# handasontam/PERT-GNN-KDD23

Hardware: AMD Instinct MI355X
Metric: training graphs/sec (whole node) (higher is better)
Workload: dtype bf16; 1 GPU; model=PERT-GNN 8L/256H, global_batch=1024, vocab=realistic, interfaces=2041, entry_unions=266, graph_mode=full, parallelism=dp1

## Files before the change

csrc/bindings.cpp:

```cpp
#include <hip/hip_runtime.h>
#include <torch/extension.h>

#include <cstdlib>

#include <c10/cuda/CUDAStream.h>

namespace {

#define CHECK_IN(t)                                                      \
  TORCH_CHECK((t).is_cuda(), #t " must be on GPU");                      \
  TORCH_CHECK((t).is_contiguous(), #t " must be contiguous")

inline hipStream_t cur_stream() {
  return (hipStream_t)c10::cuda::getCurrentCUDAStream().stream();
}

}

void launch_edge_attn_fwd(const float*, const float*, const float*,
                          const float*, const int*, const int*, const float*,
                          float*, float*, int, int, hipStream_t);
void launch_edge_attn_bwd(const float*, const float*, const float*,
                          const float*, const float*, const float*, const int*,
                          const int*, const int*, const int*, float*, float*,
                          float*, float*, float*, float*, int, int, long,
                          hipStream_t);
void launch_seg_pool_fwd(const float*, const float*, const float*, const int*,
                         float*, float*, int, int, int, hipStream_t);
void launch_seg_pool_bwd(const float*, const float*, const float*, const long*,
                         float*, long, int, hipStream_t);
void launch_embed_node_fwd(const float*, const long*, const float*, float*,
                           long, int, int, hipStream_t);
void launch_embed_node_fwd16(const float*, const long*, const float*, void*,
                             long, int, int, hipStream_t);
void launch_vocab_scatter16(const void*, const long*, long, float*, long, int,
                            int, int, int, hipStream_t);
void launch_embed_edge_fwd(const long*, const float*, const float*, float*,
                           long, int, int, hipStream_t);
void launch_gather_rows(const long*, const float*, float*, long, int,
                        hipStream_t);
bool bn_wide_ok(int);
int bn_wide_slab_rows(long, int);
void launch_bn_fwd(const float*, const float*, const float*, float*, float*,
                   float*, float*, float*, float*, long, int, float, float,
                   bool, bool, float, const unsigned long long*, float*,
                   hipStream_t);
void launch_counter_bump(unsigned long long*, hipStream_t);
void launch_bn_bwd(const float*, const float*, const float*, const float*,
                   const float*, const float*, float*, float*, float*, float*,
                   long, int, bool, float, float*, hipStream_t);
void launch_bn_stats_only(const float*, long, int, float*, float*,
                          hipStream_t);
void launch_bn_finalize_apply(const float*, const float*, const float*,
                              const float*, const float*, float*, float*,
                              float*, float*, float*, long, int, float, float,
                              bool, bool, float, const unsigned long long*,
                              hipStream_t);
void launch_bn_bwd_partials_only(const float*, const float*, const float*,
                                 const float*, const float*, long, int, bool,
                                 float*, float, float*, hipStream_t);
void launch_bn_bwd_apply_only(const float*, const float*, const float*,
                              const float*, const float*, const float*,
                              const float*, const float*, float*, long, int,
                              bool, float, hipStream_t);
void launch_bn_grad_affine(const float*, float*, float*, int, hipStream_t);
void launch_bn_stats_only16(const void*, long, int, float*, float*,
                            hipStream_t);
void launch_bn_fwd16(const void*, const float*, const float*, float*, float*,
                     float*, float*, float*, void*, long, int, float, float,
                     bool, bool, float, const unsigned long long*, float*,
                     unsigned char*, hipStream_t);
void launch_bn_finalize_apply16(const void*, const float*, const float*,
                                const float*, const float*, float*, float*,
                                float*, float*, void*, long, int, float, float,
                                bool, bool, float, const unsigned long long*,
                                unsigned char*, hipStream_t);
void launch_bn_bwd_partials_only16(const void*, const void*, const void*,
                                   const float*, const float*, long, int, bool,
                                   float*, float, float*,
                                   const unsigned char*, hipStream_t);
void launch_bn_bwd_apply_only16(const void*, const void*, const void*,
                                const float*, const float*, const float*,
                                const float*, const float*, void*, long, int,
                                bool, float, const unsigned char*,
                                hipStream_t);
void launch_bn_bwd16(const void*, const void*, const void*, const float*,
                     const float*, const float*, float*, void*, float*,
                     float*, long, int, bool, float, float*,
                     const unsigned char*, hipStream_t);
void launch_seg_pool_fwd16(const void*, const float*, const float*,
                           const int*, float*, float*, int, int, int,
                           hipStream_t);
void launch_seg_pool_bwd16(const float*, const float*, const float*,
                           const long*, void*, long, int, hipStream_t);
void launch_gemm_bf16_nt_a16o16(const void*, const float*, const float*,
                                void*, int, int, int, hipStream_t);
void launch_gemm_bf16_nn_a16o16(const void*, const float*, void*, int, int,
                                int, hipStream_t);
void launch_gemm_bf16_tn_a16b16(const void*, const void*, float*, float*, int,
                                int, int, hipStream_t);
void launch_gemm_fp16_nt_a16o16(const void*, const float*, const float*,
                                void*, int, int, int, hipStream_t);
void launch_gemm_fp16_nn_a16o16(const void*, const float*, void*, int, int,
                                int, hipStream_t);
void launch_gemm_fp16_tn_a16b16(const void*, const void*, float*, float*, int,
                                int, int, hipStream_t);
void launch_quantile_loss_fwd(const float*, const float*, float*, long, float,
                              hipStream_t);
void launch_quantile_loss_bwd(const float*, const float*, const float*, float*,
                              long, float, hipStream_t);
void launch_eval_metrics(const float*, const float*, float*, long, float,
                         hipStream_t);
void launch_adam(float*, const float*, float*, float*, float*, long, float,
                 float, float, float, float, hipStream_t);
void launch_adam_dynamic(float*, const float*, float*, float*, float*, float*,
                         long, float, float, float, float, float, float,
                         float, hipStream_t);
void launch_gemm_f32_nt(const float*, const float*, const float*, float*, int,
                        int, int, bool, hipStream_t);
void launch_gemm_f32_nn(const float*, const float*, const float*, float*, int,
                        int, int, bool, hipStream_t);
void launch_gemm_f32_tn(const float*, const float*, float*, float*, int, int,
                        int, hipStream_t);
void launch_colsum(const float*, float*, long, int, hipStream_t);
void launch_gemm_bf16_nt(const float*, const float*, const float*, float*,
                         int, int, int, bool, hipStream_t);
void launch_gemm_bf16_nn(const float*, const float*, const float*, float*,
                         int, int, int, bool, hipStream_t);
void launch_gemm_bf16_tn(const float*, const float*, float*, float*, int, int,
                         int, hipStream_t);
void launch_gemm_fp16_nt(const float*, const float*, const float*, float*,
                         int, int, int, bool, hipStream_t);
void launch_gemm_fp16_nn(const float*, const float*, const float*, float*,
                         int, int, int, bool, hipStream_t);
void launch_gemm_fp16_tn(const float*, const float*, float*, float*, int, int,
                         int, hipStream_t);
void launch_embed_grouped_scatter(const float*, const int*, const int*, float*,
                                  float*, long, int, int, int, int, int,
                                  hipStream_t);
void launch_embed_grouped_scatter_bal(const void*, int, const int*,
                                      const int*, const int*, const int*,
                                      const int*, const int*, float*, float*,
                                      float*, int, int, int, int, int, int,
                                      hipStream_t);
void launch_rows_sum_lists(const void*, int, const int*, const int*, void*, int,
                           int, int, int, hipStream_t);
void launch_vocab_scatter(const float*, const long*, long, float*, long, int,
                          int, int, int, hipStream_t);
void launch_vocab_scatter_dual(const float*, const long*, int, float*, float*,
                               long, int, int, int, hipStream_t);
void launch_edge_attn_fused_fwd(const float*, const float*, const float*,
                                const long*, int, const int*, const int*,
                                float*, float*, int, int, int, hipStream_t);
void launch_edge_attn_fused_bwd(const float*, const float*, const float*,
                                const float*, const long*, int, const float*,
                                const int*, const int*, const int*,
                                const int*, const int*, float*, float*,
                                float*, int, int, long, int, hipStream_t);
void launch_edge_attn_fused_fwd16(const void*, const void*, const void*,
                                  int, const long*, int, const int*,
                                  const int*, void*, int, float*, int, int,
                                  int, hipStream_t);
void launch_edge_attn_fused_bwd16(const void*, int, const void*,
                                  const void*, const void*, int, const long*,
                                  int, const float*, const int*, const int*,
                                  const int*, const int*, const int*, void*,
                                  void*, float*, int, int, long, int,
                                  hipStream_t);
void launch_edge_attn_fused_infer(const float*, const float*, const float*,
                                  const long*, int, const int*, const int*,
                                  const float*, const float*, int, float*,
                                  int, int, int, hipStream_t);
void launch_edge_attn_fused_infer16(const void*, const void*, const void*,
                                    int, const long*, int, const int*,
                                    const int*, const float*, const float*,
                                    int, void*, int, int, int, int,
                                    hipStream_t);
void launch_vocab_scatter_dual16(const void*, const long*, int, float*,
                                 float*, long, int, int, int, hipStream_t);
void launch_gemm_bf16_nt_o16(const float*, const float*, const float*, void*,
                             int, int, int, hipStream_t);
void launch_gemm_a16_glds_nt(const void*, const void*, const float*,
                             const float*, void*, int, int, int, int, bool,
                             hipStream_t);
void launch_convert_w16(const float*, void*, long, hipStream_t);
void launch_gemm_a16_glds_tn(const void*, const void*, float*, float*, int,
                             int, int, hipStream_t);
void launch_transpose_convert_w16(const float*, void*, int, int, hipStream_t);
void launch_gemm_skinny_nn(const void*, const float*, float*, int, int, int,
                           hipStream_t);
void launch_gemm_bf16_nn_a16(const void*, const float*, float*, int, int, int,
                             hipStream_t);
void launch_gemm_bf16_tn_a16(const void*, const float*, float*, float*, int,
                             int, int, hipStream_t);
int ptables_max_groups();
void launch_ptables_fwd(int, const float* const*, const float* const*,
                        void* const*, const int*, int, int, hipStream_t);
void launch_ptables_dgrad(const void* const*, const float* const*, const int*,
                          float* const*, const int*, int, int, bool,
                          hipStream_t);
bool launch_ptables_wgrad(int, const void* const*, const float* const*,
                          float* const*, const int*, int, bool, hipStream_t);
std::vector<torch::Tensor> collate_native(
    std::vector<torch::Tensor>, std::vector<torch::Tensor>,
    std::vector<torch::Tensor>, std::vector<torch::Tensor>,
    std::vector<torch::Tensor>, std::vector<torch::Tensor>,
    std::vector<torch::Tensor>, std::vector<torch::Tensor>,
    std::vector<torch::Tensor>, bool);


std::vector<torch::Tensor> edge_attn_fwd(torch::Tensor q, torch::Tensor k,
                                         torch::Tensor v, torch::Tensor e,
                                         torch::Tensor row_ptr,
                                         torch::Tensor csr_src,
                                         torch::Tensor skip) {
  CHECK_IN(q); CHECK_IN(k); CHECK_IN(v); CHECK_IN(e);
  CHECK_IN(row_ptr); CHECK_IN(csr_src);
  const int n = q.size(0);
  const int h = q.size(1);
  TORCH_CHECK(h <= 512, "H must be <= 512");
  auto out = torch::empty_like(q);
  auto alpha = torch::empty({e.size(0)}, q.options());
  const float* skip_p = nullptr;
  if (skip.defined() && skip.numel() > 0) {
    CHECK_IN(skip);
    skip_p = skip.data_ptr<float>();
  }
  launch_edge_attn_fwd(q.data_ptr<float>(), k.data_ptr<float>(),
                       v.data_ptr<float>(), e.data_ptr<float>(),
                       row_ptr.data_ptr<int>(), csr_src.data_ptr<int>(),
                       skip_p, out.data_ptr<float>(), alpha.data_ptr<float>(),
                       n, h, cur_stream());
  return {out, alpha};
}

std::vector<torch::Tensor> edge_attn_bwd(
    torch::Tensor g, torch::Tensor q, torch::Tensor k, torch::Tensor v,
    torch::Tensor e, torch::Tensor alpha, torch::Tensor row_ptr,
    torch::Tensor csr_src, torch::Tensor col_ptr, torch::Tensor csc_dst,
    torch::Tensor csc_eid) {
  CHECK_IN(g); CHECK_IN(q); CHECK_IN(alpha);
  const int n = q.size(0);
  const int h = q.size(1);
  const long ne = e.size(0);
  auto dq = torch::empty_like(q);
  auto dk = torch::empty_like(k);
  auto dv = torch::empty_like(v);
  auto de = torch::empty_like(e);
  auto dek = torch::empty_like(e);
  auto dev = torch::empty_like(e);
  launch_edge_attn_bwd(g.data_ptr<float>(), q.data_ptr<float>(),
                       k.data_ptr<float>(), v.data_ptr<float>(),
                       e.data_ptr<float>(), alpha.data_ptr<float>(),
                       row_ptr.data_ptr<int>(), csr_src.data_ptr<int>(),
                       col_ptr.data_ptr<int>(), csc_eid.data_ptr<int>(),
                       dq.data_ptr<float>(), dk.data_ptr<float>(),
                       dv.data_ptr<float>(), de.data_ptr<float>(),
                       dek.data_ptr<float>(), dev.data_ptr<float>(), n, h, ne,
                       cur_stream());
  return {dq, dk, dv, de};
}

torch::Tensor seg_pool_fwd(torch::Tensor x, torch::Tensor probs,
                           torch::Tensor nn, torch::Tensor batch_ptr,
                           int64_t num_graphs) {
  CHECK_IN(x); CHECK_IN(probs); CHECK_IN(nn); CHECK_IN(batch_ptr);
  const int h = x.size(1);
  const long n = x.size(0);
  long p = 8192 / std::max<int64_t>(num_graphs, 1);
  const long per_g = (n + std::max<int64_t>(num_graphs, 1) - 1) /
                     std::max<int64_t>(num_graphs, 1);
  p = std::min<long>(std::max<long>(std::min(p, per_g), 1), 64);
  auto partial = torch::empty({num_graphs * p, h}, x.options());
  auto out = torch::empty({num_graphs, h}, x.options());
  launch_seg_pool_fwd(x.data_ptr<float>(), probs.data_ptr<float>(),
                      nn.data_ptr<float>(), batch_ptr.data_ptr<int>(),
                      partial.data_ptr<float>(), out.data_ptr<float>(),
                      (int)num_graphs, (int)p, h, cur_stream());
  return out;
}

torch::Tensor seg_pool_bwd(torch::Tensor gout, torch::Tensor probs,
                           torch::Tensor nn, torch::Tensor batch) {
  CHECK_IN(gout); CHECK_IN(batch);
  const long n = batch.size(0);
  const int h = gout.size(1);
  auto dx = torch::empty({n, h}, gout.options());
  launch_seg_pool_bwd(gout.data_ptr<float>(), probs.data_ptr<float>(),
                      nn.data_ptr<float>(), batch.data_ptr<long>(),
                      dx.data_ptr<float>(), n, h, cur_stream());
  return dx;
}

torch::Tensor embed_node_fwd(torch::Tensor x_raw, torch::Tensor idx,
                             torch::Tensor table, bool out16 = false) {
  CHECK_IN(x_raw); CHECK_IN(idx); CHECK_IN(table);
  const long n = x_raw.size(0);
  const int f = x_raw.size(1);
  const int h = table.size(1);
  if (out16) {
    auto out = torch::empty({n, f + h},
                            x_raw.options().dtype(torch::kBFloat16));
    launch_embed_node_fwd16(x_raw.data_ptr<float>(), idx.data_ptr<long>(),
                            table.data_ptr<float>(), out.data_ptr(), n, f, h,
                            cur_stream());
    return out;
  }
  auto out = torch::empty({n, f + h}, x_raw.options());
  launch_embed_node_fwd(x_raw.data_ptr<float>(), idx.data_ptr<long>(),
                        table.data_ptr<float>(), out.data_ptr<float>(), n, f,
                        h, cur_stream());
  return out;
}

torch::Tensor embed_edge_fwd(torch::Tensor attr, torch::Tensor ifc,
                             torch::Tensor rpc) {
  CHECK_IN(attr); CHECK_IN(ifc); CHECK_IN(rpc);
  const long e = attr.size(0);
  const int h = ifc.size(1);
  const int astride = attr.size(1);
  auto out = torch::empty({e, 2 * h}, ifc.options());
  launch_embed_edge_fwd(attr.data_ptr<long>(), ifc.data_ptr<float>(),
                        rpc.data_ptr<float>(), out.data_ptr<float>(), e, h,
                        astride, cur_stream());
  return out;
}

torch::Tensor gather_rows(torch::Tensor idx, torch::Tensor table) {
  CHECK_IN(idx); CHECK_IN(table);
  const long n = idx.size(0);
  const int h = table.size(1);
  auto out = torch::empty({n, h}, table.options());
  launch_gather_rows(idx.data_ptr<long>(), table.data_ptr<float>(),
                     out.data_ptr<float>(), n, h, cur_stream());
  return out;
}

static const unsigned long long* rng_seed_ptr(torch::Tensor& seed,
                                              double dropout_p) {
  if (dropout_p <= 0.0 || !seed.defined() || seed.numel() == 0) return nullptr;
  TORCH_CHECK(seed.scalar_type() == torch::kLong && seed.is_cuda(),
              "dropout seed must be an int64 CUDA scalar");
  return (const unsigned long long*)seed.data_ptr<long>();
}

static torch::Tensor bn_wide_slab(const torch::Tensor& x) {
  const long rows = bn_wide_slab_rows(x.size(0), (int)x.size(1));
  return torch::empty({rows, 2 * x.size(1)},
                      x.options().dtype(torch::kFloat32));
}
static float* bn_slab_ptr(const torch::Tensor& slab) {
  return slab.numel() ? slab.data_ptr<float>() : nullptr;
}
static const unsigned char* bn_mask_ptr(const torch::Tensor& ym,
                                        const torch::Tensor& x) {
  if (ym.scalar_type() != torch::kUInt8) return nullptr;
  TORCH_CHECK(ym.is_contiguous() && x.size(1) % 8 == 0 &&
                  ym.numel() == x.size(0) * (x.size(1) / 8) &&
                  bn_wide_ok((int)x.size(1)),
              "BN keep mask must be a contiguous uint8 [n, h/8] tensor");
  return ym.data_ptr<unsigned char>();
}
static torch::Tensor bn_new_mask(const torch::Tensor& x, bool training,
                                 bool relu) {
  const long n = x.size(0), h = x.size(1);
  const bool on = training && relu && n > 0 && bn_wide_ok((int)h);
  return torch::empty({on ? n : 0, on ? h / 8 : 0},
                      x.options().dtype(torch::kUInt8));
}

std::vector<torch::Tensor> bn_relu_fwd(torch::Tensor x, torch::Tensor gamma,
                                       torch::Tensor beta,
                                       torch::Tensor running_mean,
                                       torch::Tensor running_var,
                                       double momentum, double eps,
                                       bool training, bool relu,
                                       double dropout_p = 0.0,
                                       torch::Tensor seed = {}) {
  CHECK_IN(x); CHECK_IN(gamma); CHECK_IN(beta);
  const long n = x.size(0);
  const int h = x.size(1);
  auto y = torch::empty_like(x);
  auto mean = torch::empty({h}, x.options());
  auto invstd = torch::empty({h}, x.options());
  auto partials = torch::empty({2 * h}, x.options());
  auto slab = training ? bn_wide_slab(x) : torch::empty({0}, x.options());
  const auto* sp = rng_seed_ptr(seed, dropout_p);
  launch_bn_fwd(x.data_ptr<float>(), gamma.data_ptr<float>(),
                beta.data_ptr<float>(), running_mean.data_ptr<float>(),
                running_var.data_ptr<float>(), mean.data_ptr<float>(),
                invstd.data_ptr<float>(), partials.data_ptr<float>(),
                y.data_ptr<float>(), n, h, (float)momentum, (float)eps,
                training, relu, (float)dropout_p, sp, bn_slab_ptr(slab),
                cur_stream());
  if (sp) launch_counter_bump((unsigned long long*)seed.data_ptr<long>(),
                              cur_stream());
  return {y, mean, invstd};
}

std::vector<torch::Tensor> bn_relu_bwd(torch::Tensor g, torch::Tensor x,
                                       torch::Tensor gamma, torch::Tensor mean,
                                       torch::Tensor invstd, torch::Tensor y,
                                       bool relu, double keep_inv = 1.0) {
  CHECK_IN(g); CHECK_IN(x);
  const long n = x.size(0);
  const int h = x.size(1);
  auto dx = torch::empty_like(x);
  auto dgamma = torch::empty({h}, x.options());
  auto dbeta = torch::empty({h}, x.options());
  auto partials = torch::empty({2 * h}, x.options());
  auto slab = bn_wide_slab(x);
  launch_bn_bwd(g.data_ptr<float>(), x.data_ptr<float>(), y.data_ptr<float>(),
                mean.data_ptr<float>(), invstd.data_ptr<float>(),
                gamma.data_ptr<float>(), partials.data_ptr<float>(),
                dx.data_ptr<float>(), dgamma.data_ptr<float>(),
                dbeta.data_ptr<float>(), n, h, relu, (float)keep_inv,
                bn_slab_ptr(slab), cur_stream());
  return {dx, dgamma, dbeta};
}

torch::Tensor quantile_loss_fwd(torch::Tensor y, torch::Tensor y_hat,
                                double tau) {
  CHECK_IN(y); CHECK_IN(y_hat);
  auto out = torch::empty({}, y_hat.options());
  launch_quantile_loss_fwd(y.data_ptr<float>(), y_hat.data_ptr<float>(),
                           out.data_ptr<float>(), y.size(0), (float)tau,
                           cur_stream());
  return out;
}

torch::Tensor quantile_loss_bwd(torch::Tensor g, torch::Tensor y,
                                torch::Tensor y_hat, double tau) {
  auto gc = g.contiguous();
  auto dy_hat = torch::empty_like(y_hat);
  launch_quantile_loss_bwd(gc.data_ptr<float>(), y.data_ptr<float>(),
                           y_hat.data_ptr<float>(), dy_hat.data_ptr<float>(),
                           y.size(0), (float)tau, cur_stream());
  return dy_hat;
}

std::vector<torch::Tensor> eval_metrics(torch::Tensor y, torch::Tensor y_hat,
                                        double tau) {
  CHECK_IN(y); CHECK_IN(y_hat);
  auto out3 = torch::empty({3}, y_hat.options());
  launch_eval_metrics(y.data_ptr<float>(), y_hat.data_ptr<float>(),
                      out3.data_ptr<float>(), y.size(0), (float)tau,
                      cur_stream());
  return {out3[0], out3[1], out3[2]};
}

void adam_step(torch::Tensor p, torch::Tensor g, torch::Tensor m,
               torch::Tensor v, torch::Tensor state, double lr, double b1,
               double b2, double eps, double gscale = 1.0) {
  CHECK_IN(p); CHECK_IN(g); CHECK_IN(m); CHECK_IN(v); CHECK_IN(state);
  launch_adam(p.data_ptr<float>(), g.data_ptr<float>(), m.data_ptr<float>(),
              v.data_ptr<float>(), state.data_ptr<float>(), p.numel(),
              (float)lr, (float)b1, (float)b2, (float)eps, (float)gscale, cur_stream());
}

void adam_step_dynamic(torch::Tensor p, torch::Tensor g, torch::Tensor m,
                       torch::Tensor v, torch::Tensor state,
                       torch::Tensor sstate, double lr, double b1, double b2,
                       double eps, double backoff, double growth,
                       double growth_interval) {
  CHECK_IN(p); CHECK_IN(g); CHECK_IN(m); CHECK_IN(v); CHECK_IN(state);
  CHECK_IN(sstate);
  TORCH_CHECK(sstate.numel() >= 3, "scaler state needs 3 elements");
  launch_adam_dynamic(p.data_ptr<float>(), g.data_ptr<float>(),
                      m.data_ptr<float>(), v.data_ptr<float>(),
                      state.data_ptr<float>(), sstate.data_ptr<float>(),
                      p.numel(), (float)lr, (float)b1, (float)b2, (float)eps,
// ... 467 lines not shown
      gamma.data_ptr<float>(), beta.data_ptr<float>(),
      running_mean.data_ptr<float>(), running_var.data_ptr<float>(),
      mean.data_ptr<float>(), invstd.data_ptr<float>(), y.data_ptr<float>(),
      x.size(0), h, (float)momentum, (float)eps, training, relu,
      (float)dropout_p, sp, cur_stream());
  if (sp) launch_counter_bump((unsigned long long*)seed.data_ptr<long>(),
                              cur_stream());
  return {y, mean, invstd};
}

torch::Tensor bn_bwd_partials(torch::Tensor g, torch::Tensor x,
                              torch::Tensor y, torch::Tensor mean,
                              torch::Tensor invstd, bool relu,
                              double keep_inv = 1.0) {
  CHECK_IN(g); CHECK_IN(x);
  const long h = x.size(1);
  auto partials = torch::empty({2 * h + 1}, x.options());
  auto slab = bn_wide_slab(x);
  launch_bn_bwd_partials_only(g.data_ptr<float>(), x.data_ptr<float>(),
                              y.data_ptr<float>(), mean.data_ptr<float>(),
                              invstd.data_ptr<float>(), x.size(0), h,
                              relu, partials.data_ptr<float>(),
                              (float)keep_inv, bn_slab_ptr(slab),
                              cur_stream());
  partials.narrow(0, 2 * h, 1).fill_((float)x.size(0));
  return partials;
}

std::vector<torch::Tensor> bn_bwd_apply(torch::Tensor g, torch::Tensor x,
                                        torch::Tensor y, torch::Tensor mean,
                                        torch::Tensor invstd,
                                        torch::Tensor gamma,
                                        torch::Tensor partials_global,
                                        torch::Tensor partials_local,
                                        bool relu, double keep_inv = 1.0) {
  CHECK_IN(g); CHECK_IN(x);
  const int h = x.size(1);
  TORCH_CHECK(partials_global.numel() == 2 * h + 1,
              "bn_bwd_apply expects [2h+1] partials with the global count "
              "in the tail slot");
  auto dx = torch::empty_like(x);
  auto dgamma = torch::empty({h}, x.options());
  auto dbeta = torch::empty({h}, x.options());
  launch_bn_bwd_apply_only(g.data_ptr<float>(), x.data_ptr<float>(),
                           y.data_ptr<float>(), mean.data_ptr<float>(),
                           invstd.data_ptr<float>(), gamma.data_ptr<float>(),
                           partials_global.data_ptr<float>(),
                           partials_global.data_ptr<float>() + 2 * h,
                           dx.data_ptr<float>(), x.size(0), h, relu,
                           (float)keep_inv, cur_stream());
  launch_bn_grad_affine(partials_local.data_ptr<float>(),
                        dgamma.data_ptr<float>(), dbeta.data_ptr<float>(), h,
                        cur_stream());
  return {dx, dgamma, dbeta};
}

torch::Tensor linear_dgrad(torch::Tensor g, torch::Tensor w, int64_t prec) {
  CHECK_IN(g); CHECK_IN(w);
  const int m = g.size(0);
  const int n = w.size(0);
  const int k = w.size(1);
  auto dx = torch::empty({m, k}, g.options());
  if (prec == 1)
    launch_gemm_bf16_nn(g.data_ptr<float>(), w.data_ptr<float>(), nullptr,
                        dx.data_ptr<float>(), m, n, k, false, cur_stream());
  else if (prec == 2)
    launch_gemm_fp16_nn(g.data_ptr<float>(), w.data_ptr<float>(), nullptr,
                        dx.data_ptr<float>(), m, n, k, false, cur_stream());
  else
    launch_gemm_f32_nn(g.data_ptr<float>(), w.data_ptr<float>(), nullptr,
                       dx.data_ptr<float>(), m, n, k, false, cur_stream());
  return dx;
}

std::vector<torch::Tensor> linear_wgrad(torch::Tensor g, torch::Tensor x,
                                        bool has_bias, int64_t prec) {
  CHECK_IN(g); CHECK_IN(x);
  const int m = x.size(0);
  const int k = x.size(1);
  const int n = g.size(1);
  auto dw = torch::empty({n, k}, x.options());
  torch::Tensor db = torch::empty({0}, g.options());
  float* db_ptr = nullptr;
  if (has_bias) {
    db = torch::empty({n}, g.options());
    db_ptr = db.data_ptr<float>();
  }
  if (prec == 1)
    launch_gemm_bf16_tn(g.data_ptr<float>(), x.data_ptr<float>(),
                        dw.data_ptr<float>(), db_ptr, m, n, k, cur_stream());
  else if (prec == 2)
    launch_gemm_fp16_tn(g.data_ptr<float>(), x.data_ptr<float>(),
                        dw.data_ptr<float>(), db_ptr, m, n, k, cur_stream());
  else
    launch_gemm_f32_tn(g.data_ptr<float>(), x.data_ptr<float>(),
                       dw.data_ptr<float>(), db_ptr, m, n, k, cur_stream());
  return {dw, db};
}

std::vector<torch::Tensor> vocab_scatter_dual(torch::Tensor g,
                                              torch::Tensor ea, int64_t rows0,
                                              int64_t rows1) {
  CHECK_IN(g); CHECK_IN(ea);
  const int h = g.size(1);
  TORCH_CHECK(h % 256 == 0, "dual scatter needs h % 256 == 0");
  TORCH_CHECK((size_t)(rows0 + rows1) * h * 4 <= 160 * 1024, "tables too large");
  auto fopt = g.options().dtype(torch::kFloat32);
  auto dt0 = torch::empty({rows0, h}, fopt);
  auto dt1 = torch::empty({rows1, h}, fopt);
  if (g.scalar_type() == torch::kBFloat16)
    launch_vocab_scatter_dual16(g.data_ptr(), ea.data_ptr<long>(),
                                (int)ea.size(1), dt0.data_ptr<float>(),
                                dt1.data_ptr<float>(), g.size(0), (int)rows0,
                                (int)rows1, h, cur_stream());
  else
    launch_vocab_scatter_dual(g.data_ptr<float>(), ea.data_ptr<long>(),
                              (int)ea.size(1), dt0.data_ptr<float>(),
                              dt1.data_ptr<float>(), g.size(0), (int)rows0,
                              (int)rows1, h, cur_stream());
  return {dt0, dt1};
}

torch::Tensor linear_fwd_bf16_o16(torch::Tensor x, torch::Tensor w,
                                  torch::Tensor b) {
  CHECK_IN(x); CHECK_IN(w);
  const int m = x.size(0);
  const int k = x.size(1);
  const int n = w.size(0);
  auto y = torch::empty({m, n}, x.options().dtype(torch::kBFloat16));
  const float* bias = nullptr;
  if (b.defined() && b.numel() > 0) bias = b.data_ptr<float>();
  launch_gemm_bf16_nt_o16(x.data_ptr<float>(), w.data_ptr<float>(), bias,
                          y.data_ptr(), m, n, k,
                          cur_stream());
  return y;
}

torch::Tensor linear_dgrad16(torch::Tensor g, torch::Tensor w) {
  CHECK_IN(g); CHECK_IN(w);
  const int m = g.size(0);
  const int n = w.size(0);
  const int k = w.size(1);
  auto dx = torch::empty({m, k}, w.options());
  if (m <= 16) {
    launch_gemm_skinny_nn(g.data_ptr(), w.data_ptr<float>(),
                          dx.data_ptr<float>(), m, n, k, cur_stream());
    return dx;
  }
  launch_gemm_bf16_nn_a16(g.data_ptr(),
                          w.data_ptr<float>(), dx.data_ptr<float>(), m, n, k,
                          cur_stream());
  return dx;
}

std::vector<torch::Tensor> linear_wgrad16(torch::Tensor g, torch::Tensor x,
                                          bool has_bias) {
  CHECK_IN(g); CHECK_IN(x);
  const int m = x.size(0);
  const int k = x.size(1);
  const int n = g.size(1);
  auto dw = torch::empty({n, k}, x.options());
  torch::Tensor db = torch::empty({0}, x.options());
  float* db_ptr = nullptr;
  if (has_bias) {
    db = torch::empty({n}, x.options());
    db_ptr = db.data_ptr<float>();
  }
  launch_gemm_bf16_tn_a16(g.data_ptr(),
                          x.data_ptr<float>(), dw.data_ptr<float>(), db_ptr,
                          m, n, k, cur_stream());
  return {dw, db};
}



std::vector<torch::Tensor> bn_relu_fwd16(torch::Tensor x, torch::Tensor gamma,
                                         torch::Tensor beta,
                                         torch::Tensor running_mean,
                                         torch::Tensor running_var,
                                         double momentum, double eps,
                                         bool training, bool relu,
                                         double dropout_p = 0.0,
                                         torch::Tensor seed = {}) {
  CHECK_IN(x); CHECK_IN(gamma); CHECK_IN(beta);
  const long n = x.size(0);
  const int h = x.size(1);
  auto fopt = x.options().dtype(torch::kFloat32);
  auto y = torch::empty({n, h}, x.options().dtype(torch::kBFloat16));
  auto mean = torch::empty({h}, fopt);
  auto invstd = torch::empty({h}, fopt);
  auto partials = torch::empty({2 * h}, fopt);
  auto slab = training ? bn_wide_slab(x) : torch::empty({0}, fopt);
  auto mask = bn_new_mask(x, training, relu);
  const auto* sp = rng_seed_ptr(seed, dropout_p);
  launch_bn_fwd16(x.data_ptr(), gamma.data_ptr<float>(),
                  beta.data_ptr<float>(), running_mean.data_ptr<float>(),
                  running_var.data_ptr<float>(), mean.data_ptr<float>(),
                  invstd.data_ptr<float>(), partials.data_ptr<float>(),
                  y.data_ptr(), n, h, (float)momentum, (float)eps, training,
                  relu, (float)dropout_p, sp, bn_slab_ptr(slab),
                  mask.numel() ? mask.data_ptr<unsigned char>() : nullptr,
                  cur_stream());
  if (sp) launch_counter_bump((unsigned long long*)seed.data_ptr<long>(),
                              cur_stream());
  return {y, mean, invstd, mask};
}

std::vector<torch::Tensor> bn_relu_bwd16(torch::Tensor g, torch::Tensor x,
                                         torch::Tensor gamma,
                                         torch::Tensor mean,
                                         torch::Tensor invstd, torch::Tensor y,
                                         bool relu, double keep_inv = 1.0) {
  CHECK_IN(g); CHECK_IN(x);
  const long n = x.size(0);
  const int h = x.size(1);
  auto fopt = x.options().dtype(torch::kFloat32);
  auto dx = torch::empty_like(x);
  auto dgamma = torch::empty({h}, fopt);
  auto dbeta = torch::empty({h}, fopt);
  auto partials = torch::empty({2 * h}, fopt);
  auto slab = bn_wide_slab(x);
  launch_bn_bwd16(g.data_ptr(), x.data_ptr(), y.data_ptr(),
                  mean.data_ptr<float>(), invstd.data_ptr<float>(),
                  gamma.data_ptr<float>(), partials.data_ptr<float>(),
                  dx.data_ptr(), dgamma.data_ptr<float>(),
                  dbeta.data_ptr<float>(), n, h, relu, (float)keep_inv,
                  bn_slab_ptr(slab), bn_mask_ptr(y, x), cur_stream());
  return {dx, dgamma, dbeta};
}

std::vector<torch::Tensor> bn_finalize_apply16(
    torch::Tensor x, torch::Tensor partials,
    torch::Tensor gamma, torch::Tensor beta, torch::Tensor running_mean,
    torch::Tensor running_var, double momentum, double eps, bool training,
    bool relu, double dropout_p = 0.0, torch::Tensor seed = {}) {
  CHECK_IN(x); CHECK_IN(partials);
  const int h = x.size(1);
  TORCH_CHECK(partials.numel() == 2 * h + 1,
              "bn_finalize_apply16 expects [2h+1] partials with the global "
              "count in the tail slot");
  auto fopt = x.options().dtype(torch::kFloat32);
  auto y = torch::empty({x.size(0), h}, x.options().dtype(torch::kBFloat16));
  auto mean = torch::empty({h}, fopt);
  auto invstd = torch::empty({h}, fopt);
  auto mask = bn_new_mask(x, training, relu);
  const auto* sp = rng_seed_ptr(seed, dropout_p);
  launch_bn_finalize_apply16(
      x.data_ptr(), partials.data_ptr<float>(),
      partials.data_ptr<float>() + 2 * h,
      gamma.data_ptr<float>(), beta.data_ptr<float>(),
      running_mean.data_ptr<float>(), running_var.data_ptr<float>(),
      mean.data_ptr<float>(), invstd.data_ptr<float>(), y.data_ptr(),
      x.size(0), h, (float)momentum, (float)eps, training, relu,
      (float)dropout_p, sp,
      mask.numel() ? mask.data_ptr<unsigned char>() : nullptr, cur_stream());
  if (sp) launch_counter_bump((unsigned long long*)seed.data_ptr<long>(),
                              cur_stream());
  return {y, mean, invstd, mask};
}

torch::Tensor bn_bwd_partials16(torch::Tensor g, torch::Tensor x,
                                torch::Tensor y, torch::Tensor mean,
                                torch::Tensor invstd, bool relu,
                                double keep_inv = 1.0) {
  CHECK_IN(g); CHECK_IN(x);
  const long h = x.size(1);
  auto partials = torch::empty({2 * h + 1},
                               x.options().dtype(torch::kFloat32));
  auto slab = bn_wide_slab(x);
  launch_bn_bwd_partials_only16(g.data_ptr(), x.data_ptr(),
                                y.data_ptr(), mean.data_ptr<float>(),
                                invstd.data_ptr<float>(), x.size(0), h,
                                relu, partials.data_ptr<float>(),
                                (float)keep_inv, bn_slab_ptr(slab),
                                bn_mask_ptr(y, x), cur_stream());
  partials.narrow(0, 2 * h, 1).fill_((float)x.size(0));
  return partials;
}

std::vector<torch::Tensor> bn_bwd_apply16(
    torch::Tensor g, torch::Tensor x, torch::Tensor y, torch::Tensor mean,
    torch::Tensor invstd, torch::Tensor gamma, torch::Tensor partials_global,
    torch::Tensor partials_local, bool relu, double keep_inv = 1.0) {
  CHECK_IN(g); CHECK_IN(x);
  const int h = x.size(1);
  TORCH_CHECK(partials_global.numel() == 2 * h + 1,
              "bn_bwd_apply16 expects [2h+1] partials with the global count "
              "in the tail slot");
  auto fopt = x.options().dtype(torch::kFloat32);
  auto dx = torch::empty_like(x);
  auto dgamma = torch::empty({h}, fopt);
  auto dbeta = torch::empty({h}, fopt);
  launch_bn_bwd_apply_only16(g.data_ptr(), x.data_ptr(), y.data_ptr(),
                             mean.data_ptr<float>(), invstd.data_ptr<float>(),
                             gamma.data_ptr<float>(),
                             partials_global.data_ptr<float>(),
                             partials_global.data_ptr<float>() + 2 * h,
                             dx.data_ptr(), x.size(0), h, relu,
                             (float)keep_inv, bn_mask_ptr(y, x), cur_stream());
  launch_bn_grad_affine(partials_local.data_ptr<float>(),
                        dgamma.data_ptr<float>(), dbeta.data_ptr<float>(), h,
                        cur_stream());
  return {dx, dgamma, dbeta};
}

torch::Tensor seg_pool_fwd16(torch::Tensor x, torch::Tensor probs,
                             torch::Tensor nn, torch::Tensor batch_ptr,
                             int64_t num_graphs) {
  CHECK_IN(x); CHECK_IN(probs); CHECK_IN(nn); CHECK_IN(batch_ptr);
  const int h = x.size(1);
  const long n = x.size(0);
  long p = 8192 / std::max<int64_t>(num_graphs, 1);
  const long per_g = (n + std::max<int64_t>(num_graphs, 1) - 1) /
                     std::max<int64_t>(num_graphs, 1);
  p = std::min<long>(std::max<long>(std::min(p, per_g), 1), 64);
  auto fopt = x.options().dtype(torch::kFloat32);
  auto partial = torch::empty({num_graphs * p, h}, fopt);
  auto out = torch::empty({num_graphs, h}, fopt);
  launch_seg_pool_fwd16(x.data_ptr(), probs.data_ptr<float>(),
                        nn.data_ptr<float>(), batch_ptr.data_ptr<int>(),
                        partial.data_ptr<float>(), out.data_ptr<float>(),
                        (int)num_graphs, (int)p, h, cur_stream());
  return out;
}

torch::Tensor seg_pool_bwd16(torch::Tensor gout, torch::Tensor probs,
                             torch::Tensor nn, torch::Tensor batch) {
  CHECK_IN(gout); CHECK_IN(batch);
  const long n = batch.size(0);
  const int h = gout.size(1);
  auto dx = torch::empty({n, h}, gout.options().dtype(torch::kBFloat16));
  launch_seg_pool_bwd16(gout.data_ptr<float>(), probs.data_ptr<float>(),
                        nn.data_ptr<float>(), batch.data_ptr<long>(),
                        dx.data_ptr(), n, h, cur_stream());
  return dx;
}

torch::Tensor linear_fwd_a16o16(torch::Tensor x, torch::Tensor w,
                                torch::Tensor b, bool fp16c = false) {
  CHECK_IN(x); CHECK_IN(w);
  const int m = x.size(0);
  const int k = x.size(1);
  const int n = w.size(0);
  auto y = torch::empty({m, n}, x.options());
  const float* bias = nullptr;
  if (b.defined() && b.numel() > 0) bias = b.data_ptr<float>();
  if (fp16c) {
    launch_gemm_fp16_nt_a16o16(x.data_ptr(), w.data_ptr<float>(), bias,
                               y.data_ptr(), m, n, k, cur_stream());
    return y;
  }
  if (m >= 512 && n % 128 == 0 && k % 32 == 0) {
    auto w16 = torch::empty({n, k}, x.options());
    launch_convert_w16(w.data_ptr<float>(), w16.data_ptr(), (long)n * k,
                       cur_stream());
    launch_gemm_a16_glds_nt(x.data_ptr(), w16.data_ptr(),
                            w.data_ptr<float>(), bias, y.data_ptr(),
                            1, m, n, k, false, cur_stream());
    return y;
  }
  launch_gemm_bf16_nt_a16o16(x.data_ptr(), w.data_ptr<float>(), bias,
                             y.data_ptr(), m, n, k, cur_stream());
  return y;
}

torch::Tensor linear_dgrad16_o16(torch::Tensor g, torch::Tensor w,
                                 bool fp16c = false) {
  CHECK_IN(g); CHECK_IN(w);
  const int m = g.size(0);
  const int n = w.size(0);
  const int k = w.size(1);
  auto dx = torch::empty({m, k}, g.options());
  if (fp16c) {
    launch_gemm_fp16_nn_a16o16(g.data_ptr(), w.data_ptr<float>(),
                               dx.data_ptr(), m, n, k, cur_stream());
    return dx;
  }
  if (m >= 512 && k % 128 == 0 && n % 64 == 0) {
    auto wt16 = torch::empty({k, n}, g.options());
    launch_transpose_convert_w16(w.data_ptr<float>(), wt16.data_ptr(), n, k,
                                 cur_stream());
    launch_gemm_a16_glds_nt(g.data_ptr(), wt16.data_ptr(), nullptr, nullptr,
                            dx.data_ptr(), 1, m, k, n, false,
                            cur_stream());
    const int m_done = m - m % 128;
    if (m_done < m)
      launch_gemm_bf16_nn_a16o16(
          (const char*)g.data_ptr() + (long)m_done * n * 2,
          w.data_ptr<float>(),
          (char*)dx.data_ptr() + (long)m_done * k * 2, m - m_done, n, k,
          cur_stream());
    return dx;
  }
  launch_gemm_bf16_nn_a16o16(g.data_ptr(), w.data_ptr<float>(),
                             dx.data_ptr(), m, n, k, cur_stream());
  return dx;
}

std::vector<torch::Tensor> linear_wgrad16_b16(torch::Tensor g, torch::Tensor x,
                                              bool has_bias,
                                              bool fp16c = false) {
  CHECK_IN(g); CHECK_IN(x);
  const int m = x.size(0);
  const int k = x.size(1);
  const int n = g.size(1);
  auto fopt = x.options().dtype(torch::kFloat32);
  auto dw = torch::empty({n, k}, fopt);
  torch::Tensor db = torch::empty({0}, fopt);
  float* db_ptr = nullptr;
  if (has_bias) {
    db = torch::empty({n}, fopt);
    db_ptr = db.data_ptr<float>();
  }
  if (fp16c) {
    launch_gemm_fp16_tn_a16b16(g.data_ptr(), x.data_ptr(),
                               dw.data_ptr<float>(), db_ptr, m, n, k,
                               cur_stream());
    return {dw, db};
  }
  const char* det = getenv("PERTGNN_DETERMINISTIC");
  if (!(det && det[0] == '1') && m >= 512 && n % 128 == 0 && k % 128 == 0) {
    launch_gemm_a16_glds_tn(g.data_ptr(), x.data_ptr(), dw.data_ptr<float>(),
                            db_ptr, m, n, k, cur_stream());
    return {dw, db};
  }
  launch_gemm_bf16_tn_a16b16(g.data_ptr(), x.data_ptr(),
                             dw.data_ptr<float>(), db_ptr, m, n, k,
                             cur_stream());
  return {dw, db};
}


namespace {

int ptables_check(const torch::Tensor& ifc_table,
                  const torch::Tensor& rpc_table,
                  const std::vector<torch::Tensor>& we_ifc,
                  const std::vector<torch::Tensor>& we_rpc) {
  CHECK_IN(ifc_table); CHECK_IN(rpc_table);
  TORCH_CHECK(ifc_table.dim() == 2 && rpc_table.dim() == 2,
              "ptables: tables must be 2-D");
  TORCH_CHECK(ifc_table.scalar_type() == torch::kFloat32 &&
                  rpc_table.scalar_type() == torch::kFloat32,
              "ptables: tables must be float32");
  const int64_t h = ifc_table.size(1);
  TORCH_CHECK(h > 0 && rpc_table.size(1) == h,
              "ptables: tables must share a non-empty hidden size");
  TORCH_CHECK(!we_ifc.empty() && we_ifc.size() == we_rpc.size(),
              "ptables: need one we_ifc and one we_rpc per layer, got ",
              we_ifc.size(), " and ", we_rpc.size());
  for (const auto* list : {&we_ifc, &we_rpc})
    for (const auto& w : *list) {
      TORCH_CHECK(w.is_cuda() && w.device() == ifc_table.device(),
                  "ptables: weight must be on the tables' GPU");
      TORCH_CHECK(w.is_contiguous(), "ptables: weight must be contiguous");
      TORCH_CHECK(w.scalar_type() == torch::kFloat32,
                  "ptables: weight must be float32");
      TORCH_CHECK(w.dim() == 2 && w.size(0) == h && w.size(1) == h,
                  "ptables: weight must be [", h, ", ", h, "]");
    }
  TORCH_CHECK(ifc_table.size(0) < (1 << 30) && rpc_table.size(0) < (1 << 30) &&
                  h < (1 << 15),
              "ptables: table too large");
  return (int)h;
}

}

std::vector<torch::Tensor> ptables_fwd(torch::Tensor ifc_table,
                                       torch::Tensor rpc_table,
                                       std::vector<torch::Tensor> we_ifc,
                                       std::vector<torch::Tensor> we_rpc) {
  const int h = ptables_check(ifc_table, rpc_table, we_ifc, we_rpc);
  const int layers = (int)we_ifc.size();
  auto opt = ifc_table.options().dtype(torch::kBFloat16);
  std::vector<torch::Tensor> out;
  std::vector<const float*> a, w;
  std::vector<void*> c;
  std::vector<int> m;
  for (int t = 0; t < 2; ++t) {
    const auto& table = t == 0 ? ifc_table : rpc_table;
    const auto& ws = t == 0 ? we_ifc : we_rpc;
    for (int l = 0; l < layers; ++l) {
      out.push_back(torch::empty({table.size(0), h}, opt));
      a.push_back(table.data_ptr<float>());
      w.push_back(ws[l].data_ptr<float>());
      c.push_back(out.back().data_ptr());
      m.push_back((int)table.size(0));
    }
  }
  launch_ptables_fwd(2 * layers, a.data(), w.data(), c.data(), m.data(), h, h,
                     cur_stream());
  return out;
}

std::vector<torch::Tensor> ptables_bwd(std::vector<torch::Tensor> dP,
                                       torch::Tensor ifc_table,
                                       torch::Tensor rpc_table,
                                       std::vector<torch::Tensor> we_ifc,
                                       std::vector<torch::Tensor> we_rpc,
                                       int64_t dgrad_splits) {
  const int h = ptables_check(ifc_table, rpc_table, we_ifc, we_rpc);
  const int layers = (int)we_ifc.size();
  TORCH_CHECK((int)dP.size() == 2 * layers, "ptables_bwd: need ", 2 * layers,
              " dP entries, got ", dP.size());
  const int64_t rows[2] = {ifc_table.size(0), rpc_table.size(0)};
  bool missing = false;
  for (int g = 0; g < 2 * layers; ++g) {
    const auto& d = dP[g];
    if (!d.defined() || d.numel() == 0) {
      missing |= rows[g / layers] > 0;
      continue;
    }
    TORCH_CHECK(d.is_cuda() && d.device() == ifc_table.device(),
                "ptables_bwd: dP must be on the tables' GPU");
    TORCH_CHECK(d.is_contiguous(), "ptables_bwd: dP must be contiguous");
    TORCH_CHECK(d.scalar_type() == torch::kBFloat16,
                "ptables_bwd: dP must be bfloat16");
    TORCH_CHECK(d.dim() == 2 && d.size(0) == rows[g / layers] && d.size(1) == h,
                "ptables_bwd: dP[", g, "] must be [", rows[g / layers], ", ",
                h, "]");
  }
  const char* det_env = getenv("PERTGNN_DETERMINISTIC");
  const bool det = det_env && det_env[0] == '1';
  const int splits =
      det ? 1 : (int)std::min<int64_t>(std::max<int64_t>(dgrad_splits, 1), layers);

  const int64_t hh = (int64_t)h * h;
  const int64_t n_dw = 2 * layers * hh;
  auto buf = torch::empty({n_dw + (rows[0] + rows[1]) * h},
                          ifc_table.options());
  auto dW = buf.narrow(0, 0, n_dw).view({2 * layers, h, h});
  auto d_ifc = buf.narrow(0, n_dw, rows[0] * h).view({rows[0], h});
  auto d_rpc = buf.narrow(0, n_dw + rows[0] * h, rows[1] * h).view({rows[1], h});

  std::vector<const void*> dp_w, dp_d;
  std::vector<const float*> a_w, w_d;
  std::vector<float*> dw_w;
  std::vector<int> m_w;
  int npairs[2] = {0, 0};
  for (int g = 0; g < 2 * layers; ++g) {
    const auto& d = dP[g];
    if (!d.defined() || d.numel() == 0) continue;
    const int t = g / layers;
    const auto& table = t == 0 ? ifc_table : rpc_table;
    const auto& w = (t == 0 ? we_ifc : we_rpc)[g % layers];
    dp_w.push_back(d.data_ptr());
    a_w.push_back(table.data_ptr<float>());
    dw_w.push_back(dW.data_ptr<float>() + g * hh);
    m_w.push_back((int)rows[t]);
    dp_d.push_back(d.data_ptr());
    w_d.push_back(w.data_ptr<float>());
    ++npairs[t];
  }
  auto s = cur_stream();
  const bool zero_dw =
      missing || launch_ptables_wgrad((int)dp_w.size(), dp_w.data(), a_w.data(),
                                      dw_w.data(), m_w.data(), h, true, s);
  const bool zero_dt = splits > 1;
  if (zero_dw || zero_dt) {
    float* beg = buf.data_ptr<float>() + (zero_dw ? 0 : n_dw);
    const int64_t cnt = (zero_dw ? n_dw : 0) +
                        (zero_dt ? (rows[0] + rows[1]) * h : 0);
    const hipError_t err = hipMemsetAsync(beg, 0, cnt * sizeof(float), s);
    TORCH_CHECK(err == hipSuccess, "ptables_bwd: memset failed: ",
                hipGetErrorString(err));
  }
  float* outs[2] = {d_ifc.data_ptr<float>(), d_rpc.data_ptr<float>()};
  const int ms[2] = {(int)rows[0], (int)rows[1]};
  launch_ptables_dgrad(dp_d.data(), w_d.data(), npairs, outs, ms, h, splits,
                       zero_dt, s);
  launch_ptables_wgrad((int)dp_w.size(), dp_w.data(), a_w.data(), dw_w.data(),
                       m_w.data(), h, false, s);
  return {d_ifc, d_rpc, dW};
}

PYBIND11_MODULE(TORCH_EXTENSION_NAME, mod) {
  mod.def("ptables_fwd", &ptables_fwd, py::arg("ifc_table"),
          py::arg("rpc_table"), py::arg("we_ifc"), py::arg("we_rpc"));
  mod.def("ptables_bwd", &ptables_bwd, py::arg("dP"), py::arg("ifc_table"),
          py::arg("rpc_table"), py::arg("we_ifc"), py::arg("we_rpc"),
          py::arg("dgrad_splits") = 1);
  mod.def("ptables_max_groups", &ptables_max_groups);
  mod.def("linear_fwd_bf16_o16", &linear_fwd_bf16_o16);
  mod.def("linear_dgrad16", &linear_dgrad16);
  mod.def("linear_wgrad16", &linear_wgrad16);
  mod.def("vocab_scatter_dual", &vocab_scatter_dual);
  mod.def("linear_dgrad", &linear_dgrad);
  mod.def("linear_wgrad", &linear_wgrad);
  mod.def("embed_grouped_scatter_bal", &embed_grouped_scatter_bal);
  mod.def("edge_table_grad", &edge_table_grad, py::arg("de"), py::arg("idx1"),
          py::arg("lptr1"), py::arg("idx2"), py::arg("lptr2"),
          py::arg("idx3"), py::arg("lptr3"), py::arg("V"), py::arg("R"),
          py::arg("out_dtype"), py::arg("unroll") = 8);
  mod.def("bn_stats", &bn_stats);
  mod.def("bn_finalize_apply", &bn_finalize_apply, py::arg("x"),
          py::arg("partials"), py::arg("gamma"), py::arg("beta"),
          py::arg("running_mean"), py::arg("running_var"), py::arg("momentum"),
          py::arg("eps"), py::arg("training"), py::arg("relu"),
          py::arg("dropout_p") = 0.0, py::arg("seed") = torch::Tensor());
  mod.def("bn_bwd_partials", &bn_bwd_partials, py::arg("g"), py::arg("x"),
          py::arg("y"), py::arg("mean"), py::arg("invstd"), py::arg("relu"),
          py::arg("keep_inv") = 1.0);
  mod.def("bn_bwd_apply", &bn_bwd_apply, py::arg("g"), py::arg("x"),
          py::arg("y"), py::arg("mean"), py::arg("invstd"), py::arg("gamma"),
          py::arg("partials_global"), py::arg("partials_local"),
          py::arg("relu"), py::arg("keep_inv") = 1.0);
  mod.def("vocab_scatter", &vocab_scatter);
  mod.def("collate_native", &collate_native,
          py::call_guard<py::gil_scoped_release>());
  mod.def("edge_attn_fused_fwd", &edge_attn_fused_fwd, py::arg("qkvs"),
          py::arg("pifc"), py::arg("prpc"), py::arg("edge_attr"),
          py::arg("row_ptr"), py::arg("csr_src"), py::arg("out16"),
          py::arg("heads") = 1);
  mod.def("edge_attn_fused_bwd", &edge_attn_fused_bwd, py::arg("g"),
          py::arg("qkvs"), py::arg("pifc"), py::arg("prpc"),
          py::arg("edge_attr"), py::arg("alpha"), py::arg("row_ptr"),
          py::arg("csr_src"), py::arg("col_ptr"), py::arg("csc_dst"),
          py::arg("csc_eid"), py::arg("heads") = 1);
  mod.def("edge_attn_fused_infer", &edge_attn_fused_infer, py::arg("qkvs"),
          py::arg("pifc"), py::arg("prpc"), py::arg("edge_attr"),
          py::arg("row_ptr"), py::arg("csr_src"), py::arg("bn_scale"),
          py::arg("bn_shift"), py::arg("relu"), py::arg("out16"),
          py::arg("heads") = 1);
  mod.def("embed_grouped_scatter", &embed_grouped_scatter);
  mod.def("linear_fwd", &linear_fwd);
  mod.def("linear_fwd_bf16", &linear_fwd_bf16);
  mod.def("linear_fwd_fp16", &linear_fwd_fp16);
  mod.def("linear_bwd_fp16", &linear_bwd_fp16);
  mod.def("linear_bwd_bf16", &linear_bwd_bf16);
  mod.def("gemm_nt_bf16", &gemm_nt_bf16);
  mod.def("gemm_nn_bf16", &gemm_nn_bf16);
  mod.def("gemm_tn_bf16", &gemm_tn_bf16);
  mod.def("linear_bwd", &linear_bwd);
  mod.def("gemm_nt", &gemm_nt);
  mod.def("gemm_nn", &gemm_nn);
  mod.def("gemm_tn", &gemm_tn);
  mod.def("edge_attn_fwd", &edge_attn_fwd);
  mod.def("edge_attn_bwd", &edge_attn_bwd);
  mod.def("seg_pool_fwd", &seg_pool_fwd);
  mod.def("seg_pool_bwd", &seg_pool_bwd);
  mod.def("embed_node_fwd", &embed_node_fwd, py::arg("x_raw"), py::arg("idx"), py::arg("table"), py::arg("out16") = false);
  mod.def("embed_edge_fwd", &embed_edge_fwd);
  mod.def("gather_rows", &gather_rows);
  mod.def("bn_relu_fwd16", &bn_relu_fwd16, py::arg("x"), py::arg("gamma"),
          py::arg("beta"), py::arg("running_mean"), py::arg("running_var"),
          py::arg("momentum"), py::arg("eps"), py::arg("training"),
          py::arg("relu"), py::arg("dropout_p") = 0.0,
          py::arg("seed") = torch::Tensor());
  mod.def("bn_relu_bwd16", &bn_relu_bwd16, py::arg("g"), py::arg("x"),
          py::arg("gamma"), py::arg("mean"), py::arg("invstd"), py::arg("y"),
          py::arg("relu"), py::arg("keep_inv") = 1.0);
  mod.def("bn_finalize_apply16", &bn_finalize_apply16, py::arg("x"),
          py::arg("partials"), py::arg("gamma"), py::arg("beta"),
          py::arg("running_mean"), py::arg("running_var"), py::arg("momentum"),
          py::arg("eps"), py::arg("training"), py::arg("relu"),
          py::arg("dropout_p") = 0.0, py::arg("seed") = torch::Tensor());
  mod.def("bn_bwd_partials16", &bn_bwd_partials16, py::arg("g"), py::arg("x"),
          py::arg("y"), py::arg("mean"), py::arg("invstd"), py::arg("relu"),
          py::arg("keep_inv") = 1.0);
  mod.def("bn_bwd_apply16", &bn_bwd_apply16, py::arg("g"), py::arg("x"),
          py::arg("y"), py::arg("mean"), py::arg("invstd"), py::arg("gamma"),
          py::arg("partials_global"), py::arg("partials_local"),
          py::arg("relu"), py::arg("keep_inv") = 1.0);
  mod.def("seg_pool_fwd16", &seg_pool_fwd16);
  mod.def("seg_pool_bwd16", &seg_pool_bwd16);
  mod.def("linear_fwd_a16o16", &linear_fwd_a16o16, py::arg("x"), py::arg("w"),
          py::arg("b"), py::arg("fp16c") = false);
  mod.def("linear_dgrad16_o16", &linear_dgrad16_o16, py::arg("g"),
          py::arg("w"), py::arg("fp16c") = false);
  mod.def("linear_wgrad16_b16", &linear_wgrad16_b16, py::arg("g"),
          py::arg("x"), py::arg("has_bias"), py::arg("fp16c") = false);
  mod.def("bn_relu_fwd", &bn_relu_fwd, py::arg("x"), py::arg("gamma"),
          py::arg("beta"), py::arg("running_mean"), py::arg("running_var"),
          py::arg("momentum"), py::arg("eps"), py::arg("training"),
          py::arg("relu"), py::arg("dropout_p") = 0.0,
          py::arg("seed") = torch::Tensor());
  mod.def("bn_relu_bwd", &bn_relu_bwd, py::arg("g"), py::arg("x"),
          py::arg("gamma"), py::arg("mean"), py::arg("invstd"), py::arg("y"),
          py::arg("relu"), py::arg("keep_inv") = 1.0);
  mod.def("quantile_loss_fwd", &quantile_loss_fwd);
  mod.def("quantile_loss_bwd", &quantile_loss_bwd);
  mod.def("eval_metrics", &eval_metrics);
  mod.def("adam_step_dynamic", &adam_step_dynamic);
  mod.def("adam_step", &adam_step, py::arg("p"), py::arg("g"), py::arg("m"),
          py::arg("v"), py::arg("state"), py::arg("lr"), py::arg("b1"),
          py::arg("b2"), py::arg("eps"), py::arg("gscale") = 1.0);
}
```

csrc/hip/common.h:

```cpp
#pragma once

#include <hip/hip_runtime.h>

#include <stdexcept>
#include <string>

#define PERTGNN_WAVE 64

#define HIP_CHECK(expr)                                                        \
  do {                                                                         \
    hipError_t _e = (expr);                                                    \
    if (_e != hipSuccess) {                                                    \
      throw std::runtime_error(std::string("HIP error ") +                     \
                               hipGetErrorString(_e) + " at " + __FILE__ +     \
                               ":" + std::to_string(__LINE__));                \
    }                                                                          \
  } while (0)

[[noreturn]] inline void pertgnn_shape_fail(const char* launcher,
                                            const char* what, long v) {
  throw std::runtime_error(std::string("pertgnn ") + launcher +
                           ": unsupported shape (" + what + "=" +
                           std::to_string(v) + ")");
}

__device__ __forceinline__ float wave_reduce_sum(float v) {
#pragma unroll
  for (int off = 32; off > 0; off >>= 1) v += __shfl_xor(v, off, 64);
  return v;
}

template <int W>
__device__ __forceinline__ float subwave_reduce_sum(float v) {
#pragma unroll
  for (int off = W / 2; off > 0; off >>= 1) v += __shfl_xor(v, off, 64);
  return v;
}

__device__ __forceinline__ float wave_reduce_max(float v) {
#pragma unroll
  for (int off = 32; off > 0; off >>= 1) v = fmaxf(v, __shfl_xor(v, off, 64));
  return v;
}

static inline int ceil_div(long a, long b) { return (int)((a + b - 1) / b); }

__device__ __forceinline__ int xcd_swizzle(int bid, int nwg) {
  const int xcd = bid % 8;
  const int q = nwg / 8;
  const int r = nwg % 8;
  return (xcd < r ? xcd * (q + 1) : r * (q + 1) + (xcd - r) * q) + bid / 8;
}
```

csrc/hip/edge_attn_fused.hip:

```cpp

#include "common.h"
#include <cmath>
#include <cstdlib>

#define WAVES_PER_BLOCK 4

typedef __attribute__((ext_vector_type(4))) float f32x4_t;
typedef __attribute__((ext_vector_type(4))) __bf16 bf16x4_t;

template <int VPT, bool VEC>
struct Slice {
  static __device__ __forceinline__ void load(const float* base, int lane,
                                              int h, float (&dst)[VPT]) {
    if constexpr (VEC) {
#pragma unroll
      for (int q = 0; q < VPT; q += 4)
        *reinterpret_cast<f32x4_t*>(&dst[q]) =
            *reinterpret_cast<const f32x4_t*>(&base[lane * VPT + q]);
    } else {
#pragma unroll
      for (int j = 0; j < VPT; ++j) {
        const int c = lane + j * PERTGNN_WAVE;
        dst[j] = (c < h) ? base[c] : 0.f;
      }
    }
  }
  static __device__ __forceinline__ void load(const __bf16* base, int lane,
                                              int h, float (&dst)[VPT]) {
    if constexpr (VEC) {
#pragma unroll
      for (int q = 0; q < VPT; q += 4) {
        const bf16x4_t v =
            *reinterpret_cast<const bf16x4_t*>(&base[lane * VPT + q]);
#pragma unroll
        for (int u = 0; u < 4; ++u) dst[q + u] = (float)v[u];
      }
    } else {
#pragma unroll
      for (int j = 0; j < VPT; ++j) {
        const int c = lane + j * PERTGNN_WAVE;
        dst[j] = (c < h) ? (float)base[c] : 0.f;
      }
    }
  }
  static __device__ __forceinline__ void load_add(const float* a,
                                                  const float* b, int lane,
                                                  int h, float (&dst)[VPT]) {
    if constexpr (VEC) {
#pragma unroll
      for (int q = 0; q < VPT; q += 4) {
        const f32x4_t va = *reinterpret_cast<const f32x4_t*>(&a[lane * VPT + q]);
        const f32x4_t vb = *reinterpret_cast<const f32x4_t*>(&b[lane * VPT + q]);
#pragma unroll
        for (int u = 0; u < 4; ++u) dst[q + u] = va[u] + vb[u];
      }
    } else {
#pragma unroll
      for (int j = 0; j < VPT; ++j) {
        const int c = lane + j * PERTGNN_WAVE;
        dst[j] = (c < h) ? a[c] + b[c] : 0.f;
      }
    }
  }
  static __device__ __forceinline__ void load_add(const __bf16* a,
                                                  const __bf16* b, int lane,
                                                  int h, float (&dst)[VPT]) {
    if constexpr (VEC) {
#pragma unroll
      for (int q = 0; q < VPT; q += 4) {
        const bf16x4_t va =
            *reinterpret_cast<const bf16x4_t*>(&a[lane * VPT + q]);
        const bf16x4_t vb =
            *reinterpret_cast<const bf16x4_t*>(&b[lane * VPT + q]);
#pragma unroll
        for (int u = 0; u < 4; ++u) dst[q + u] = (float)va[u] + (float)vb[u];
      }
    } else {
#pragma unroll
      for (int j = 0; j < VPT; ++j) {
        const int c = lane + j * PERTGNN_WAVE;
        dst[j] = (c < h) ? (float)a[c] + (float)b[c] : 0.f;
      }
    }
  }
  static __device__ __forceinline__ void store(float* base, int lane, int h,
                                               const float (&src)[VPT]) {
    if constexpr (VEC) {
#pragma unroll
      for (int q = 0; q < VPT; q += 4)
        *reinterpret_cast<f32x4_t*>(&base[lane * VPT + q]) =
            *reinterpret_cast<const f32x4_t*>(&src[q]);
    } else {
#pragma unroll
      for (int j = 0; j < VPT; ++j) {
        const int c = lane + j * PERTGNN_WAVE;
        if (c < h) base[c] = src[j];
      }
    }
  }
  static __device__ __forceinline__ void store(__bf16* base, int lane, int h,
                                               const float (&src)[VPT]) {
    if constexpr (VEC) {
#pragma unroll
      for (int q = 0; q < VPT; q += 4) {
        bf16x4_t v;
#pragma unroll
        for (int u = 0; u < 4; ++u) v[u] = (__bf16)src[q + u];
        *reinterpret_cast<bf16x4_t*>(&base[lane * VPT + q]) = v;
      }
    } else {
#pragma unroll
      for (int j = 0; j < VPT; ++j) {
        const int c = lane + j * PERTGNN_WAVE;
        if (c < h) base[c] = (__bf16)src[j];
      }
    }
  }
};

template <int LPR, int LPH>
struct HeadMap {
  static constexpr int HEADS = LPR / LPH;
  static __device__ __forceinline__ int head(int lane) {
    if constexpr (HEADS == 1) return 0;
    else return lane / LPH;
  }
  static __device__ __forceinline__ int sub(int lane) {
    if constexpr (HEADS == 1) return lane;
    else return lane % LPH;
  }
  static __device__ __forceinline__ long slot(int p, int hd) {
    if constexpr (HEADS == 1) return p;
    else return (long)p * HEADS + hd;
  }
};

template <int VPT, bool VEC, typename QT = float, int LPR = PERTGNN_WAVE,
          typename TO = float, typename PT = float, int LPH = LPR,
          bool PCH = false>
__global__ void edge_attn_fused_fwd_kernel(
    const QT* __restrict__ qkvs,
    const PT* __restrict__ pifc,
    const PT* __restrict__ prpc,
    const long* __restrict__ ea, int astride,
    const int* __restrict__ row_ptr, const int* __restrict__ csr_src,
    TO* __restrict__ out, float* __restrict__ alpha, int n, int h,
    float scale) {
  using S = Slice<VPT, VEC>;
  static_assert(VEC || LPR == PERTGNN_WAVE, "sub-wave rows need VEC layout");
  static_assert(PCH ? !VEC : (VEC || LPH == LPR),
                "heads split the sub-row (VEC) or the columns (PCH)");
  static_assert(LPH >= 1 && LPH <= LPR && (LPH & (LPH - 1)) == 0,
                "lanes per head: a power of two within the row");
  constexpr int RPW = PERTGNN_WAVE / LPR;
  const int wid = threadIdx.x / PERTGNN_WAVE;
  const int lane0 = threadIdx.x % PERTGNN_WAVE;
  const int sub = lane0 / LPR;
  const int lane = lane0 % LPR;
  const int row = (blockIdx.x * WAVES_PER_BLOCK + wid) * RPW + sub;
  if (row >= n) return;
  const long ld = 4L * h;

  float qr[VPT], acc[VPT];
  S::load(&qkvs[row * ld], lane, h, qr);
#pragma unroll
  for (int j = 0; j < VPT; ++j) acc[j] = 0.f;

  const int beg = row_ptr[row], end = row_ptr[row + 1];
  if constexpr (PCH) {
    constexpr int HPJ = PERTGNN_WAVE / LPH;
    const int heads = h / LPH;
    const int hg = lane / LPH, hl = lane % LPH;
    float m[VPT], s[VPT];
#pragma unroll
    for (int j = 0; j < VPT; ++j) { m[j] = -INFINITY; s[j] = 0.f; }
    for (int p = beg; p < end; ++p) {
      const long src = csr_src[p];
      const long a0 = ea[(long)p * astride];
      const long a1 = ea[(long)p * astride + 1];
      float ec[VPT], ke[VPT], ve[VPT], logit[VPT];
      S::load_add(&pifc[a0 * h], &prpc[a1 * h], lane, h, ec);
      S::load(&qkvs[src * ld + h], lane, h, ke);
      S::load(&qkvs[src * ld + 2 * h], lane, h, ve);
#pragma unroll
      for (int j = 0; j < VPT; ++j)
        logit[j] = subwave_reduce_sum<LPH>(qr[j] * (ke[j] + ec[j])) * scale;
      const bool writer = hl == (p - beg) % LPH;
#pragma unroll
      for (int j = 0; j < VPT; ++j) {
        if (writer && lane + j * PERTGNN_WAVE < h)
          alpha[(long)p * heads + hg + j * HPJ] = logit[j];
        const float m_new = fmaxf(m[j], logit[j]);
        const float corr = __expf(m[j] - m_new);
        const float pexp = __expf(logit[j] - m_new);
        s[j] = s[j] * corr + pexp;
        acc[j] = acc[j] * corr + pexp * (ve[j] + ec[j]);
        m[j] = m_new;
      }
    }
    float sk[VPT], res[VPT], inv_s[VPT];
    S::load(&qkvs[row * ld + 3 * h], lane, h, sk);
#pragma unroll
    for (int j = 0; j < VPT; ++j) {
      inv_s[j] = (s[j] > 0.f) ? 1.f / s[j] : 0.f;
      res[j] = acc[j] * inv_s[j] + sk[j];
    }
    S::store(&out[(long)row * h], lane, h, res);
#pragma unroll
    for (int j = 0; j < VPT; ++j) {
      if (lane + j * PERTGNN_WAVE < h) {
        for (int p = beg + hl; p < end; p += LPH) {
          const long sl = (long)p * heads + hg + j * HPJ;
          alpha[sl] = __expf(alpha[sl] - m[j]) * inv_s[j];
        }
      }
    }
    return;
  }
  using HM = HeadMap<LPR, LPH>;
  const int hd = HM::head(lane), hl = HM::sub(lane);
  float m = -INFINITY, s = 0.f;
  for (int p = beg; p < end; ++p) {
    const long src = csr_src[p];
    const long a0 = ea[(long)p * astride];
    const long a1 = ea[(long)p * astride + 1];
    float ec[VPT], ke[VPT], ve[VPT];
    S::load_add(&pifc[a0 * h], &prpc[a1 * h], lane, h, ec);
    S::load(&qkvs[src * ld + h], lane, h, ke);
    S::load(&qkvs[src * ld + 2 * h], lane, h, ve);
    float part = 0.f;
#pragma unroll
    for (int j = 0; j < VPT; ++j) part += qr[j] * (ke[j] + ec[j]);
    const float logit = subwave_reduce_sum<LPH>(part) * scale;
    if (hl == (p - beg) % LPH) alpha[HM::slot(p, hd)] = logit;
    const float m_new = fmaxf(m, logit);
    const float corr = __expf(m - m_new);
    const float pexp = __expf(logit - m_new);
    s = s * corr + pexp;
#pragma unroll
    for (int j = 0; j < VPT; ++j)
      acc[j] = acc[j] * corr + pexp * (ve[j] + ec[j]);
    m = m_new;
  }

  const float inv_s = (s > 0.f) ? 1.f / s : 0.f;
  float sk[VPT], res[VPT];
  S::load(&qkvs[row * ld + 3 * h], lane, h, sk);
#pragma unroll
  for (int j = 0; j < VPT; ++j) res[j] = acc[j] * inv_s + sk[j];
  S::store(&out[(long)row * h], lane, h, res);
  for (int p = beg + hl; p < end; p += LPH)
    alpha[HM::slot(p, hd)] = __expf(alpha[HM::slot(p, hd)] - m) * inv_s;
}

template <int VPT, bool VEC, typename QT = float, int LPR = PERTGNN_WAVE,
          typename TO = float, typename PT = float, int LPH = LPR,
          bool PCH = false>
__global__ void edge_attn_fused_infer_kernel(
    const QT* __restrict__ qkvs,
    const PT* __restrict__ pifc,
    const PT* __restrict__ prpc,
    const long* __restrict__ ea, int astride,
    const int* __restrict__ row_ptr, const int* __restrict__ csr_src,
    const float* __restrict__ bn_scale,
    const float* __restrict__ bn_shift,
    int relu, TO* __restrict__ out, int n, int h, float scale) {
  using S = Slice<VPT, VEC>;
  static_assert(VEC || LPR == PERTGNN_WAVE, "sub-wave rows need VEC layout");
  static_assert(PCH ? !VEC : (VEC || LPH == LPR),
                "heads split the sub-row (VEC) or the columns (PCH)");
  static_assert(LPH >= 1 && LPH <= LPR && (LPH & (LPH - 1)) == 0,
                "lanes per head: a power of two within the row");
  constexpr int RPW = PERTGNN_WAVE / LPR;
  const int wid = threadIdx.x / PERTGNN_WAVE;
  const int lane0 = threadIdx.x % PERTGNN_WAVE;
  const int sub = lane0 / LPR;
  const int lane = lane0 % LPR;
  const int row = (blockIdx.x * WAVES_PER_BLOCK + wid) * RPW + sub;
  if (row >= n) return;
  const long ld = 4L * h;

  float qr[VPT], acc[VPT];
  S::load(&qkvs[row * ld], lane, h, qr);
#pragma unroll
  for (int j = 0; j < VPT; ++j) acc[j] = 0.f;

  const int beg = row_ptr[row], end = row_ptr[row + 1];
  float sk[VPT], res[VPT];
  if constexpr (PCH) {
    float m[VPT], s[VPT];
#pragma unroll
    for (int j = 0; j < VPT; ++j) { m[j] = -INFINITY; s[j] = 0.f; }
    for (int p = beg; p < end; ++p) {
      const long src = csr_src[p];
      const long a0 = ea[(long)p * astride];
      const long a1 = ea[(long)p * astride + 1];
      float ec[VPT], ke[VPT], ve[VPT];
      S::load_add(&pifc[a0 * h], &prpc[a1 * h], lane, h, ec);
      S::load(&qkvs[src * ld + h], lane, h, ke);
      S::load(&qkvs[src * ld + 2 * h], lane, h, ve);
#pragma unroll
      for (int j = 0; j < VPT; ++j) {
        const float logit =
            subwave_reduce_sum<LPH>(qr[j] * (ke[j] + ec[j])) * scale;
        const float m_new = fmaxf(m[j], logit);
        const float corr = __expf(m[j] - m_new);
        const float pexp = __expf(logit - m_new);
        s[j] = s[j] * corr + pexp;
        acc[j] = acc[j] * corr + pexp * (ve[j] + ec[j]);
        m[j] = m_new;
      }
    }
    S::load(&qkvs[row * ld + 3 * h], lane, h, sk);
#pragma unroll
    for (int j = 0; j < VPT; ++j)
      res[j] = acc[j] * ((s[j] > 0.f) ? 1.f / s[j] : 0.f) + sk[j];
  } else {
    float m = -INFINITY, s = 0.f;
    for (int p = beg; p < end; ++p) {
      const long src = csr_src[p];
      const long a0 = ea[(long)p * astride];
      const long a1 = ea[(long)p * astride + 1];
      float ec[VPT], ke[VPT], ve[VPT];
      S::load_add(&pifc[a0 * h], &prpc[a1 * h], lane, h, ec);
      S::load(&qkvs[src * ld + h], lane, h, ke);
      S::load(&qkvs[src * ld + 2 * h], lane, h, ve);
      float part = 0.f;
#pragma unroll
      for (int j = 0; j < VPT; ++j) part += qr[j] * (ke[j] + ec[j]);
      const float logit = subwave_reduce_sum<LPH>(part) * scale;
      const float m_new = fmaxf(m, logit);
      const float corr = __expf(m - m_new);
      const float pexp = __expf(logit - m_new);
      s = s * corr + pexp;
#pragma unroll
      for (int j = 0; j < VPT; ++j)
        acc[j] = acc[j] * corr + pexp * (ve[j] + ec[j]);
      m = m_new;
    }

    const float inv_s = (s > 0.f) ? 1.f / s : 0.f;
    S::load(&qkvs[row * ld + 3 * h], lane, h, sk);
#pragma unroll
    for (int j = 0; j < VPT; ++j) res[j] = acc[j] * inv_s + sk[j];
  }
  if (bn_scale != nullptr) {
    float bs[VPT], bb[VPT];
    S::load(bn_scale, lane, h, bs);
    S::load(bn_shift, lane, h, bb);
#pragma unroll
    for (int j = 0; j < VPT; ++j) res[j] = res[j] * bs[j] + bb[j];
  }
  if (relu) {
#pragma unroll
    for (int j = 0; j < VPT; ++j) res[j] = fmaxf(res[j], 0.f);
  }
  S::store(&out[(long)row * h], lane, h, res);
}

template <int VPT, bool VEC, typename QT = float,
          int LPR = PERTGNN_WAVE, typename TG = float, typename PT = float,
          int LPH = LPR, bool PCH = false>
__global__ void edge_attn_fused_bwd_row_kernel(
    const TG* __restrict__ g, const QT* __restrict__ qkvs,
    const PT* __restrict__ pifc, const PT* __restrict__ prpc,
    const long* __restrict__ ea, int astride, const float* __restrict__ alpha,
    const int* __restrict__ row_ptr, const int* __restrict__ csr_src,
    QT* __restrict__ dqkvs, float* __restrict__ dal, int n, int h,
    float scale) {
  using S = Slice<VPT, VEC>;
  static_assert(VEC || LPR == PERTGNN_WAVE, "sub-wave rows need VEC layout");
  static_assert(PCH ? !VEC : (VEC || LPH == LPR),
                "heads split the sub-row (VEC) or the columns (PCH)");
  static_assert(LPH >= 1 && LPH <= LPR && (LPH & (LPH - 1)) == 0,
                "lanes per head: a power of two within the row");
  constexpr int RPW = PERTGNN_WAVE / LPR;
  const int wid = threadIdx.x / PERTGNN_WAVE;
  const int lane0 = threadIdx.x % PERTGNN_WAVE;
  const int lane = lane0 % LPR;
  const int row = (blockIdx.x * WAVES_PER_BLOCK + wid) * RPW + lane0 / LPR;
  if (row >= n) return;
  const long ld = 4L * h;

  float gr[VPT], a1[VPT], a2[VPT];
  S::load(&g[(long)row * h], lane, h, gr);
#pragma unroll
  for (int j = 0; j < VPT; ++j) { a1[j] = 0.f; a2[j] = 0.f; }

  const int beg = row_ptr[row], end = row_ptr[row + 1];
  if constexpr (PCH) {
    constexpr int HPJ = PERTGNN_WAVE / LPH;
    const int heads = h / LPH;
    const int hg = lane / LPH, hl = lane % LPH;
    float sdot[VPT];
#pragma unroll
    for (int j = 0; j < VPT; ++j) sdot[j] = 0.f;
    for (int p = beg; p < end; ++p) {
      const long src = csr_src[p];
      const long e0 = ea[(long)p * astride];
      const long e1 = ea[(long)p * astride + 1];
      float ec[VPT], ke[VPT], ve[VPT];
      S::load_add(&pifc[e0 * h], &prpc[e1 * h], lane, h, ec);
      S::load(&qkvs[src * ld + h], lane, h, ke);
      S::load(&qkvs[src * ld + 2 * h], lane, h, ve);
      const bool writer = hl == (p - beg) % LPH;
#pragma unroll
      for (int j = 0; j < VPT; ++j) {
        const float dalpha =
            subwave_reduce_sum<LPH>(gr[j] * (ve[j] + ec[j]));
        const bool live = lane + j * PERTGNN_WAVE < h;
        const long sl = (long)p * heads + hg + j * HPJ;
        const float a = live ? alpha[sl] : 0.f;
        sdot[j] += a * dalpha;
        if (writer && live) dal[sl] = dalpha;
        const float kec = ke[j] + ec[j];
        a1[j] += a * dalpha * kec;
        a2[j] += a * kec;
      }
    }
    float dq[VPT];
#pragma unroll
    for (int j = 0; j < VPT; ++j) dq[j] = scale * (a1[j] - sdot[j] * a2[j]);
    S::store(&dqkvs[row * ld], lane, h, dq);
    S::store(&dqkvs[row * ld + 3 * h], lane, h, gr);
#pragma unroll
    for (int j = 0; j < VPT; ++j) {
      if (lane + j * PERTGNN_WAVE < h) {
        for (int p = beg + hl; p < end; p += LPH) {
          const long sl = (long)p * heads + hg + j * HPJ;
          dal[sl] = scale * alpha[sl] * (dal[sl] - sdot[j]);
        }
      }
    }
    return;
  }
  using HM = HeadMap<LPR, LPH>;
  const int hd = HM::head(lane), hl = HM::sub(lane);
  float sdot = 0.f;
  for (int p = beg; p < end; ++p) {
    const long src = csr_src[p];
    const long e0 = ea[(long)p * astride];
    const long e1 = ea[(long)p * astride + 1];
    float ec[VPT], ke[VPT], ve[VPT];
    S::load_add(&pifc[e0 * h], &prpc[e1 * h], lane, h, ec);
    S::load(&qkvs[src * ld + h], lane, h, ke);
    S::load(&qkvs[src * ld + 2 * h], lane, h, ve);
    float part = 0.f;
#pragma unroll
    for (int j = 0; j < VPT; ++j) part += gr[j] * (ve[j] + ec[j]);
    const float dalpha = subwave_reduce_sum<LPH>(part);
    const float a = alpha[HM::slot(p, hd)];
    sdot += a * dalpha;
    if (hl == (p - beg) % LPH) dal[HM::slot(p, hd)] = dalpha;
#pragma unroll
    for (int j = 0; j < VPT; ++j) {
      const float kec = ke[j] + ec[j];
      a1[j] += a * dalpha * kec;
      a2[j] += a * kec;
    }
  }
  float dq[VPT];
#pragma unroll
  for (int j = 0; j < VPT; ++j) dq[j] = scale * (a1[j] - sdot * a2[j]);
  S::store(&dqkvs[row * ld], lane, h, dq);
  S::store(&dqkvs[row * ld + 3 * h], lane, h, gr);
  for (int p = beg + hl; p < end; p += LPH)
    dal[HM::slot(p, hd)] =
        scale * alpha[HM::slot(p, hd)] * (dal[HM::slot(p, hd)] - sdot);
}

template <int VPT, bool VEC, typename QT = float, typename ET = float,
          int LPR = PERTGNN_WAVE, typename TG = float, int LPH = LPR,
          bool PCH = false>
__global__ void edge_attn_fused_bwd_col_kernel(
    const TG* __restrict__ g, const QT* __restrict__ qkvs,
    const float* __restrict__ alpha, const float* __restrict__ dal,
    const int* __restrict__ col_ptr, const int* __restrict__ csc_dst,
    const int* __restrict__ csc_eid, QT* __restrict__ dqkvs,
    ET* __restrict__ de, int n, int h) {
  using S = Slice<VPT, VEC>;
  static_assert(VEC || LPR == PERTGNN_WAVE, "sub-wave rows need VEC layout");
  static_assert(PCH ? !VEC : (VEC || LPH == LPR),
                "heads split the sub-row (VEC) or the columns (PCH)");
  static_assert(LPH >= 1 && LPH <= LPR && (LPH & (LPH - 1)) == 0,
                "lanes per head: a power of two within the row");
  constexpr int RPW = PERTGNN_WAVE / LPR;
  const int wid = threadIdx.x / PERTGNN_WAVE;
  const int lane0 = threadIdx.x % PERTGNN_WAVE;
  const int lane = lane0 % LPR;
  const int row = (blockIdx.x * WAVES_PER_BLOCK + wid) * RPW + lane0 / LPR;
  if (row >= n) return;
  const long ld = 4L * h;
  float ka[VPT], va[VPT];
#pragma unroll
  for (int j = 0; j < VPT; ++j) { ka[j] = 0.f; va[j] = 0.f; }
  if constexpr (PCH) {
    constexpr int HPJ = PERTGNN_WAVE / LPH;
    const int heads = h / LPH;
    const int hg = lane / LPH;
    for (int p = col_ptr[row]; p < col_ptr[row + 1]; ++p) {
      const long eid = csc_eid[p];
      const long dst = csc_dst[p];
      float qd[VPT], gd[VPT], des[VPT];
      S::load(&qkvs[dst * ld], lane, h, qd);
      S::load(&g[dst * h], lane, h, gd);
#pragma unroll
      for (int j = 0; j < VPT; ++j) {
        const bool live = lane + j * PERTGNN_WAVE < h;
        const long sl = eid * heads + hg + j * HPJ;
        const float dk1 = (live ? dal[sl] : 0.f) * qd[j];
        const float dv1 = (live ? alpha[sl] : 0.f) * gd[j];
        ka[j] += dk1;
        va[j] += dv1;
        des[j] = dk1 + dv1;
      }
      S::store(&de[eid * h], lane, h, des);
    }
    S::store(&dqkvs[(long)row * ld + h], lane, h, ka);
    S::store(&dqkvs[(long)row * ld + 2 * h], lane, h, va);
    return;
  }
  using HM = HeadMap<LPR, LPH>;
  const int hd = HM::head(lane);
  for (int p = col_ptr[row]; p < col_ptr[row + 1]; ++p) {
    const long eid = csc_eid[p];
    const long dst = csc_dst[p];
    const float dl = dal[eid * HM::HEADS + hd];
    const float a = alpha[eid * HM::HEADS + hd];
    float qd[VPT], gd[VPT], des[VPT];
    S::load(&qkvs[dst * ld], lane, h, qd);
    S::load(&g[dst * h], lane, h, gd);
#pragma unroll
    for (int j = 0; j < VPT; ++j) {
      const float dk1 = dl * qd[j];
      const float dv1 = a * gd[j];
      ka[j] += dk1;
      va[j] += dv1;
      des[j] = dk1 + dv1;
    }
    S::store(&de[eid * h], lane, h, des);
  }
  S::store(&dqkvs[(long)row * ld + h], lane, h, ka);
  S::store(&dqkvs[(long)row * ld + 2 * h], lane, h, va);
}




[[noreturn]] static void attn_heads_fail(const char* launcher, int h,
                                         int heads, int lpr) {
  throw std::runtime_error(
      std::string("pertgnn ") + launcher + ": unsupported shape (h=" +
      std::to_string(h) + ", heads=" + std::to_string(heads) + ", lpr=" +
      std::to_string(lpr) + "): the lanes of a row cannot be split into " +
      "these heads");
}

static bool attn_heads_ok(int h, int heads) {
  return heads >= 1 && h % heads == 0;
}

static int vec_lph(int h, int heads, int vpt, int lpr) {
  if (!attn_heads_ok(h, heads)) return 0;
  const int c = h / heads;
  if (c % vpt != 0) return 0;
  const int lph = c / vpt;
  if (lph < 1 || lph > lpr || (lph & (lph - 1)) != 0) return 0;
  return lph;
}

static int pch_lanes(int h, int heads) {
  if (!attn_heads_ok(h, heads)) return 0;
  const int c = h / heads;
  return (c <= PERTGNN_WAVE && PERTGNN_WAVE % c == 0) ? c : 0;
}

#define HEAD_CHAIN(M, A, LPR, L, NAME)                                         \
  do {                                                                         \
    if ((L) == 64 && 64 <= LPR) M(A, LPR, (64 <= LPR ? 64 : LPR));             \
    else if ((L) == 32 && 32 <= LPR) M(A, LPR, (32 <= LPR ? 32 : LPR));        \
    else if ((L) == 16 && 16 <= LPR) M(A, LPR, (16 <= LPR ? 16 : LPR));        \
    else if ((L) == 8 && 8 <= LPR) M(A, LPR, (8 <= LPR ? 8 : LPR));            \
    else if ((L) == 4 && 4 <= LPR) M(A, LPR, (4 <= LPR ? 4 : LPR));            \
    else if ((L) == 2 && 2 <= LPR) M(A, LPR, (2 <= LPR ? 2 : LPR));            \
    else if ((L) == 1) M(A, LPR, 1);                                           \
    else attn_heads_fail(NAME, h, heads, LPR);                                 \
  } while (0)

void launch_edge_attn_fused_fwd(const float* qkvs, const float* pifc,
                                const float* prpc, const long* ea, int astride,
                                const int* row_ptr, const int* csr_src,
                                float* out, float* alpha, int n, int h,
                                int heads, hipStream_t stream) {
  const int vpt = (h + PERTGNN_WAVE - 1) / PERTGNN_WAVE;
  const bool vec = (h % 256 == 0);
  if (heads != 1) {
    const dim3 grid(ceil_div(n, WAVES_PER_BLOCK));
    const dim3 block(WAVES_PER_BLOCK * PERTGNN_WAVE);
    const float scale =
        attn_heads_ok(h, heads) ? 1.f / std::sqrt((float)(h / heads)) : 0.f;
#define FWD_VEC(V, LPR, LPH)                                                   \
  do {                                                                         \
    if (n > 0)                                                                 \
      edge_attn_fused_fwd_kernel<V, true, float, LPR, float, float, LPH>       \
          <<<grid, block, 0, stream>>>(qkvs, pifc, prpc, ea, astride, row_ptr, \
                                       csr_src, out, alpha, n, h, scale);      \
  } while (0)
#define FWD_PCH(V, LPR, C)                                                     \
  do {                                                                         \
    if (n > 0)                                                                 \
      edge_attn_fused_fwd_kernel<V, false, float, LPR, float, float, C, true>  \
          <<<grid, block, 0, stream>>>(qkvs, pifc, prpc, ea, astride, row_ptr, \
                                       csr_src, out, alpha, n, h, scale);      \
  } while (0)
    const char* name = "edge_attn_fused launcher";
    if (vec && vpt == 4) {
      HEAD_CHAIN(FWD_VEC, 4, 64, vec_lph(h, heads, 4, 64), name);
    } else if (vec && vpt == 8) {
      HEAD_CHAIN(FWD_VEC, 8, 64, vec_lph(h, heads, 8, 64), name);
    } else if (!vec && vpt >= 1 && vpt <= 8) {
      const int c = pch_lanes(h, heads);
      switch (vpt) {
#define CASE(V) case V: HEAD_CHAIN(FWD_PCH, V, 64, c, name); break;
        CASE(1) CASE(2) CASE(3) CASE(4) CASE(5) CASE(6) CASE(7) CASE(8)
#undef CASE
      }
    } else {
      attn_heads_fail(name, h, heads, PERTGNN_WAVE);
    }
#undef FWD_VEC
#undef FWD_PCH
    return;
  }
  if (n == 0) return;
  const float scale = 1.f / std::sqrt((float)h);
  const dim3 grid(ceil_div(n, WAVES_PER_BLOCK));
  const dim3 block(WAVES_PER_BLOCK * PERTGNN_WAVE);
  switch (vpt) {
#define CASE(V)                                                                \
  case V:                                                                      \
    if (vec && (V % 4 == 0))                                                   \
      edge_attn_fused_fwd_kernel<V, true><<<grid, block, 0, stream>>>(         \
          qkvs, pifc, prpc, ea, astride, row_ptr, csr_src, out, alpha, n, h,   \
          scale);                                                              \
    else                                                                       \
      edge_attn_fused_fwd_kernel<V, false><<<grid, block, 0, stream>>>(        \
          qkvs, pifc, prpc, ea, astride, row_ptr, csr_src, out, alpha, n, h,   \
          scale);                                                              \
    break;
    CASE(1) CASE(2) CASE(3) CASE(4) CASE(5) CASE(6) CASE(7) CASE(8)
#undef CASE
    default: pertgnn_shape_fail("edge_attn_fused launcher", "vpt", vpt);
  }
}

void launch_edge_attn_fused_bwd(const float* g, const float* qkvs,
                                const float* pifc, const float* prpc,
                                const long* ea, int astride,
                                const float* alpha, const int* row_ptr,
                                const int* csr_src, const int* col_ptr,
                                const int* csc_dst, const int* csc_eid,
                                float* dqkvs, float* de, float* dal, int n,
                                int h, long num_edges, int heads,
                                hipStream_t stream) {
  const int vpt = (h + PERTGNN_WAVE - 1) / PERTGNN_WAVE;
  const bool vec = (h % 256 == 0);
  if (heads != 1) {
    const dim3 grid(ceil_div(n, WAVES_PER_BLOCK));
    const dim3 block(WAVES_PER_BLOCK * PERTGNN_WAVE);
    const float scale =
        attn_heads_ok(h, heads) ? 1.f / std::sqrt((float)(h / heads)) : 0.f;
#define BWD_VEC(V, LPR, LPH)                                                   \
  do {                                                                         \
    if (n > 0) {                                                               \
      edge_attn_fused_bwd_row_kernel<V, true, float, LPR, float, float, LPH>   \
          <<<grid, block, 0, stream>>>(g, qkvs, pifc, prpc, ea, astride,       \
                                       alpha, row_ptr, csr_src, dqkvs, dal,    \
                                       n, h, scale);                           \
      edge_attn_fused_bwd_col_kernel<V, true, float, float, LPR, float, LPH>   \
          <<<grid, block, 0, stream>>>(g, qkvs, alpha, dal, col_ptr, csc_dst,  \
                                       csc_eid, dqkvs, de, n, h);              \
    }                                                                          \
  } while (0)
#define BWD_PCH(V, LPR, C)                                                     \
  do {                                                                         \
    if (n > 0) {                                                               \
      edge_attn_fused_bwd_row_kernel<V, false, float, LPR, float, float, C,    \
                                     true>                                     \
          <<<grid, block, 0, stream>>>(g, qkvs, pifc, prpc, ea, astride,       \
                                       alpha, row_ptr, csr_src, dqkvs, dal,    \
                                       n, h, scale);                           \
      edge_attn_fused_bwd_col_kernel<V, false, float, float, LPR, float, C,    \
                                     true>                                     \
          <<<grid, block, 0, stream>>>(g, qkvs, alpha, dal, col_ptr, csc_dst,  \
                                       csc_eid, dqkvs, de, n, h);              \
    }                                                                          \
  } while (0)
    const char* name = "edge_attn_fused launcher";
    if (vec && vpt == 4) {
      HEAD_CHAIN(BWD_VEC, 4, 64, vec_lph(h, heads, 4, 64), name);
    } else if (vec && vpt == 8) {
      HEAD_CHAIN(BWD_VEC, 8, 64, vec_lph(h, heads, 8, 64), name);
    } else if (!vec && vpt >= 1 && vpt <= 8) {
      const int c = pch_lanes(h, heads);
      switch (vpt) {
#define CASE(V) case V: HEAD_CHAIN(BWD_PCH, V, 64, c, name); break;
        CASE(1) CASE(2) CASE(3) CASE(4) CASE(5) CASE(6) CASE(7) CASE(8)
#undef CASE
      }
    } else {
      attn_heads_fail(name, h, heads, PERTGNN_WAVE);
    }
#undef BWD_VEC
#undef BWD_PCH
    return;
  }
  if (n == 0) return;
  const float scale = 1.f / std::sqrt((float)h);
  const dim3 grid(ceil_div(n, WAVES_PER_BLOCK));
  const dim3 block(WAVES_PER_BLOCK * PERTGNN_WAVE);
  switch (vpt) {
#define CASE(V)                                                                \
  case V:                                                                      \
    if (vec && (V % 4 == 0)) {                                                 \
      edge_attn_fused_bwd_row_kernel<V, true><<<grid, block, 0, stream>>>(     \
          g, qkvs, pifc, prpc, ea, astride, alpha, row_ptr, csr_src, dqkvs,    \
          dal, n, h, scale);                                                   \
      edge_attn_fused_bwd_col_kernel<V, true><<<grid, block, 0, stream>>>(     \
          g, qkvs, alpha, dal, col_ptr, csc_dst, csc_eid, dqkvs, de, n, h);    \
    } else {                                                                   \
      edge_attn_fused_bwd_row_kernel<V, false><<<grid, block, 0, stream>>>(    \
          g, qkvs, pifc, prpc, ea, astride, alpha, row_ptr, csr_src, dqkvs,    \
          dal, n, h, scale);                                                   \
      edge_attn_fused_bwd_col_kernel<V, false><<<grid, block, 0, stream>>>(    \
          g, qkvs, alpha, dal, col_ptr, csc_dst, csc_eid, dqkvs, de, n, h);    \
    }                                                                          \
    break;
    CASE(1) CASE(2) CASE(3) CASE(4) CASE(5) CASE(6) CASE(7) CASE(8)
#undef CASE
    default: pertgnn_shape_fail("edge_attn_fused launcher", "vpt", vpt);
  }
}



static int attn_lpr() {
  static int v = [] {
    const char* e = getenv("PERTGNN_ATTN_LPR");
    const int x = e ? atoi(e) : 32;
    return (x == 16 || x == 32 || x == 64) ? x : 32;
  }();
  return v;
}

void launch_edge_attn_fused_fwd16(const void* qkvs_v, const void* pifc_v,
                                  const void* prpc_v, int p16, const long* ea,
                                  int astride, const int* row_ptr,
                                  const int* csr_src, void* out_v, int out16,
                                  float* alpha, int n, int h, int heads,
                                  hipStream_t stream) {
  const __bf16* qkvs = (const __bf16*)qkvs_v;
  if (n == 0 && heads == 1) return;
  const float scale =
      attn_heads_ok(h, heads) ? 1.f / std::sqrt((float)(h / heads)) : 0.f;
  const dim3 block(WAVES_PER_BLOCK * PERTGNN_WAVE);
  const int lpr = attn_lpr();
  const int rpb = WAVES_PER_BLOCK * (PERTGNN_WAVE / lpr);
  const dim3 grid(ceil_div(n, rpb));
  const char* name = "edge_attn_fused act16 launcher";
#define FWD16(VPT, LPR, LPH)                                                   \
  do {                                                                         \
    if (n == 0) break;                                                         \
    if (p16 && out16) {                                                        \
      edge_attn_fused_fwd_kernel<VPT, true, __bf16, LPR, __bf16, __bf16, LPH>  \
          <<<grid, block, 0, stream>>>(qkvs, (const __bf16*)pifc_v,            \
                                       (const __bf16*)prpc_v, ea, astride,     \
                                       row_ptr, csr_src, (__bf16*)out_v,       \
                                       alpha, n, h, scale);                    \
    } else if (p16) {                                                          \
      edge_attn_fused_fwd_kernel<VPT, true, __bf16, LPR, float, __bf16, LPH>   \
          <<<grid, block, 0, stream>>>(qkvs, (const __bf16*)pifc_v,            \
                                       (const __bf16*)prpc_v, ea, astride,     \
                                       row_ptr, csr_src, (float*)out_v,        \
                                       alpha, n, h, scale);                    \
    } else if (out16) {                                                        \
      edge_attn_fused_fwd_kernel<VPT, true, __bf16, LPR, __bf16, float, LPH>   \
          <<<grid, block, 0, stream>>>(qkvs, (const float*)pifc_v,             \
                                       (const float*)prpc_v, ea, astride,      \
                                       row_ptr, csr_src, (__bf16*)out_v,       \
                                       alpha, n, h, scale);                    \
    } else {                                                                   \
      edge_attn_fused_fwd_kernel<VPT, true, __bf16, LPR, float, float, LPH>    \
          <<<grid, block, 0, stream>>>(qkvs, (const float*)pifc_v,             \
                                       (const float*)prpc_v, ea, astride,      \
                                       row_ptr, csr_src, (float*)out_v,        \
                                       alpha, n, h, scale);                    \
    }                                                                          \
  } while (0)
#define FWD16_H(VPT, LPR)                                                      \
  HEAD_CHAIN(FWD16, VPT, LPR, vec_lph(h, heads, VPT, LPR), name)
  if (h == 256) {
    if (lpr == 16) FWD16_H(16, 16);
    else if (lpr == 32) FWD16_H(8, 32);
    else FWD16_H(4, 64);
  } else if (h == 512) {
    if (lpr == 16 || lpr == 32) FWD16_H(16, 32);
    else FWD16_H(8, 64);
  } else if (h % 256 == 0 && h / PERTGNN_WAVE <= 32) {
    if (heads != 1) attn_heads_fail(name, h, heads, PERTGNN_WAVE);
    const int vpt = h / PERTGNN_WAVE;
    if (vpt == 4) FWD16(4, 64, 64);
    else if (vpt == 8) FWD16(8, 64, 64);
    else if (vpt == 16) FWD16(16, 64, 64);
    else FWD16(32, 64, 64);
  } else {
    pertgnn_shape_fail("edge_attn_fused act16 launcher", "h", h);
  }
#undef FWD16_H
#undef FWD16
}

void launch_edge_attn_fused_bwd16(const void* g_v, int g16,
                                  const void* qkvs_v,
                                  const void* pifc_v, const void* prpc_v,
                                  int p16, const long* ea, int astride,
                                  const float* alpha, const int* row_ptr,
                                  const int* csr_src, const int* col_ptr,
                                  const int* csc_dst, const int* csc_eid,
                                  void* dqkvs_v, void* de_v, float* dal,
                                  int n, int h, long num_edges, int heads,
                                  hipStream_t stream) {
  const __bf16* qkvs = (const __bf16*)qkvs_v;
  __bf16* dqkvs = (__bf16*)dqkvs_v;
  __bf16* de = (__bf16*)de_v;
  if (n == 0 && heads == 1) return;
  const float scale =
      attn_heads_ok(h, heads) ? 1.f / std::sqrt((float)(h / heads)) : 0.f;
  const dim3 block(WAVES_PER_BLOCK * PERTGNN_WAVE);
  const int lpr = attn_lpr();
  const int rpb = WAVES_PER_BLOCK * (PERTGNN_WAVE / lpr);
  const dim3 grid(ceil_div(n, rpb));
  const char* name = "edge_attn_fused act16 launcher";
#define BWD16(VPT, LPR, LPH)                                                   \
  do {                                                                         \
    if (n == 0) break;                                                         \
    if (g16 && p16) {                                                          \
      edge_attn_fused_bwd_row_kernel<VPT, true, __bf16, LPR, __bf16, __bf16,   \
                                     LPH>                                      \
          <<<grid, block, 0, stream>>>((const __bf16*)g_v, qkvs,               \
                                       (const __bf16*)pifc_v,                  \
                                       (const __bf16*)prpc_v,                  \
                                       ea, astride, alpha, row_ptr, csr_src,   \
                                       dqkvs, dal, n, h, scale);               \
      edge_attn_fused_bwd_col_kernel<VPT, true, __bf16, __bf16, LPR, __bf16,   \
                                     LPH>                                      \
          <<<grid, block, 0, stream>>>((const __bf16*)g_v, qkvs, alpha, dal,   \
                                       col_ptr, csc_dst, csc_eid, dqkvs, de,   \
                                       n, h);                                  \
    } else if (g16) {                                                          \
      edge_attn_fused_bwd_row_kernel<VPT, true, __bf16, LPR, __bf16, float,    \
                                     LPH>                                      \
          <<<grid, block, 0, stream>>>((const __bf16*)g_v, qkvs,               \
                                       (const float*)pifc_v,                   \
                                       (const float*)prpc_v,                   \
                                       ea, astride, alpha, row_ptr, csr_src,   \
                                       dqkvs, dal, n, h, scale);               \
      edge_attn_fused_bwd_col_kernel<VPT, true, __bf16, __bf16, LPR, __bf16,   \
                                     LPH>                                      \
          <<<grid, block, 0, stream>>>((const __bf16*)g_v, qkvs, alpha, dal,   \
                                       col_ptr, csc_dst, csc_eid, dqkvs, de,   \
                                       n, h);                                  \
    } else if (p16) {                                                          \
              \
      edge_attn_fused_bwd_row_kernel<VPT, true, __bf16, LPR, float, __bf16,    \
                                     LPH>                                      \
          <<<grid, block, 0, stream>>>((const float*)g_v, qkvs,                \
                                       (const __bf16*)pifc_v,                  \
                                       (const __bf16*)prpc_v,                  \
                                       ea, astride, alpha, row_ptr, csr_src,   \
                                       dqkvs, dal, n, h, scale);               \
      edge_attn_fused_bwd_col_kernel<VPT, true, __bf16, __bf16, LPR, float,    \
                                     LPH>                                      \
          <<<grid, block, 0, stream>>>((const float*)g_v, qkvs, alpha, dal,    \
                                       col_ptr, csc_dst, csc_eid, dqkvs, de,   \
                                       n, h);                                  \
    } else {                                                                   \
      edge_attn_fused_bwd_row_kernel<VPT, true, __bf16, LPR, float, float,     \
                                     LPH>                                      \
          <<<grid, block, 0, stream>>>((const float*)g_v, qkvs,                \
                                       (const float*)pifc_v,                   \
                                       (const float*)prpc_v,                   \
                                       ea, astride, alpha, row_ptr, csr_src,   \
                                       dqkvs, dal, n, h, scale);               \
      edge_attn_fused_bwd_col_kernel<VPT, true, __bf16, __bf16, LPR, float,    \
                                     LPH>                                      \
          <<<grid, block, 0, stream>>>((const float*)g_v, qkvs, alpha, dal,    \
                                       col_ptr, csc_dst, csc_eid, dqkvs, de,   \
                                       n, h);                                  \
    }                                                                          \
  } while (0)
#define BWD16_H(VPT, LPR)                                                      \
  HEAD_CHAIN(BWD16, VPT, LPR, vec_lph(h, heads, VPT, LPR), name)
  if (h == 256) {
    if (lpr == 16) BWD16_H(16, 16);
    else if (lpr == 32) BWD16_H(8, 32);
    else BWD16_H(4, 64);
  } else if (h == 512) {
    if (lpr == 16 || lpr == 32) BWD16_H(16, 32);
    else BWD16_H(8, 64);
  } else if (h % 256 == 0 && h / PERTGNN_WAVE <= 32) {
    if (heads != 1) attn_heads_fail(name, h, heads, PERTGNN_WAVE);
    const int vpt = h / PERTGNN_WAVE;
    if (vpt == 4) BWD16(4, 64, 64);
    else if (vpt == 8) BWD16(8, 64, 64);
    else if (vpt == 16) BWD16(16, 64, 64);
    else BWD16(32, 64, 64);
  } else {
    pertgnn_shape_fail("edge_attn_fused act16 launcher", "h", h);
  }
#undef BWD16_H
#undef BWD16
}



void launch_edge_attn_fused_infer(const float* qkvs, const float* pifc,
                                  const float* prpc, const long* ea,
                                  int astride, const int* row_ptr,
                                  const int* csr_src, const float* bn_scale,
                                  const float* bn_shift, int relu, float* out,
                                  int n, int h, int heads,
                                  hipStream_t stream) {
  const int vpt = (h + PERTGNN_WAVE - 1) / PERTGNN_WAVE;
  const bool vec = (h % 256 == 0);
  if (heads != 1) {
    const dim3 grid(ceil_div(n, WAVES_PER_BLOCK));
    const dim3 block(WAVES_PER_BLOCK * PERTGNN_WAVE);
    const float scale =
        attn_heads_ok(h, heads) ? 1.f / std::sqrt((float)(h / heads)) : 0.f;
#define INF_VEC(V, LPR, LPH)                                                   \
  do {                                                                         \
    if (n > 0)                                                                 \
      edge_attn_fused_infer_kernel<V, true, float, LPR, float, float, LPH>     \
          <<<grid, block, 0, stream>>>(qkvs, pifc, prpc, ea, astride, row_ptr, \
                                       csr_src, bn_scale, bn_shift, relu, out, \
                                       n, h, scale);                           \
  } while (0)
#define INF_PCH(V, LPR, C)                                                     \
  do {                                                                         \
    if (n > 0)                                                                 \
      edge_attn_fused_infer_kernel<V, false, float, LPR, float, float, C,      \
                                   true>                                       \
          <<<grid, block, 0, stream>>>(qkvs, pifc, prpc, ea, astride, row_ptr, \
                                       csr_src, bn_scale, bn_shift, relu, out, \
                                       n, h, scale);                           \
  } while (0)
    const char* name = "edge_attn_fused infer launcher";
    if (vec && vpt == 4) {
      HEAD_CHAIN(INF_VEC, 4, 64, vec_lph(h, heads, 4, 64), name);
    } else if (vec && vpt == 8) {
      HEAD_CHAIN(INF_VEC, 8, 64, vec_lph(h, heads, 8, 64), name);
    } else if (!vec && vpt >= 1 && vpt <= 8) {
      const int c = pch_lanes(h, heads);
      switch (vpt) {
#define CASE(V) case V: HEAD_CHAIN(INF_PCH, V, 64, c, name); break;
        CASE(1) CASE(2) CASE(3) CASE(4) CASE(5) CASE(6) CASE(7) CASE(8)
#undef CASE
      }
    } else {
      attn_heads_fail(name, h, heads, PERTGNN_WAVE);
    }
#undef INF_VEC
#undef INF_PCH
    return;
  }
  if (n == 0) return;
  const float scale = 1.f / std::sqrt((float)h);
  const dim3 grid(ceil_div(n, WAVES_PER_BLOCK));
  const dim3 block(WAVES_PER_BLOCK * PERTGNN_WAVE);
  switch (vpt) {
#define CASE(V)                                                                \
  case V:                                                                      \
    if (vec && (V % 4 == 0))                                                   \
      edge_attn_fused_infer_kernel<V, true><<<grid, block, 0, stream>>>(       \
          qkvs, pifc, prpc, ea, astride, row_ptr, csr_src, bn_scale,           \
          bn_shift, relu, out, n, h, scale);                                   \
    else                                                                       \
      edge_attn_fused_infer_kernel<V, false><<<grid, block, 0, stream>>>(      \
          qkvs, pifc, prpc, ea, astride, row_ptr, csr_src, bn_scale,           \
          bn_shift, relu, out, n, h, scale);                                   \
    break;
    CASE(1) CASE(2) CASE(3) CASE(4) CASE(5) CASE(6) CASE(7) CASE(8)
#undef CASE
    default: pertgnn_shape_fail("edge_attn_fused infer launcher", "vpt", vpt);
  }
}

void launch_edge_attn_fused_infer16(const void* qkvs_v, const void* pifc_v,
                                    const void* prpc_v, int p16,
                                    const long* ea, int astride,
                                    const int* row_ptr, const int* csr_src,
                                    const float* bn_scale,
                                    const float* bn_shift, int relu,
                                    void* out_v, int out16, int n, int h,
                                    int heads, hipStream_t stream) {
  const __bf16* qkvs = (const __bf16*)qkvs_v;
  if (n == 0 && heads == 1) return;
  const float scale =
      attn_heads_ok(h, heads) ? 1.f / std::sqrt((float)(h / heads)) : 0.f;
  const dim3 block(WAVES_PER_BLOCK * PERTGNN_WAVE);
  const int lpr = attn_lpr();
  const int rpb = WAVES_PER_BLOCK * (PERTGNN_WAVE / lpr);
  const dim3 grid(ceil_div(n, rpb));
  const char* name = "edge_attn_fused infer act16 launcher";
#define INF16(VPT, LPR, LPH)                                                   \
  do {                                                                         \
    if (n == 0) break;                                                         \
    if (p16 && out16) {                                                        \
      edge_attn_fused_infer_kernel<VPT, true, __bf16, LPR, __bf16, __bf16,     \
                                   LPH>                                        \
          <<<grid, block, 0, stream>>>(qkvs, (const __bf16*)pifc_v,            \
                                       (const __bf16*)prpc_v, ea, astride,     \
                                       row_ptr, csr_src, bn_scale, bn_shift,   \
                                       relu, (__bf16*)out_v, n, h, scale);     \
    } else if (p16) {                                                          \
      edge_attn_fused_infer_kernel<VPT, true, __bf16, LPR, float, __bf16,      \
                                   LPH>                                        \
          <<<grid, block, 0, stream>>>(qkvs, (const __bf16*)pifc_v,            \
                                       (const __bf16*)prpc_v, ea, astride,     \
                                       row_ptr, csr_src, bn_scale, bn_shift,   \
                                       relu, (float*)out_v, n, h, scale);      \
    } else if (out16) {                                                        \
      edge_attn_fused_infer_kernel<VPT, true, __bf16, LPR, __bf16, float,      \
                                   LPH>                                        \
          <<<grid, block, 0, stream>>>(qkvs, (const float*)pifc_v,             \
                                       (const float*)prpc_v, ea, astride,      \
                                       row_ptr, csr_src, bn_scale, bn_shift,   \
                                       relu, (__bf16*)out_v, n, h, scale);     \
    } else {                                                                   \
      edge_attn_fused_infer_kernel<VPT, true, __bf16, LPR, float, float,       \
                                   LPH>                                        \
          <<<grid, block, 0, stream>>>(qkvs, (const float*)pifc_v,             \
                                       (const float*)prpc_v, ea, astride,      \
                                       row_ptr, csr_src, bn_scale, bn_shift,   \
                                       relu, (float*)out_v, n, h, scale);      \
    }                                                                          \
  } while (0)
#define INF16_H(VPT, LPR)                                                      \
  HEAD_CHAIN(INF16, VPT, LPR, vec_lph(h, heads, VPT, LPR), name)
  if (h == 256) {
    if (lpr == 16) INF16_H(16, 16);
    else if (lpr == 32) INF16_H(8, 32);
    else INF16_H(4, 64);
  } else if (h == 512) {
    if (lpr == 16 || lpr == 32) INF16_H(16, 32);
    else INF16_H(8, 64);
  } else if (h % 256 == 0 && h / PERTGNN_WAVE <= 32) {
    if (heads != 1) attn_heads_fail(name, h, heads, PERTGNN_WAVE);
    const int vpt = h / PERTGNN_WAVE;
    if (vpt == 4) INF16(4, 64, 64);
    else if (vpt == 8) INF16(8, 64, 64);
    else if (vpt == 16) INF16(16, 64, 64);
    else INF16(32, 64, 64);
  } else {
    pertgnn_shape_fail("edge_attn_fused infer act16 launcher", "h", h);
  }
#undef INF16_H
#undef INF16
}
```

csrc/hip/segops.hip:

```cpp
#include "common.h"
#include <cstdlib>


#define WAVES_PER_BLOCK 4

template <int VPT, typename TX = float>
__global__ void seg_pool_p1_kernel(const TX* __restrict__ x,
                                   const float* __restrict__ probs,
                                   const float* __restrict__ nn,
                                   const int* __restrict__ batch_ptr,
                                   float* __restrict__ partial, int b, int P,
                                   int h) {
  const int wid = threadIdx.x / PERTGNN_WAVE;
  const int lane = threadIdx.x % PERTGNN_WAVE;
  const int w = blockIdx.x * WAVES_PER_BLOCK + wid;
  if (w >= b * P) return;
  const int g = w / P;
  const int sub = w % P;
  float acc[VPT];
#pragma unroll
  for (int j = 0; j < VPT; ++j) acc[j] = 0.f;
  for (int i = batch_ptr[g] + sub; i < batch_ptr[g + 1]; i += P) {
    const float wt = probs[i] / nn[i];
#pragma unroll
// ... 1369 lines not shown
  }
}

template <typename TS, int U>
__global__ __launch_bounds__(256) void bn_stats_wide_kernel(
    const TS* __restrict__ x, long n, int h, float* __restrict__ out,
    int slab) {
  __shared__ float red[4096];
  const int lpr = h >> 3;
  const int slots = 256 / lpr;
  const int slot = threadIdx.x / lpr;
  const int c0 = (threadIdx.x - slot * lpr) * 8;
  const long rows_per_block = (n + gridDim.x - 1) / gridDim.x;
  const long r0 = (long)blockIdx.x * rows_per_block;
  const long r1 = min(n, r0 + rows_per_block);
  float s[8], q[8];
#pragma unroll
  for (int j = 0; j < 8; ++j) s[j] = q[j] = 0.f;
  long r = r0 + slot;
  for (; r + (long)(U - 1) * slots < r1; r += (long)U * slots) {
    float v[U][8];
#pragma unroll
    for (int u = 0; u < U; ++u) bn_ld8(&x[(r + (long)u * slots) * h + c0], v[u]);
#pragma unroll
    for (int u = 0; u < U; ++u)
#pragma unroll
      for (int j = 0; j < 8; ++j) {
        s[j] += v[u][j];
        q[j] += v[u][j] * v[u][j];
      }
  }
  for (; r < r1; r += slots) {
    float v[8];
    bn_ld8(&x[r * h + c0], v);
#pragma unroll
    for (int j = 0; j < 8; ++j) {
      s[j] += v[j];
      q[j] += v[j] * v[j];
    }
  }
  bn_wide_combine(red, s, q, slot, slots, c0, h, out, slab, r0 < r1);
}

template <typename TS, int MODE, int U>
__global__ __launch_bounds__(256) void bn_bwd_partial_wide_kernel(
    const TS* __restrict__ g, const TS* __restrict__ x,
    const void* __restrict__ ym, const float* __restrict__ mean,
    const float* __restrict__ invstd, long n, int h, float* __restrict__ out,
    int slab, float keep_inv) {
  __shared__ float red[4096];
  const TS* y = (const TS*)ym;
  const unsigned char* mask = (const unsigned char*)ym;
  const int lpr = h >> 3;
  const int slots = 256 / lpr;
  const int slot = threadIdx.x / lpr;
  const int lane = threadIdx.x - slot * lpr;
  const int c0 = lane * 8;
  const long rows_per_block = (n + gridDim.x - 1) / gridDim.x;
  const long r0 = (long)blockIdx.x * rows_per_block;
  const long r1 = min(n, r0 + rows_per_block);
  float s[8], q[8], m[8], is[8];
#pragma unroll
  for (int j = 0; j < 8; ++j) {
    s[j] = q[j] = 0.f;
    m[j] = mean[c0 + j];
    is[j] = invstd[c0 + j];
  }
  auto acc = [&](const float (&gv)[8], const float (&xv)[8],
                 const float (&yv)[8], unsigned bits) {
#pragma unroll
    for (int j = 0; j < 8; ++j) {
      bool dead = false;
      if (MODE == 1) dead = yv[j] <= 0.f;
      if (MODE == 2) dead = !((bits >> j) & 1u);
      const float gm = dead ? 0.f : gv[j] * keep_inv;
      s[j] += gm;
      q[j] += gm * (xv[j] - m[j]) * is[j];
    }
  };
  long r = r0 + slot;
  for (; r + (long)(U - 1) * slots < r1; r += (long)U * slots) {
    float gv[U][8], xv[U][8], yv[U][8];
    unsigned bits[U];
#pragma unroll
    for (int u = 0; u < U; ++u) {
      const long rr = r + (long)u * slots;
      bn_ld8(&g[rr * h + c0], gv[u]);
      bn_ld8(&x[rr * h + c0], xv[u]);
      if (MODE == 1) bn_ld8(&y[rr * h + c0], yv[u]);
      bits[u] = (MODE == 2) ? mask[rr * lpr + lane] : 0u;
    }
#pragma unroll
    for (int u = 0; u < U; ++u) acc(gv[u], xv[u], yv[u], bits[u]);
  }
  for (; r < r1; r += slots) {
    float gv[8], xv[8], yv[8];
    bn_ld8(&g[r * h + c0], gv);
    bn_ld8(&x[r * h + c0], xv);
    if (MODE == 1) bn_ld8(&y[r * h + c0], yv);
    const unsigned bits = (MODE == 2) ? mask[r * lpr + lane] : 0u;
    acc(gv, xv, yv, bits);
  }
  bn_wide_combine(red, s, q, slot, slots, c0, h, out, slab, r0 < r1);
}

__device__ __forceinline__ void bn_finalize_one(
    int c, float sum, float sumsq, float nf, float eps, float momentum,
    float* __restrict__ mean, float* __restrict__ invstd,
    float* __restrict__ running_mean, float* __restrict__ running_var) {
  const float m = sum / nf;
  const float var = fmaxf(sumsq / nf - m * m, 0.f);
  mean[c] = m;
  invstd[c] = rsqrtf(var + eps);
  const float unbiased = (nf > 1.f) ? var * nf / (nf - 1.f) : var;
  running_mean[c] = (1.f - momentum) * running_mean[c] + momentum * m;
  running_var[c] = (1.f - momentum) * running_var[c] + momentum * unbiased;
}

template <int EPI>
__global__ __launch_bounds__(256) void bn_slab_fold_kernel(
    const float* __restrict__ slab, int nb, int h,
    float* __restrict__ partials, long n, float eps, float momentum,
    float* __restrict__ o0, float* __restrict__ o1,
    float* __restrict__ running_mean, float* __restrict__ running_var) {
  __shared__ float red[16][16];
  __shared__ float tot[16];
  const int j = threadIdx.x & 15;
  const int sl = threadIdx.x >> 4;
  const int ch = blockIdx.x * 8 + (j & 7);
  const int col = (j >> 3) * h + ch;
  const int per = (nb + 15) / 16;
  const int b0 = sl * per;
  const int b1 = min(nb, b0 + per);
  float a = 0.f;
  if (ch < h) {
#pragma unroll 8
    for (int b = b0; b < b1; ++b) a += slab[(long)b * 2 * h + col];
  }
  red[sl][j] = a;
  __syncthreads();
  if (threadIdx.x < 16) {
    float t = 0.f;
#pragma unroll
    for (int k = 0; k < 16; ++k) t += red[k][threadIdx.x];
    tot[threadIdx.x] = t;
    if (ch < h) partials[col] = t;
  }
  if (EPI == 0) return;
  __syncthreads();
  if (threadIdx.x < 8 && ch < h) {
    if (EPI == 1) {
      bn_finalize_one(ch, tot[threadIdx.x], tot[8 + threadIdx.x], (float)n,
                      eps, momentum, o0, o1, running_mean, running_var);
    } else {
      o0[ch] = tot[8 + threadIdx.x];
      o1[ch] = tot[threadIdx.x];
    }
  }
}

template <typename TS>
static void bn_stats_wide_launch(const TS* x, long n, int h,
                                 float* partials, float* slab, bool finalize,
                                 float eps, float momentum, float* mean,
                                 float* invstd, float* running_mean,
                                 float* running_var, hipStream_t s) {
  const int nb = bn_wide_blocks(n);
  constexpr int U = 16 / sizeof(TS);
  if (slab) {
    bn_stats_wide_kernel<TS, U><<<nb, 256, 0, s>>>(x, n, h, slab, 1);
    if (finalize)
      bn_slab_fold_kernel<1><<<h / 8, 256, 0, s>>>(
          slab, nb, h, partials, n, eps, momentum, mean, invstd, running_mean,
          running_var);
    else
      bn_slab_fold_kernel<0><<<h / 8, 256, 0, s>>>(
          slab, nb, h, partials, n, 0.f, 0.f, nullptr, nullptr, nullptr,
          nullptr);
    return;
  }
  HIP_CHECK(hipMemsetAsync(partials, 0, 2 * h * sizeof(float), s));
  bn_stats_wide_kernel<TS, U><<<nb, 256, 0, s>>>(x, n, h, partials, 0);
  if (finalize)
    bn_finalize_kernel<<<ceil_div(h, 256), 256, 0, s>>>(
        partials, n, h, eps, momentum, mean, invstd, running_mean,
        running_var, 1);
}

template <typename TS>
static void bn_bwd_partials_wide_launch(
    const TS* g, const TS* x, const TS* y,
    const unsigned char* mask, const float* mean, const float* invstd, long n,
    int h, bool relu, float* partials, float* slab, float* dgamma,
    float* dbeta, float keep_inv, hipStream_t s) {
  const int nb = bn_wide_blocks(n);
  float* out = slab ? slab : partials;
  const int sl = slab ? 1 : 0;
  constexpr int U = 8 / sizeof(TS);
  if (!slab) HIP_CHECK(hipMemsetAsync(partials, 0, 2 * h * sizeof(float), s));
  if (!relu)
    bn_bwd_partial_wide_kernel<TS, 0, U><<<nb, 256, 0, s>>>(
        g, x, nullptr, mean, invstd, n, h, out, sl, keep_inv);
  else if (mask)
    bn_bwd_partial_wide_kernel<TS, 2, U><<<nb, 256, 0, s>>>(
        g, x, mask, mean, invstd, n, h, out, sl, keep_inv);
  else
    bn_bwd_partial_wide_kernel<TS, 1, U><<<nb, 256, 0, s>>>(
        g, x, y, mean, invstd, n, h, out, sl, keep_inv);
  if (slab) {
    if (dgamma)
      bn_slab_fold_kernel<2><<<h / 8, 256, 0, s>>>(
          slab, nb, h, partials, n, 0.f, 0.f, dgamma, dbeta, nullptr,
          nullptr);
    else
      bn_slab_fold_kernel<0><<<h / 8, 256, 0, s>>>(
          slab, nb, h, partials, n, 0.f, 0.f, nullptr, nullptr, nullptr,
          nullptr);
  } else if (dgamma) {
    bn_grad_affine_kernel<<<ceil_div(h, 256), 256, 0, s>>>(partials, dgamma,
                                                           dbeta, h);
  }
}

template <bool DROP>
__global__ __launch_bounds__(256) void bn_apply_mask_kernel(
    const __bf16* __restrict__ x, const float* __restrict__ mean,
    const float* __restrict__ invstd, const float* __restrict__ gamma,
    const float* __restrict__ beta, __bf16* __restrict__ y,
    unsigned char* __restrict__ mask, long n, int h, float dropout_p,
    const unsigned long long* __restrict__ seed_ptr) {
  const float keep_inv = DROP ? 1.f / (1.f - dropout_p) : 1.f;
  unsigned long long seed = 0ull;
  if constexpr (DROP) seed = seed_ptr ? *seed_ptr : 0ull;
  const long numo = n * (h >> 3);
  const long i0 = (long)blockIdx.x * blockDim.x + threadIdx.x;
  const long stride = (long)gridDim.x * blockDim.x;
  const int c = (int)((i0 * 8) % h);
  float mu[8], is[8], ga[8], be[8];
#pragma unroll
  for (int u = 0; u < 8; ++u) {
    mu[u] = mean[c + u];
    is[u] = invstd[c + u];
    ga[u] = gamma[c + u];
    be[u] = beta[c + u];
  }
  for (long o = i0; o < numo; o += stride) {
    const long t = o * 8;
    float xv[8];
    bn_ld8(&x[t], xv);
    __bf16 ov[8];
    unsigned bits = 0u;
#pragma unroll
    for (int u = 0; u < 8; ++u) {
      float v = (xv[u] - mu[u]) * is[u] * ga[u] + be[u];
      v = fmaxf(v, 0.f);
      if constexpr (DROP)
        v = (bn_rand01(seed, t + u) >= dropout_p) ? v * keep_inv : 0.f;
      ov[u] = (__bf16)v;
      if (!((float)ov[u] <= 0.f)) bits |= 1u << u;
    }
    bn_st8(&y[t], ov);
    mask[o] = (unsigned char)bits;
  }
}

template <int MODE>
__global__ __launch_bounds__(256) void bn_bwd_apply_wide_kernel(
    const __bf16* __restrict__ g, const __bf16* __restrict__ x,
    const void* __restrict__ ym, const float* __restrict__ mean,
    const float* __restrict__ invstd, const float* __restrict__ gamma,
    const float* __restrict__ partials, __bf16* __restrict__ dx, long n,
    long count, int h, const float* __restrict__ count_ptr, float keep_inv) {
  const float invn = 1.f / (count_ptr ? *count_ptr : (float)count);
  const long numo = n * (h >> 3);
  const long i0 = (long)blockIdx.x * blockDim.x + threadIdx.x;
  const long stride = (long)gridDim.x * blockDim.x;
  const int c = (int)((i0 * 8) % h);
  float mu[8], is[8], ga[8], p0[8], p1[8];
#pragma unroll
  for (int u = 0; u < 8; ++u) {
    mu[u] = mean[c + u];
    is[u] = invstd[c + u];
    ga[u] = gamma[c + u];
    p0[u] = partials[c + u];
    p1[u] = partials[h + c + u];
  }
  for (long o = i0; o < numo; o += stride) {
    const long t = o * 8;
    float gv[8], xv[8];
    bn_ld8(&g[t], gv);
    bn_ld8(&x[t], xv);
    unsigned bits = 0u;
    if (MODE == 2) {
      bits = ((const unsigned char*)ym)[o];
    } else {
      float yv[8];
      bn_ld8((const __bf16*)ym + t, yv);
#pragma unroll
      for (int u = 0; u < 8; ++u)
        if (!(yv[u] <= 0.f)) bits |= 1u << u;
    }
    __bf16 ov[8];
#pragma unroll
    for (int u = 0; u < 8; ++u) {
      float gm = gv[u] * keep_inv;
      if (!((bits >> u) & 1u)) gm = 0.f;
      const float xhat = (xv[u] - mu[u]) * is[u];
      ov[u] = (__bf16)(ga[u] * is[u] *
                       (gm - p0[u] * invn - xhat * p1[u] * invn));
    }
    bn_st8(&dx[t], ov);
  }
}

static void bn_apply_mask_launch(const __bf16* x, const float* mean,
                                 const float* invstd, const float* gamma,
                                 const float* beta, __bf16* y,
                                 unsigned char* mask, long n, int h,
                                 float dropout_p,
                                 const unsigned long long* seed_ptr,
                                 hipStream_t s) {
  const int grid = grid_for(n * (h / 8));
  if (dropout_p > 0.f)
    bn_apply_mask_kernel<true><<<grid, 256, 0, s>>>(
        x, mean, invstd, gamma, beta, y, mask, n, h, dropout_p, seed_ptr);
  else
    bn_apply_mask_kernel<false><<<grid, 256, 0, s>>>(
        x, mean, invstd, gamma, beta, y, mask, n, h, 0.f, nullptr);
}

__global__ void bn_eval_stats_kernel(const float* __restrict__ rm,
                                     const float* __restrict__ rv,
                                     float* __restrict__ mean,
                                     float* __restrict__ invstd, int h,
                                     float eps) {
  const int c = blockIdx.x * blockDim.x + threadIdx.x;
  if (c >= h) return;
  mean[c] = rm[c];
  invstd[c] = rsqrtf(rv[c] + eps);
}

void launch_bn_eval_stats(const float* running_mean, const float* running_var,
                          float* mean, float* invstd, int h, float eps,
                          hipStream_t s) {
  bn_eval_stats_kernel<<<ceil_div(h, 256), 256, 0, s>>>(running_mean,
                                                        running_var, mean,
                                                        invstd, h, eps);
}


void launch_bn_stats_only(const float* x, long n, int h, float* partials,
                          float* slab, hipStream_t s) {
  if (n == 0) {
    HIP_CHECK(hipMemsetAsync(partials, 0, 2 * h * sizeof(float), s));
    return;
  }
  if (bn_wide_ok(h)) {
    bn_stats_wide_launch(x, n, h, partials, slab, false, 0.f, 0.f, nullptr,
                         nullptr, nullptr, nullptr, s);
    return;
  }
  bn_stats_dispatch(x, n, h, partials, s);
}

void launch_bn_finalize_apply(const float* x, const float* partials,
                              const float* count_ptr, const float* gamma,
                              const float* beta, float* running_mean,
                              float* running_var, float* mean, float* invstd,
                              float* y, long n, int h, float momentum,
                              float eps, bool training, bool relu,
                              float dropout_p,
                              const unsigned long long* seed_ptr,
                              hipStream_t s) {
  if (training) {
    bn_finalize_kernel<<<ceil_div(h, 256), 256, 0, s>>>(
        partials, n, h, eps, momentum, mean, invstd, running_mean,
        running_var, 1, count_ptr);
  } else {
    bn_eval_stats_kernel<<<ceil_div(h, 256), 256, 0, s>>>(
        running_mean, running_var, mean, invstd, h, eps);
  }
  if (n > 0) {
    if (training && dropout_p > 0.f)
      bn_apply_kernel<float, float, true><<<grid_for(n * h), 256, 0, s>>>(
          x, mean, invstd, gamma, beta, y, n, h, relu ? 1 : 0, dropout_p,
          seed_ptr);
    else
      bn_apply_kernel<<<grid_for(n * h), 256, 0, s>>>(x, mean, invstd, gamma,
                                                      beta, y, n, h,
                                                      relu ? 1 : 0);
  }
}

void launch_bn_bwd_partials_only(const float* g, const float* x,
                                 const float* y, const float* mean,
                                 const float* invstd, long n, int h, bool relu,
                                 float* partials, float keep_inv,
                                 float* slab, hipStream_t s) {
  if (n == 0) {
    HIP_CHECK(hipMemsetAsync(partials, 0, 2 * h * sizeof(float), s));
    return;
  }
  if (bn_wide_ok(h)) {
    bn_bwd_partials_wide_launch(g, x, y, nullptr, mean, invstd, n, h, relu,
                                partials, slab, nullptr, nullptr, keep_inv, s);
    return;
  }
  bn_bwd_partials_dispatch(g, x, y, mean, invstd, n, h, relu, partials,
                           keep_inv, s);
}

void launch_bn_bwd_apply_only(const float* g, const float* x, const float* y,
                              const float* mean, const float* invstd,
                              const float* gamma, const float* partials,
                              const float* count_ptr, float* dx, long n, int h,
                              bool relu, float keep_inv, hipStream_t s) {
  if (n == 0) return;
  bn_bwd_apply_kernel<<<grid_for(n * h), 256, 0, s>>>(
      g, x, y, mean, invstd, gamma, partials, dx, n, n, h, relu ? 1 : 0,
      count_ptr, keep_inv);
}

void launch_bn_grad_affine(const float* partials, float* dgamma, float* dbeta,
                           int h, hipStream_t s) {
  bn_grad_affine_kernel<<<ceil_div(h, 256), 256, 0, s>>>(partials, dgamma,
                                                         dbeta, h);
}

void launch_bn_fwd(const float* x, const float* gamma, const float* beta,
                   float* running_mean, float* running_var, float* mean,
                   float* invstd, float* partials, float* y, long n, int h,
                   float momentum, float eps, bool training, bool relu,
                   float dropout_p, const unsigned long long* seed_ptr,
                   float* slab, hipStream_t s) {
  if (n == 0) return;
  if (training && bn_wide_ok(h)) {
    bn_stats_wide_launch(x, n, h, partials, slab, true, eps, momentum, mean,
                         invstd, running_mean, running_var, s);
  } else if (training) {
    bn_stats_dispatch(x, n, h, partials, s);
    bn_finalize_kernel<<<ceil_div(h, 256), 256, 0, s>>>(
        partials, n, h, eps, momentum, mean, invstd, running_mean, running_var,
        1);
  } else {
    launch_bn_eval_stats(running_mean, running_var, mean, invstd, h, eps, s);
  }
  if (training && dropout_p > 0.f)
    bn_apply_kernel<float, float, true><<<grid_for(n * h), 256, 0, s>>>(
        x, mean, invstd, gamma, beta, y, n, h, relu ? 1 : 0, dropout_p,
        seed_ptr);
  else
    bn_apply_kernel<<<grid_for(n * h), 256, 0, s>>>(x, mean, invstd, gamma,
                                                    beta, y, n, h,
                                                    relu ? 1 : 0);
}

void launch_counter_bump(unsigned long long* c, hipStream_t s) {
  counter_bump_kernel<<<1, 1, 0, s>>>(c);
}

void launch_bn_bwd(const float* g, const float* x, const float* y,
                   const float* mean, const float* invstd, const float* gamma,
                   float* partials, float* dx, float* dgamma, float* dbeta,
                   long n, int h, bool relu, float keep_inv, float* slab,
                   hipStream_t s) {
  if (n == 0) return;
  const bool wide = bn_wide_ok(h);
  if (wide)
    bn_bwd_partials_wide_launch(g, x, y, nullptr, mean, invstd, n, h, relu,
                                partials, slab, dgamma, dbeta, keep_inv, s);
  else
    bn_bwd_partials_dispatch(g, x, y, mean, invstd, n, h, relu, partials,
                             keep_inv, s);
  bn_bwd_apply_kernel<<<grid_for(n * h), 256, 0, s>>>(
      g, x, y, mean, invstd, gamma, partials, dx, n, n, h, relu ? 1 : 0,
      nullptr, keep_inv);
  if (wide) return;
  bn_grad_affine_kernel<<<ceil_div(h, 256), 256, 0, s>>>(partials, dgamma,
                                                         dbeta, h);
}


void launch_bn_stats_only16(const void* x, long n, int h, float* partials,
                            float* slab, hipStream_t s) {
  if (n == 0) {
    HIP_CHECK(hipMemsetAsync(partials, 0, 2 * h * sizeof(float), s));
    return;
  }
  if (bn_wide_ok(h)) {
    bn_stats_wide_launch((const __bf16*)x, n, h, partials, slab, false, 0.f,
                         0.f, nullptr, nullptr, nullptr, nullptr, s);
    return;
  }
  bn_stats_dispatch((const __bf16*)x, n, h, partials, s);
}

void launch_bn_fwd16(const void* x, const float* gamma, const float* beta,
                     float* running_mean, float* running_var, float* mean,
                     float* invstd, float* partials, void* y, long n, int h,
                     float momentum, float eps, bool training, bool relu,
                     float dropout_p, const unsigned long long* seed_ptr,
                     float* slab, unsigned char* mask, hipStream_t s) {
  if (n == 0) return;
  if (training && bn_wide_ok(h)) {
    bn_stats_wide_launch((const __bf16*)x, n, h, partials, slab, true, eps,
                         momentum, mean, invstd, running_mean, running_var, s);
  } else if (training) {
    bn_stats_dispatch((const __bf16*)x, n, h, partials, s);
    bn_finalize_kernel<<<ceil_div(h, 256), 256, 0, s>>>(
        partials, n, h, eps, momentum, mean, invstd, running_mean, running_var,
        1);
  } else {
    launch_bn_eval_stats(running_mean, running_var, mean, invstd, h, eps, s);
  }
  if (mask) {
    bn_apply_mask_launch((const __bf16*)x, mean, invstd, gamma, beta,
                         (__bf16*)y, mask, n, h, dropout_p, seed_ptr, s);
    return;
  }
  if (training && dropout_p > 0.f)
    bn_apply_kernel<__bf16, __bf16, true><<<grid_for(n * h), 256, 0, s>>>(
        (const __bf16*)x, mean, invstd, gamma, beta, (__bf16*)y, n, h,
        relu ? 1 : 0, dropout_p, seed_ptr);
  else
    bn_apply_kernel<<<grid_for(n * h), 256, 0, s>>>((const __bf16*)x, mean,
                                                    invstd, gamma, beta,
                                                    (__bf16*)y, n, h,
                                                    relu ? 1 : 0);
}

void launch_bn_finalize_apply16(const void* x, const float* partials,
                                const float* count_ptr, const float* gamma,
                                const float* beta, float* running_mean,
                                float* running_var, float* mean, float* invstd,
                                void* y, long n, int h, float momentum,
                                float eps, bool training, bool relu,
                                float dropout_p,
                                const unsigned long long* seed_ptr,
                                unsigned char* mask, hipStream_t s) {
  if (training) {
    bn_finalize_kernel<<<ceil_div(h, 256), 256, 0, s>>>(
        partials, n, h, eps, momentum, mean, invstd, running_mean,
        running_var, 1, count_ptr);
  } else {
    bn_eval_stats_kernel<<<ceil_div(h, 256), 256, 0, s>>>(
        running_mean, running_var, mean, invstd, h, eps);
  }
  if (n > 0 && mask) {
    bn_apply_mask_launch((const __bf16*)x, mean, invstd, gamma, beta,
                         (__bf16*)y, mask, n, h, dropout_p, seed_ptr, s);
  } else if (n > 0) {
    if (training && dropout_p > 0.f)
      bn_apply_kernel<__bf16, __bf16, true><<<grid_for(n * h), 256, 0, s>>>(
          (const __bf16*)x, mean, invstd, gamma, beta, (__bf16*)y, n, h,
          relu ? 1 : 0, dropout_p, seed_ptr);
    else
      bn_apply_kernel<<<grid_for(n * h), 256, 0, s>>>((const __bf16*)x, mean,
                                                      invstd, gamma, beta,
                                                      (__bf16*)y, n, h,
                                                      relu ? 1 : 0);
  }
}

void launch_bn_bwd_partials_only16(const void* g, const void* x,
                                   const void* y, const float* mean,
                                   const float* invstd, long n, int h,
                                   bool relu, float* partials, float keep_inv,
                                   float* slab, const unsigned char* mask,
                                   hipStream_t s) {
  if (n == 0) {
    HIP_CHECK(hipMemsetAsync(partials, 0, 2 * h * sizeof(float), s));
    return;
  }
  if (bn_wide_ok(h)) {
    bn_bwd_partials_wide_launch((const __bf16*)g, (const __bf16*)x,
                                (const __bf16*)y, mask, mean, invstd, n, h,
                                relu, partials, slab, nullptr, nullptr,
                                keep_inv, s);
    return;
  }
  bn_bwd_partials_dispatch((const __bf16*)g, (const __bf16*)x,
                           (const __bf16*)y, mean, invstd, n, h, relu,
                           partials, keep_inv, s);
}

void launch_bn_bwd_apply_only16(const void* g, const void* x, const void* y,
                                const float* mean, const float* invstd,
                                const float* gamma, const float* partials,
                                const float* count_ptr, void* dx, long n,
                                int h, bool relu, float keep_inv,
                                const unsigned char* mask, hipStream_t s) {
  if (n == 0) return;
  if (relu && bn_wide_ok(h)) {
    if (mask)
      bn_bwd_apply_wide_kernel<2><<<grid_for(n * (h / 8)), 256, 0, s>>>(
          (const __bf16*)g, (const __bf16*)x, mask, mean, invstd, gamma,
          partials, (__bf16*)dx, n, n, h, count_ptr, keep_inv);
    else
      bn_bwd_apply_wide_kernel<1><<<grid_for(n * (h / 8)), 256, 0, s>>>(
          (const __bf16*)g, (const __bf16*)x, y, mean, invstd, gamma,
          partials, (__bf16*)dx, n, n, h, count_ptr, keep_inv);
    return;
  }
  bn_bwd_apply_kernel<<<grid_for(n * h), 256, 0, s>>>(
      (const __bf16*)g, (const __bf16*)x, (const __bf16*)y, mean, invstd,
      gamma, partials, (__bf16*)dx, n, n, h, relu ? 1 : 0, count_ptr,
      keep_inv);
}

void launch_bn_bwd16(const void* g, const void* x, const void* y,
                     const float* mean, const float* invstd,
                     const float* gamma, float* partials, void* dx,
                     float* dgamma, float* dbeta, long n, int h, bool relu,
                     float keep_inv, float* slab, const unsigned char* mask,
                     hipStream_t s) {
  if (n == 0) return;
  const bool wide = bn_wide_ok(h);
  if (wide)
    bn_bwd_partials_wide_launch((const __bf16*)g, (const __bf16*)x,
                                (const __bf16*)y, mask, mean, invstd, n, h,
                                relu, partials, slab, dgamma, dbeta, keep_inv,
                                s);
  else
    bn_bwd_partials_dispatch((const __bf16*)g, (const __bf16*)x,
                             (const __bf16*)y, mean, invstd, n, h, relu,
                             partials, keep_inv, s);
  if (relu && wide && mask)
    bn_bwd_apply_wide_kernel<2><<<grid_for(n * (h / 8)), 256, 0, s>>>(
        (const __bf16*)g, (const __bf16*)x, mask, mean, invstd, gamma,
        partials, (__bf16*)dx, n, n, h, nullptr, keep_inv);
  else if (relu && wide)
    bn_bwd_apply_wide_kernel<1><<<grid_for(n * (h / 8)), 256, 0, s>>>(
        (const __bf16*)g, (const __bf16*)x, y, mean, invstd, gamma, partials,
        (__bf16*)dx, n, n, h, nullptr, keep_inv);
  else
    bn_bwd_apply_kernel<<<grid_for(n * h), 256, 0, s>>>(
        (const __bf16*)g, (const __bf16*)x, (const __bf16*)y, mean, invstd,
        gamma, partials, (__bf16*)dx, n, n, h, relu ? 1 : 0, nullptr,
        keep_inv);
  if (wide) return;
  bn_grad_affine_kernel<<<ceil_div(h, 256), 256, 0, s>>>(partials, dgamma,
                                                         dbeta, h);
}


__global__ void quantile_loss_fwd_kernel(const float* __restrict__ y,
                                         const float* __restrict__ y_hat,
                                         float* __restrict__ out, long b,
                                         float tau) {
  __shared__ float smem[256];
  float acc = 0.f;
  for (long i = (long)blockIdx.x * blockDim.x + threadIdx.x; i < b;
       i += (long)gridDim.x * blockDim.x) {
    const float e = y[i] - y_hat[i];
    acc += fmaxf(tau * e, (tau - 1.f) * e);
  }
  smem[threadIdx.x] = acc;
  __syncthreads();
  for (int off = blockDim.x / 2; off > 0; off >>= 1) {
    if (threadIdx.x < off) smem[threadIdx.x] += smem[threadIdx.x + off];
    __syncthreads();
  }
  if (threadIdx.x == 0) atomicAdd(out, smem[0] / b);
}

__global__ void quantile_loss_bwd_kernel(const float* __restrict__ g,
                                         const float* __restrict__ y,
                                         const float* __restrict__ y_hat,
                                         float* __restrict__ dy_hat, long b,
                                         float tau) {
  const float gs = g[0] / b;
  for (long i = (long)blockIdx.x * blockDim.x + threadIdx.x; i < b;
       i += (long)gridDim.x * blockDim.x) {
    const float e = y[i] - y_hat[i];
    float d;
    if (e > 0.f) d = -tau;
    else if (e < 0.f) d = 1.f - tau;
    else d = 0.5f * (-tau) + 0.5f * (1.f - tau);
    dy_hat[i] = gs * d;
  }
}

__global__ void eval_metrics_kernel(const float* __restrict__ y,
                                    const float* __restrict__ y_hat,
                                    float* __restrict__ out3, long b,
                                    float tau) {
  __shared__ float smem[3][256];
  float mae = 0.f, mape = 0.f, q = 0.f;
  for (long i = (long)blockIdx.x * blockDim.x + threadIdx.x; i < b;
       i += (long)gridDim.x * blockDim.x) {
    const float err = y_hat[i] - y[i];
    const float a = fabsf(err);
    mae += a;
    mape += a / y[i];
    const float e = -err;
    q += fmaxf(tau * e, (tau - 1.f) * e);
  }
  smem[0][threadIdx.x] = mae;
  smem[1][threadIdx.x] = mape;
  smem[2][threadIdx.x] = q;
  __syncthreads();
  for (int off = blockDim.x / 2; off > 0; off >>= 1) {
    if (threadIdx.x < off)
      for (int k = 0; k < 3; ++k)
        smem[k][threadIdx.x] += smem[k][threadIdx.x + off];
    __syncthreads();
  }
  if (threadIdx.x == 0)
    for (int k = 0; k < 3; ++k) atomicAdd(&out3[k], smem[k][0]);
}

void launch_quantile_loss_fwd(const float* y, const float* y_hat, float* out,
                              long b, float tau, hipStream_t s) {
  HIP_CHECK(hipMemsetAsync(out, 0, sizeof(float), s));
  quantile_loss_fwd_kernel<<<grid_for(b, 256, 256), 256, 0, s>>>(y, y_hat, out,
                                                                 b, tau);
}
void launch_quantile_loss_bwd(const float* g, const float* y,
                              const float* y_hat, float* dy_hat, long b,
                              float tau, hipStream_t s) {
  quantile_loss_bwd_kernel<<<grid_for(b), 256, 0, s>>>(g, y, y_hat, dy_hat, b,
                                                       tau);
}
void launch_eval_metrics(const float* y, const float* y_hat, float* out3,
                         long b, float tau, hipStream_t s) {
  HIP_CHECK(hipMemsetAsync(out3, 0, 3 * sizeof(float), s));
  eval_metrics_kernel<<<grid_for(b, 256, 256), 256, 0, s>>>(y, y_hat, out3, b,
                                                            tau);
}


__global__ void adam_tick_kernel(float* __restrict__ state, float b1,
                                 float b2,
                                 const float* __restrict__ sstate = nullptr) {
  if (sstate && sstate[2] != 0.f) return;
  const float t = state[0] + 1.f;
  state[0] = t;
  state[1] = 1.f - powf(b1, t);
  state[2] = 1.f - powf(b2, t);
}

__global__ void adam_kernel(float* __restrict__ p, const float* __restrict__ g,
                            float* __restrict__ m, float* __restrict__ v,
                            const float* __restrict__ state, long numel,
                            float lr, float b1, float b2, float eps,
                            float gscale,
                            const float* __restrict__ sstate = nullptr) {
  if (sstate && sstate[2] != 0.f) return;
  const long i0 = (long)blockIdx.x * blockDim.x + threadIdx.x;
  const long stride = (long)gridDim.x * blockDim.x;
  const float step_size = lr / state[1];
  const float sqrt_bias2 = sqrtf(state[2]);
  const float gs = sstate ? 1.f / sstate[0] : gscale;
  for (long t = i0; t < numel; t += stride) {
    const float gt = g[t] * gs;
    const float mt = b1 * m[t] + (1.f - b1) * gt;
    const float vt = b2 * v[t] + (1.f - b2) * gt * gt;
    m[t] = mt;
    v[t] = vt;
    const float denom = sqrtf(vt) / sqrt_bias2 + eps;
    p[t] -= step_size * mt / denom;
  }
}

__global__ void scaler_begin_kernel(float* __restrict__ sstate) {
  sstate[2] = 0.f;
}

__global__ void grad_scan_kernel(const float* __restrict__ g, long numel,
                                 float* __restrict__ sstate) {
  const long i0 = (long)blockIdx.x * blockDim.x + threadIdx.x;
  const long stride = (long)gridDim.x * blockDim.x;
  float bad = 0.f;
  for (long t = i0; t < numel; t += stride) {
    const float x = g[t];
    if (!isfinite(x)) { bad = 1.f; break; }
  }
  if (bad != 0.f) sstate[2] = 1.f;
}

__global__ void scaler_update_kernel(float* __restrict__ sstate, float backoff,
                                     float growth, float interval) {
  if (sstate[2] != 0.f) {
    sstate[0] = fmaxf(sstate[0] * backoff, 1.f);
    sstate[1] = 0.f;
  } else {
    sstate[1] += 1.f;
    if (sstate[1] >= interval) {
      sstate[0] = fminf(sstate[0] * growth, 4294967296.f);
      sstate[1] = 0.f;
    }
  }
}

void launch_adam(float* p, const float* g, float* m, float* v, float* state,
                 long numel, float lr, float b1, float b2, float eps, float gscale,
                 hipStream_t s) {
  if (numel == 0) return;
  adam_tick_kernel<<<1, 1, 0, s>>>(state, b1, b2, nullptr);
  adam_kernel<<<grid_for(numel), 256, 0, s>>>(p, g, m, v, state, numel, lr,
                                              b1, b2, eps, gscale, nullptr);
}

void launch_adam_dynamic(float* p, const float* g, float* m, float* v,
                         float* state, float* sstate, long numel, float lr,
                         float b1, float b2, float eps, float backoff,
                         float growth, float interval, hipStream_t s) {
  if (numel == 0) return;
  scaler_begin_kernel<<<1, 1, 0, s>>>(sstate);
  grad_scan_kernel<<<grid_for(numel), 256, 0, s>>>(g, numel, sstate);
  adam_tick_kernel<<<1, 1, 0, s>>>(state, b1, b2, sstate);
  adam_kernel<<<grid_for(numel), 256, 0, s>>>(p, g, m, v, state, numel, lr,
                                              b1, b2, eps, 1.f, sstate);
  scaler_update_kernel<<<1, 1, 0, s>>>(sstate, backoff, growth, interval);
}
```

pertgnn/models/pert_gnn.py:

```python
from __future__ import annotations

import torch
import torch.nn.functional as F
from torch import nn

from ..ops import functional as ops


class _EdgeLinearView:

    def __init__(self, conv):
        object.__setattr__(self, "_conv", conv)

    @property
    def weight(self):
        c = self._conv
        return torch.cat([c.we_ifc, c.we_rpc], dim=1)

    bias = None


class _SegLinearView:

    def __init__(self, conv, seg, has_bias=True):
        object.__setattr__(self, "_conv", conv)
        object.__setattr__(self, "_seg", seg)
        object.__setattr__(self, "_has_bias", has_bias)

    @property
    def weight(self):
        c = self._conv
        h = c.out_channels
        return c.w4[self._seg * h:(self._seg + 1) * h, :c.in_channels]

    @property
    def bias(self):
        if not self._has_bias:
            return None
        c = self._conv
        h = c.out_channels
        return c.b4[self._seg * h:(self._seg + 1) * h]


class TransformerConv(nn.Module):

    def __init__(self, in_channels: int, out_channels: int, heads: int = 1, edge_dim: int | None = None):
        super().__init__()
        if not isinstance(heads, int) or heads < 1 or out_channels % heads != 0:
            raise ValueError(
                f"heads={heads!r} must be a positive integer that divides "
                f"out_channels={out_channels}")
        self.in_channels = in_channels
        self.out_channels = out_channels
        self.heads = heads
        self.edge_dim = edge_dim
        k32 = (in_channels + 31) // 32 * 32
        k128 = (in_channels + 127) // 128 * 128
        self.k_padded = k128 if k128 <= 1.35 * k32 else k32
        self.w4 = nn.Parameter(torch.zeros(4 * out_channels, self.k_padded))
        self.b4 = nn.Parameter(torch.zeros(4 * out_channels))
        self.lin_query = _SegLinearView(self, 0)
        self.lin_key = _SegLinearView(self, 1)
        self.lin_value = _SegLinearView(self, 2)
        self.lin_skip = _SegLinearView(self, 3)
        assert edge_dim == 2 * out_channels
        self.we_ifc = nn.Parameter(torch.empty(out_channels, out_channels))
        self.we_rpc = nn.Parameter(torch.empty(out_channels, out_channels))
        self.lin_edge = _EdgeLinearView(self)
        self.reset_parameters()

    def reset_parameters(self):
        with torch.no_grad():
            self.w4.zero_()
            self.b4.zero_()
        for lin in (self.lin_key, self.lin_query, self.lin_value, self.lin_skip):
            nn.init.xavier_uniform_(lin.weight)
            if lin.bias is not None:
                nn.init.zeros_(lin.bias)
        h = self.out_channels
        w = torch.empty(h, 2 * h)
        nn.init.xavier_uniform_(w)
        with torch.no_grad():
            self.we_ifc.copy_(w[:, :h])
            self.we_rpc.copy_(w[:, h:])

    _SEG_NAMES = ("lin_query", "lin_key", "lin_value", "lin_skip")

    def _save_to_state_dict(self, destination, prefix, keep_vars):
        super()._save_to_state_dict(destination, prefix, keep_vars)
        del destination[prefix + "w4"]
        del destination[prefix + "b4"]
        del destination[prefix + "we_ifc"]
        del destination[prefix + "we_rpc"]
        for i, name in enumerate(self._SEG_NAMES):
            view = getattr(self, name)
            w = view.weight
            b = view.bias
            destination[prefix + name + ".weight"] = w if keep_vars else w.detach().clone()
            destination[prefix + name + ".bias"] = b if keep_vars else b.detach().clone()
        we = self.lin_edge.weight
        destination[prefix + "lin_edge.weight"] = we if keep_vars else we.detach()

    def _load_from_state_dict(self, state_dict, prefix, local_metadata, strict,
                              missing_keys, unexpected_keys, error_msgs):
        h = self.out_channels
        with torch.no_grad():
            for i, name in enumerate(self._SEG_NAMES):
                wk, bk = prefix + name + ".weight", prefix + name + ".bias"
                if wk in state_dict:
                    self.w4[i * h:(i + 1) * h, :self.in_channels].copy_(state_dict[wk])
                    self.w4[i * h:(i + 1) * h, self.in_channels:].zero_()
                    state_dict = {k: v for k, v in state_dict.items() if k != wk}
                else:
                    missing_keys.append(wk)
                if bk in state_dict:
                    self.b4[i * h:(i + 1) * h].copy_(state_dict[bk])
                    state_dict = {k: v for k, v in state_dict.items() if k != bk}
                else:
                    missing_keys.append(bk)
        we_key = prefix + "lin_edge.weight"
        if we_key in state_dict:
            with torch.no_grad():
                w = state_dict[we_key]
                self.we_ifc.copy_(w[:, :h])
                self.we_rpc.copy_(w[:, h:])
        else:
            missing_keys.append(we_key)
        filtered = {k: v for k, v in state_dict.items()
                    if k != we_key
                    and not any(k == prefix + n + s for n in self._SEG_NAMES
                                for s in (".weight", ".bias"))}
        super()._load_from_state_dict(filtered, prefix, local_metadata, strict,
                                      missing_keys, unexpected_keys, error_msgs)
        for k in (prefix + "w4", prefix + "b4", prefix + "we_ifc",
                  prefix + "we_rpc"):
            if k in missing_keys:
                missing_keys.remove(k)

    def forward(self, x, edge_index, edge_embeds, csr=None, num_nodes=None):
        n = x.shape[0] if num_nodes is None else num_nodes
        q = ops.linear(x, self.lin_query.weight.contiguous(), self.lin_query.bias)
        k = ops.linear(x, self.lin_key.weight.contiguous(), self.lin_key.bias)
        v = ops.linear(x, self.lin_value.weight.contiguous(), self.lin_value.bias)
        e = ops.linear(edge_embeds, self.lin_edge.weight, None)
        skip = ops.linear(x, self.lin_skip.weight.contiguous(), self.lin_skip.bias)
        return ops.edge_attention(q, k, v, e, skip, edge_index, n, csr=csr,
                                  heads=self.heads)

    def forward_fused(self, x, edge_attr, ifc_weight, rpc_weight, csr,
                      out16=False, pifc=None, prpc=None):
        h = self.out_channels
        if x.shape[1] != self.k_padded:
            x = torch.nn.functional.pad(x, (0, self.k_padded - x.shape[1]))
        act16 = (ops.gemm_precision() in ("bf16", "fp16") and h % 256 == 0
                 and ops.act16_enabled())
        if act16:
            qkvs = ops.linear16(x, self.w4, self.b4)
            if pifc is not None and prpc is not None:
                pass
            elif ops.p16_enabled():
                pifc = ops.linear16(ifc_weight, self.we_ifc)
                prpc = ops.linear16(rpc_weight, self.we_rpc)
            else:
                pifc = ops.linear(ifc_weight, self.we_ifc, None)
                prpc = ops.linear(rpc_weight, self.we_rpc, None)
        else:
            qkvs = ops.linear(x, self.w4, self.b4)
            pifc = ops.linear(ifc_weight, self.we_ifc, None)
            prpc = ops.linear(rpc_weight, self.we_rpc, None)
        return ops.edge_attention_fused(qkvs, pifc, prpc, edge_attr, csr,
                                        out16=out16, heads=self.heads)


class SAGEDeterministic(nn.Module):

    def __init__(
        self,
        in_channels,
        cat_dims,
        entry_id_max,
        interface_id_max,
        rpctype_id_max,
        hidden_channels,
        num_layers,
        dropout,
        *,
        heads=1,
    ):
        super().__init__()
        self.heads = heads
        self.convs = nn.ModuleList()
        self.convs.append(
            TransformerConv(
                in_channels=in_channels + hidden_channels,
                out_channels=hidden_channels,
                heads=heads,
                edge_dim=hidden_channels * 2,
            )
        )
        self.bns = nn.ModuleList()
        self.bns.append(nn.BatchNorm1d(hidden_channels))
        for _ in range(num_layers - 2):
            self.convs.append(
                TransformerConv(
                    in_channels=hidden_channels,
                    out_channels=hidden_channels,
                    heads=heads,
                    edge_dim=hidden_channels * 2,
                )
            )
            self.bns.append(nn.BatchNorm1d(hidden_channels))
        self.convs.append(
            TransformerConv(
                in_channels=hidden_channels,
                out_channels=hidden_channels,
                heads=heads,
                edge_dim=hidden_channels * 2,
            )
        )
        self.local_linear = nn.Linear(hidden_channels, 1)
        self.global_linear1 = nn.Linear(hidden_channels * 2, hidden_channels)
        self.global_linear2 = nn.Linear(hidden_channels, 1)
        self.cat_embedding = nn.ModuleList()
        for num_categories in cat_dims:
            self.cat_embedding.append(nn.Embedding(num_categories, hidden_channels))

        self.dropout = dropout
        self.entry_embeds = nn.Embedding(entry_id_max + 1, hidden_channels)
        self.interface_embeds = nn.Embedding(interface_id_max + 1, hidden_channels)
        self.rpctype_embeds = nn.Embedding(rpctype_id_max + 1, hidden_channels)
        self.edge_linear = nn.LazyLinear(hidden_channels * 2)
        self._bn_comm = None

    def enable_sync_bn(self, comm):
        self._bn_comm = comm

    def reset_parameters(self):
        for conv in self.convs:
            conv.reset_parameters()
        for bn in self.bns:
            bn.reset_parameters()

    def forward(
        self,
        x,
        cat_X,
        edge_index,
        edge_attr,
        pattern_num_nodes,
        pattern_probs,
        entry_id,
        batch,
        csr=None,
        num_graphs=None,
    ):
        if num_graphs is None:
            num_graphs = int(batch.max().item()) + 1 if batch.numel() else 0
        from ..ops.backend import use_hip

        fused = csr is not None and use_hip(x)
        hidden = self.bns[0].weight.shape[0] if len(self.bns) else 0
        out16 = (fused and ops.gemm_precision() in ("bf16", "fp16")
                 and hidden % 256 == 0 and ops.act16_enabled())
        x = ops.embed_concat_node(x, cat_X,
                                  [t.weight for t in self.cat_embedding],
                                  out16=out16)
        edge_embeds = None
        if not fused:
            edge_embeds = ops.embed_concat_edge(
                edge_attr, self.interface_embeds.weight, self.rpctype_embeds.weight
            )
        n = x.shape[0]

        ptables = {}
        if out16 and ops.p16_enabled() and ops.ptable_group_enabled():
            pifcs, prpcs = ops.ptables_grouped(
                self.interface_embeds.weight, self.rpctype_embeds.weight,
                [c.we_ifc for c in self.convs], [c.we_rpc for c in self.convs])
            ptables = {id(c): pair
                       for c, pair in zip(self.convs, zip(pifcs, prpcs))}

        def run_conv(conv, x, out16=False):
            if fused:
                pifc, prpc = ptables.get(id(conv), (None, None))
                return conv.forward_fused(
                    x, edge_attr, self.interface_embeds.weight,
                    self.rpctype_embeds.weight, csr, out16=out16,
                    pifc=pifc, prpc=prpc,
                )
            return conv(x, edge_index, edge_embeds, csr=csr, num_nodes=n)

        for i, conv in enumerate(self.convs[:-1]):
            x = run_conv(conv, x, out16=out16)
            bn = self.bns[i]
            x = ops.batchnorm_relu(
                x, bn.weight, bn.bias, bn.running_mean, bn.running_var,
                bn.momentum, bn.eps, self.training, fuse_relu=True,
                comm=self._bn_comm, out16=out16, dropout_p=self.dropout,
            )
            if self.training and bn.track_running_stats and bn.num_batches_tracked is not None:
                bn.num_batches_tracked += 1
        x = run_conv(self.convs[-1], x)
        local_predict = ops.linear(x, self.local_linear.weight, self.local_linear.bias)
        mean_x = ops.pattern_pool(x, pattern_probs, pattern_num_nodes, batch, num_graphs)
        entry_vec = ops.embedding(entry_id, self.entry_embeds.weight)
        global_predict = torch.cat([mean_x, entry_vec], dim=1)
        h = ops.linear(global_predict, self.global_linear1.weight, self.global_linear1.bias)
        global_predict = ops.linear(F.relu(h), self.global_linear2.weight, self.global_linear2.bias)
        return global_predict, local_predict
```

pertgnn/ops/functional.py:

```python
from __future__ import annotations

from typing import NamedTuple

import torch

from . import reference as ref
from .backend import ext, use_hip


def deterministic() -> bool:
    import os
    return os.environ.get("PERTGNN_DETERMINISTIC", "0") == "1"


def _table_grad(m, g, idx, rows, h, col_off):
    if rows * h * 4 <= 160 * 1024 and not deterministic():
        if g.dtype == torch.bfloat16 and (
                h % 64 != 0 or 4 * rows * 64 * 4 > 160 * 1024):
            g = g.float()
        return m.vocab_scatter(g, idx, rows, h, col_off)
    order, ptr, row_map, wave_start, row_map2, wave_start2 = _group_by(idx, rows)
    if g.dtype not in (torch.float32, torch.bfloat16):
        g = g.float()
    return m.embed_grouped_scatter_bal(g, order, ptr, row_map, wave_start,
# ... 67 lines not shown

class EdgeTablePlan(NamedTuple):
    idx1: torch.Tensor
    lptr1: torch.Tensor
    idx2: torch.Tensor
    lptr2: torch.Tensor
    idx3: torch.Tensor
    lptr3: torch.Tensor
    n1: int
    n2: int
    V: int
    R: int
    C: int

    def tensors(self):
        return (self.idx1, self.lptr1, self.idx2, self.lptr2, self.idx3,
                self.lptr3)


def _chunk_segments(counts: torch.Tensor, c: int):
    total = int(counts.sum())
    cps = (counts + c - 1) // c
    n_chunks = int(cps.sum())
    seg = torch.repeat_interleave(torch.arange(counts.numel()), cps)
    first = cps.cumsum(0) - cps
    seg_start = counts.cumsum(0) - counts
    start = seg_start[seg] + (torch.arange(n_chunks) - first[seg]) * c
    return seg, torch.cat([start, torch.tensor([total])])


def _build_edge_table_plan(ifc, rpc, V: int, R: int, C: int):
    E = ifc.numel()
    if E and (int(ifc.min()) < 0 or int(ifc.max()) >= V
              or int(rpc.min()) < 0 or int(rpc.max()) >= R):
        raise IndexError("edge_attr index outside the P tables")
    key = ifc * R + rpc
    order = torch.argsort(key, stable=True)
    ukeys, runs = torch.unique_consecutive(key[order], return_counts=True)
    run_of_chunk, lptr1 = _chunk_segments(runs, C)
    ck = ukeys[run_of_chunk]
    n1 = ck.numel()
    members = torch.cat([torch.arange(n1),
                         torch.argsort(ck % R, stable=True)])
    cnt = torch.cat([torch.bincount(ck // R, minlength=V),
                     torch.bincount(ck % R, minlength=R)])
    out_of_member = torch.repeat_interleave(torch.arange(V + R), cnt)
    big = cnt > C
    in_big = big[out_of_member]
    idx2 = members[in_big]
    _, lptr2 = _chunk_segments(cnt[big], C)
    n2 = lptr2.numel() - 1
    len3 = torch.where(big, (cnt + C - 1) // C, cnt)
    lptr3 = torch.cat([torch.zeros(1, dtype=torch.long), len3.cumsum(0)])
    from_l2 = big[torch.repeat_interleave(torch.arange(V + R), len3)]
    idx3 = torch.empty(int(len3.sum()), dtype=torch.long)
    idx3[from_l2] = n1 + torch.arange(n2)
    idx3[~from_l2] = members[~in_big]
    assert order.numel() == E and int(lptr1[-1]) == E
    assert int(lptr2[-1]) == idx2.numel() and int(lptr3[-1]) == idx3.numel()
    assert idx2.numel() == 0 or int(idx2.max()) < n1
    assert idx3.numel() == 0 or int(idx3.max()) < n1 + n2
    assert max(E, n1 + n2, idx3.numel(), idx2.numel()) < 2 ** 31
    i32 = lambda t: t.to(torch.int32)
    return EdgeTablePlan(i32(order), i32(lptr1), i32(idx2), i32(lptr2),
                         i32(idx3), i32(lptr3), n1, n2, V, R, C)


def edge_table_plan(edge_attr: torch.Tensor, V: int, R: int,
                    C: int | None = None) -> EdgeTablePlan:
    if C is None:
        C = _scatter_iters()
    key = ("edge_table", edge_attr.data_ptr(), edge_attr.numel(),
           tuple(edge_attr.stride()), V, R, C)
    hit = _GROUP_CACHE.get(key)
    if hit is not None:
        _GROUP_CACHE.move_to_end(key)
        return hit[1]
    ea = edge_attr[:, :2].cpu().long()
    plan = _build_edge_table_plan(ea[:, 0].contiguous(), ea[:, 1].contiguous(),
                                  V, R, C)
    dev = edge_attr.device
    plan = plan._replace(**{f: getattr(plan, f).to(dev) for f in
                            ("idx1", "lptr1", "idx2", "lptr2", "idx3",
                             "lptr3")})
    nbytes = sum(t.numel() for t in plan.tensors()) * 4
    while _GROUP_CACHE and _GROUP_CACHE_BYTES[0] + nbytes > _GROUP_CACHE_CAP:
        _, old = _GROUP_CACHE.popitem(last=False)
        _GROUP_CACHE_BYTES[0] -= old[-1]
    _GROUP_CACHE[key] = (edge_attr, plan, nbytes)
    _GROUP_CACHE_BYTES[0] += nbytes
    return plan


def apply_plan_reference(plan: EdgeTablePlan, de: torch.Tensor):
    acc = torch.float64 if de.dtype == torch.float64 else torch.float32
    h = de.shape[1]

    def level(src, idx, lptr):
        lens = (lptr[1:] - lptr[:-1]).long()
        seg = torch.repeat_interleave(
            torch.arange(lens.numel(), device=src.device), lens)
        out = torch.zeros(lens.numel(), h, dtype=acc, device=src.device)
        return out.index_add_(0, seg, src.index_select(0, idx.long()))

    p1 = level(de.to(acc), plan.idx1, plan.lptr1)
    p2 = level(p1, plan.idx2, plan.lptr2)
    out = level(torch.cat([p1, p2]), plan.idx3, plan.lptr3)
    return out[:plan.V], out[plan.V:]


def _edge_table_grads(m, de, pifc, prpc, edge_attr):
    V, R, h = pifc.shape[0], prpc.shape[0], de.shape[1]
    if h in (256, 512) and (V * h * 4 > 160 * 1024 or deterministic()):
        if de.dtype not in (torch.float32, torch.bfloat16):
            de = de.float()
        plan = edge_table_plan(edge_attr, V, R)
        od = pifc.dtype if pifc.dtype == torch.bfloat16 else torch.float32
        out = m.edge_table_grad(de, *plan.tensors(), V, R, od).to(pifc.dtype)
        return out[:V], out[V:]
    dpifc = _table_grad(m, de, edge_attr[:, 0], V, h, 0)
    dprpc = _table_grad(m, de, edge_attr[:, 1], R, h, 0)
    if dpifc.dtype != pifc.dtype:
        dpifc = dpifc.to(pifc.dtype)
        dprpc = dprpc.to(prpc.dtype)
    return dpifc, dprpc



class _EdgeAttentionFn(torch.autograd.Function):
    @staticmethod
    def forward(ctx, q, k, v, e, skip, row_ptr, csr_src, col_ptr, csc_dst, csc_eid):
        m = ext()
        out, alpha = m.edge_attn_fwd(q, k, v, e, row_ptr, csr_src, skip)
        ctx.save_for_backward(q, k, v, e, alpha, row_ptr, csr_src, col_ptr, csc_dst, csc_eid)
        return out

    @staticmethod
    def backward(ctx, g):
        q, k, v, e, alpha, row_ptr, csr_src, col_ptr, csc_dst, csc_eid = ctx.saved_tensors
        m = ext()
        dq, dk, dv, de = m.edge_attn_bwd(
            g.contiguous(), q, k, v, e, alpha, row_ptr, csr_src, col_ptr, csc_dst, csc_eid
        )
        return dq, dk, dv, de, g, None, None, None, None, None


def _device_csr(edge_index, num_nodes):
    dev = edge_index.device
    src, dst = edge_index[0], edge_index[1]
    perm = torch.argsort(dst, stable=True)
    src_s = src.index_select(0, perm)
    dst_s = dst.index_select(0, perm)
    row_ptr = torch.zeros(num_nodes + 1, dtype=torch.int32, device=dev)
    row_ptr[1:] = torch.bincount(dst_s, minlength=num_nodes).cumsum(0).to(torch.int32)
    perm2 = torch.argsort(src_s, stable=True)
    col_ptr = torch.zeros(num_nodes + 1, dtype=torch.int32, device=dev)
    col_ptr[1:] = torch.bincount(src_s, minlength=num_nodes).cumsum(0).to(torch.int32)
    csr = (row_ptr, src_s.to(torch.int32), col_ptr,
           dst_s.index_select(0, perm2).to(torch.int32), perm2.to(torch.int32))
    return perm, csr


def edge_attention(q, k, v, e, skip, edge_index, num_nodes, csr=None,
                   heads=1):
    if use_hip(q):
        if csr is None:
            perm, csr = _device_csr(edge_index, num_nodes)
            e = e.index_select(0, perm)
        row_ptr, csr_src, col_ptr, csc_dst, csc_eid = csr
        if heads == 1:
            return _EdgeAttentionFn.apply(q, k, v, e, skip, row_ptr, csr_src, col_ptr, csc_dst, csc_eid)
        h = q.shape[1]
        if heads < 1 or h % heads != 0:
            raise ValueError(f"heads={heads} does not divide H={h}")
        c = h // heads
        outs = [
            _EdgeAttentionFn.apply(
                *(t[:, i * c:(i + 1) * c].contiguous()
                  for t in (q, k, v, e, skip)),
                row_ptr, csr_src, col_ptr, csc_dst, csc_eid)
            for i in range(heads)
        ]
        return torch.cat(outs, dim=1)
    return ref.edge_attention(q, k, v, e, edge_index, num_nodes, skip,
                              heads=heads)


class _Linear16Fn(torch.autograd.Function):

    @staticmethod
    def forward(ctx, x, w, b):
        m = ext()
        bb = b if b is not None else torch.empty(0, dtype=torch.float32, device=x.device)
        fp16c = gemm_precision() == "fp16"
        if x.dtype == torch.bfloat16:
            y = m.linear_fwd_a16o16(x, w, bb, fp16c)
        else:
            y = m.linear_fwd_bf16_o16(x, w, bb)
        ctx.save_for_backward(x, w)
        ctx.has_bias = b is not None
        ctx.fp16c = fp16c
        return y

    @staticmethod
    def backward(ctx, g):
        x, w = ctx.saved_tensors
        m = ext()
        g = g.contiguous()
        if x.dtype == torch.bfloat16:
            dx = m.linear_dgrad16_o16(g, w, ctx.fp16c)
            dw, db = m.linear_wgrad16_b16(g, x, ctx.has_bias, ctx.fp16c)
        else:
            dx = m.linear_dgrad16(g, w)
            dw, db = m.linear_wgrad16(g, x, ctx.has_bias)
        return dx, dw, (db if ctx.has_bias else None)


def linear16(x, w, b=None):
    return _Linear16Fn.apply(x, w, b)


class _PTablesFn(torch.autograd.Function):

    @staticmethod
    def forward(ctx, ifc_table, rpc_table, *weights):
        layers = len(weights) // 2
        we_ifc, we_rpc = list(weights[:layers]), list(weights[layers:])
        ctx.set_materialize_grads(False)
        ctx.save_for_backward(ifc_table, rpc_table, *weights)
        return tuple(ext().ptables_fwd(ifc_table, rpc_table, we_ifc, we_rpc))

    @staticmethod
    def backward(ctx, *dps):
        ifc_table, rpc_table, *weights = ctx.saved_tensors
        layers = len(weights) // 2
        none = torch.empty(0, dtype=torch.bfloat16, device=ifc_table.device)
        d_ifc, d_rpc, dw = ext().ptables_bwd(
            [none if g is None else g.contiguous() for g in dps],
            ifc_table, rpc_table, weights[:layers], weights[layers:],
            ptable_dgrad_splits())
        return (d_ifc, d_rpc,
                *(None if g is None else dw[i] for i, g in enumerate(dps)))


def ptables_grouped(ifc_table, rpc_table, we_ifc, we_rpc):
    if len(we_ifc) != len(we_rpc):
        raise ValueError(f"{len(we_ifc)} we_ifc vs {len(we_rpc)} we_rpc")
    layers = len(we_ifc)
    out = _PTablesFn.apply(ifc_table, rpc_table, *we_ifc, *we_rpc)
    return list(out[:layers]), list(out[layers:])


def ptable_group_enabled() -> bool:
    import os
    return os.environ.get("PERTGNN_NO_PTABLE_GROUP", "0") != "1"


def ptable_dgrad_splits() -> int:
    import os
    return int(os.environ.get("PERTGNN_PTABLE_DGRAD_SPLIT", "4"))


_ACT16 = None
_P16 = None


def p16_enabled() -> bool:
    global _P16
    if _P16 is None:
        import os
        _P16 = os.environ.get("PERTGNN_NO_P16", "0") != "1"
    return _P16


def act16_enabled() -> bool:
    global _ACT16
    if _ACT16 is None:
        import os
        _ACT16 = os.environ.get("PERTGNN_NO_ACT16", "0") != "1"
    return _ACT16



class _EdgeAttentionFusedFn(torch.autograd.Function):
    @staticmethod
    def forward(ctx, qkvs, pifc, prpc, edge_attr, row_ptr, csr_src, col_ptr,
                csc_dst, csc_eid, out16=False, heads=1):
        m = ext()
        out, alpha = m.edge_attn_fused_fwd(qkvs, pifc, prpc, edge_attr, row_ptr, csr_src, out16, heads)
        ctx.save_for_backward(qkvs, pifc, prpc, edge_attr, alpha,
                              row_ptr, csr_src, col_ptr, csc_dst, csc_eid)
        ctx.heads = heads
        return out

    @staticmethod
    def backward(ctx, g):
        (qkvs, pifc, prpc, edge_attr, alpha, row_ptr, csr_src, col_ptr,
         csc_dst, csc_eid) = ctx.saved_tensors
        m = ext()
        dqkvs, de = m.edge_attn_fused_bwd(
            g.contiguous(), qkvs, pifc, prpc, edge_attr, alpha,
            row_ptr, csr_src, col_ptr, csc_dst, csc_eid, ctx.heads,
        )
        if not _overlap_enabled():
            h = de.shape[1]
            if (h % 256 == 0 and not deterministic()
                    and (pifc.shape[0] + prpc.shape[0]) * h * 4 <= 160 * 1024):
                dpifc, dprpc = m.vocab_scatter_dual(de, edge_attr, pifc.shape[0], prpc.shape[0])
                if dpifc.dtype != pifc.dtype:
                    dpifc = dpifc.to(pifc.dtype)
                    dprpc = dprpc.to(prpc.dtype)
            else:
                dpifc, dprpc = _edge_table_grads(m, de, pifc, prpc, edge_attr)
            return dqkvs, dpifc, dprpc, None, None, None, None, None, None, None, None
        cur = torch.cuda.current_stream()
        side = _side_stream()
        ev = torch.cuda.Event()
        ev.record(cur)
        side.wait_event(ev)
        with torch.cuda.stream(side):
            dpifc, dprpc = _edge_table_grads(m, de, pifc, prpc, edge_attr)
        ev2 = torch.cuda.Event()
        ev2.record(side)
        cur.wait_event(ev2)
        _mark_cross_stream(dpifc, cur)
        _mark_cross_stream(dprpc, cur)
        return dqkvs, dpifc, dprpc, None, None, None, None, None, None, None, None


def _fused_eager(qkvs, pifc, prpc, edge_attr, csr, heads):
    row_ptr, csr_src = csr[0], csr[1]
    n = qkvs.shape[0]
    h = qkvs.shape[1] // 4
    q, k, v, skip = qkvs.float().split(h, dim=1)
    e = (pifc.float().index_select(0, edge_attr[:, 0])
         + prpc.float().index_select(0, edge_attr[:, 1]))
    deg = (row_ptr[1:] - row_ptr[:-1]).long()
    dst = torch.repeat_interleave(
        torch.arange(n, dtype=torch.long, device=qkvs.device), deg)
    edge_index = torch.stack([csr_src.long(), dst])
    return ref.edge_attention(q, k, v, e, edge_index, n, skip, heads=heads)


def edge_attention_fused(qkvs, pifc, prpc, edge_attr, csr, out16=False,
                         heads=1):
    if not use_hip(qkvs):
        out = _fused_eager(qkvs, pifc, prpc, edge_attr, csr, heads)
        return out.to(torch.bfloat16) if out16 else out
    row_ptr, csr_src, col_ptr, csc_dst, csc_eid = csr
    return _EdgeAttentionFusedFn.apply(
        qkvs, pifc, prpc, edge_attr, row_ptr, csr_src, col_ptr, csc_dst,
        csc_eid, out16, heads
    )


def edge_attention_fused_infer(qkvs, pifc, prpc, edge_attr, csr,
                               bn_scale=None, bn_shift=None, relu=False,
                               out16=False, heads=1):
    if (bn_scale is None) != (bn_shift is None):
        raise ValueError("bn_scale and bn_shift must be given together")
    if torch.is_grad_enabled() and any(
            t is not None and t.requires_grad
            for t in (qkvs, pifc, prpc, bn_scale, bn_shift)):
        raise RuntimeError(
            "edge_attention_fused_infer is forward-only (no backward); call "
            "it under torch.no_grad() or use edge_attention_fused")
    if not use_hip(qkvs):
        return ref.edge_attention_fused_infer(
            qkvs, pifc, prpc, edge_attr, csr, bn_scale, bn_shift, relu, out16,
            heads)
    if bn_scale is None:
        bn_scale = bn_shift = torch.empty(0, dtype=torch.float32,
                                          device=qkvs.device)
    return ext().edge_attn_fused_infer(qkvs, pifc, prpc, edge_attr, csr[0],
                                       csr[1], bn_scale, bn_shift, bool(relu),
                                       bool(out16), int(heads))



class _PatternPoolFn(torch.autograd.Function):
    @staticmethod
    def forward(ctx, x, probs, nnodes, batch, num_graphs):
        m = ext()
        counts = torch.zeros(num_graphs, dtype=torch.long, device=x.device)
        counts.scatter_add_(0, batch, torch.ones_like(batch))
        batch_ptr = torch.zeros(num_graphs + 1, dtype=torch.int32, device=x.device)
        batch_ptr[1:] = torch.cumsum(counts, 0).to(torch.int32)
        out = m.seg_pool_fwd(x, probs.contiguous(), nnodes.contiguous(), batch_ptr, num_graphs)
        ctx.save_for_backward(probs, nnodes, batch)
        return out

    @staticmethod
    def backward(ctx, g):
        probs, nnodes, batch = ctx.saved_tensors
        m = ext()
        dx = m.seg_pool_bwd(g.contiguous(), probs, nnodes, batch)
        return dx, None, None, None, None


def pattern_pool(x, pattern_probs, pattern_num_nodes, batch, num_graphs):
    if use_hip(x):
        return _PatternPoolFn.apply(x, pattern_probs, pattern_num_nodes, batch, num_graphs)
    return ref.pattern_pool(x, pattern_probs, pattern_num_nodes, batch, num_graphs)



class _EmbedNodeFn(torch.autograd.Function):
    @staticmethod
    def forward(ctx, x_raw, cat_idx, table, out16=False):
        m = ext()
        out = m.embed_node_fwd(x_raw, cat_idx, table, out16)
        ctx.save_for_backward(cat_idx)
        ctx.f = x_raw.shape[1]
        ctx.rows = table.shape[0]
        return out

    @staticmethod
    def backward(ctx, g):
        (cat_idx,) = ctx.saved_tensors
        m = ext()
        g = g.contiguous()
        dx_raw = g[:, : ctx.f].contiguous()
        if dx_raw.dtype != torch.float32:
            dx_raw = dx_raw.float()
        h = g.shape[1] - ctx.f
        dtable = _table_grad(m, g, cat_idx, ctx.rows, h, ctx.f)
        return dx_raw, None, dtable, None


class _EmbedEdgeFn(torch.autograd.Function):
    @staticmethod
    def forward(ctx, edge_attr, ifc_table, rpc_table):
        m = ext()
        out = m.embed_edge_fwd(edge_attr, ifc_table, rpc_table)
        ctx.save_for_backward(edge_attr)
        ctx.rows = (ifc_table.shape[0], rpc_table.shape[0])
        return out

    @staticmethod
    def backward(ctx, g):
        (edge_attr,) = ctx.saved_tensors
        m = ext()
        g = g.contiguous()
        h = g.shape[1] // 2
        d_ifc = _table_grad(m, g, edge_attr[:, 0], ctx.rows[0], h, 0)
        d_rpc = _table_grad(m, g, edge_attr[:, 1], ctx.rows[1], h, h)
        return None, d_ifc, d_rpc


def embed_concat_node(x_raw, cat_X, tables, out16=False):
    if len(tables) == 1 and use_hip(x_raw):
        return _EmbedNodeFn.apply(x_raw, cat_X[:, 0].contiguous(), tables[0], out16)
    return ref.embed_concat_node(x_raw, cat_X, tables)


def embed_concat_edge(edge_attr, interface_table, rpctype_table):
    if use_hip(interface_table):
        return _EmbedEdgeFn.apply(edge_attr, interface_table, rpctype_table)
    return ref.embed_concat_edge(edge_attr, interface_table, rpctype_table)



class _EmbeddingFn(torch.autograd.Function):
    @staticmethod
    def forward(ctx, idx, table):
        m = ext()
        out = m.gather_rows(idx, table)
        ctx.save_for_backward(idx)
        ctx.rows = table.shape[0]
        return out

    @staticmethod
    def backward(ctx, g):
        (idx,) = ctx.saved_tensors
        m = ext()
        g = g.contiguous()
        return None, _table_grad(m, g, idx, ctx.rows, g.shape[1], 0)


def embedding(idx, table):
    if use_hip(table):
        return _EmbeddingFn.apply(idx.contiguous(), table)
    return table.index_select(0, idx)



_RNG_COUNTER = {}


def _rng_counter(device):
    key = str(device)
    t = _RNG_COUNTER.get(key)
    if t is None:
        t = torch.randint(0, 2 ** 62, (1,), dtype=torch.int64, device=device)
        _RNG_COUNTER[key] = t
    return t


class _BNReLUFn(torch.autograd.Function):
    @staticmethod
    def forward(ctx, x, gamma, beta, running_mean, running_var, momentum, eps,
                training, fuse_relu, comm, out16=False, dropout_p=0.0):
        m = ext()
        sync = comm is not None and getattr(comm, "distributed", False) and training
        drop = float(dropout_p) if training else 0.0
        if drop > 0.0:
            assert fuse_relu, "fused dropout rides the ReLU mask (model.py:102-103)"
        seed = _rng_counter(x.device) if drop > 0.0 else torch.empty(
            0, dtype=torch.int64, device=x.device)
        if sync:
            partials = m.bn_stats(x)
            comm.all_reduce_(partials)
            fin = (m.bn_finalize_apply16 if x.dtype == torch.bfloat16
                   else m.bn_finalize_apply)
            out = fin(
                x, partials, gamma, beta, running_mean, running_var,
                momentum, eps, training, fuse_relu, drop, seed)
        else:
            fwd = (m.bn_relu_fwd16 if x.dtype == torch.bfloat16
                   else m.bn_relu_fwd)
            out = fwd(
                x, gamma, beta, running_mean, running_var, momentum, eps,
                training, fuse_relu, drop, seed
            )
        y, save_mean, save_invstd = out[:3]
        mask = out[3] if len(out) > 3 and out[3].numel() > 0 else None
        ctx.save_for_backward(x, gamma, save_mean, save_invstd,
                              y if mask is None else mask)
        ctx.y16 = y.dtype == torch.bfloat16
        ctx.fuse_relu = fuse_relu
        ctx.comm = comm if sync else None
        ctx.keep_inv = 1.0 / (1.0 - drop) if drop > 0.0 else 1.0
        return y

    @staticmethod
    def backward(ctx, g):
        x, gamma, save_mean, save_invstd, y = ctx.saved_tensors
        m = ext()
        g = g.contiguous()
        y16 = ctx.y16
        if ctx.comm is not None:
            bwd_partials = m.bn_bwd_partials16 if y16 else m.bn_bwd_partials
            bwd_apply = m.bn_bwd_apply16 if y16 else m.bn_bwd_apply
            partials_local = bwd_partials(g, x, y, save_mean, save_invstd,
                                          ctx.fuse_relu, ctx.keep_inv)
            partials_global = partials_local.clone()
            ctx.comm.all_reduce_(partials_global)
            dx, dgamma, dbeta = bwd_apply(
                g, x, y, save_mean, save_invstd, gamma,
                partials_global, partials_local, ctx.fuse_relu, ctx.keep_inv)
        else:
            bwd = m.bn_relu_bwd16 if y16 else m.bn_relu_bwd
            dx, dgamma, dbeta = bwd(
                g, x, gamma, save_mean, save_invstd, y, ctx.fuse_relu,
                ctx.keep_inv
            )
        return (dx, dgamma, dbeta, None, None, None, None, None, None, None,
                None, None)


class _EagerSyncBNFn(torch.autograd.Function):

    @staticmethod
    def forward(ctx, x, gamma, beta, running_mean, running_var, momentum, eps,
                fuse_relu, comm):
        with torch.no_grad():
            n_local = x.shape[0]
            h = x.shape[1]
            pack = torch.cat([x.sum(0), (x * x).sum(0),
                              torch.tensor([float(n_local)], dtype=x.dtype, device=x.device)])
            comm.all_reduce_(pack)
            count = float(pack[-1])
            mean = pack[:h] / count
            var = (pack[h:2 * h] / count - mean * mean).clamp_min(0)
            invstd = (var + eps).rsqrt()
            unbiased = var * (count / max(count - 1.0, 1.0))
            running_mean.mul_(1 - momentum).add_(mean, alpha=momentum)
            running_var.mul_(1 - momentum).add_(unbiased, alpha=momentum)
            y = (x - mean) * invstd * gamma + beta
            if fuse_relu:
                y = torch.nn.functional.relu(y)
        ctx.save_for_backward(x, gamma, mean, invstd, y)
        ctx.fuse_relu = fuse_relu
        ctx.comm = comm
        ctx.count = count
        return y

    @staticmethod
    def backward(ctx, g):
        x, gamma, mean, invstd, y = ctx.saved_tensors
        gm = g.clone()
        if ctx.fuse_relu:
            gm[y <= 0] = 0
        xhat = (x - mean) * invstd
        s1_local = gm.sum(0)
        s2_local = (gm * xhat).sum(0)
        pack = torch.cat([s1_local, s2_local])
        ctx.comm.all_reduce_(pack)
        h = x.shape[1]
        s1_g = pack[:h] / ctx.count
        s2_g = pack[h:] / ctx.count
        dx = gamma * invstd * (gm - s1_g - xhat * s2_g)
        return dx, s2_local, s1_local, None, None, None, None, None, None


def _eager_sync_batchnorm(x, gamma, beta, running_mean, running_var, momentum,
                          eps, fuse_relu, comm):
    return _EagerSyncBNFn.apply(x, gamma, beta, running_mean, running_var,
                                momentum, eps, fuse_relu, comm)


def batchnorm_relu(x, gamma, beta, running_mean, running_var, momentum, eps,
                   training, fuse_relu=True, comm=None, out16=False,
                   dropout_p=0.0):
    if use_hip(x):
        return _BNReLUFn.apply(x, gamma, beta, running_mean, running_var,
                               momentum, eps, training, fuse_relu, comm,
                               out16, dropout_p)
    if comm is not None and getattr(comm, "distributed", False) and training:
        y = _eager_sync_batchnorm(x, gamma, beta, running_mean, running_var,
                                  momentum, eps, fuse_relu, comm)
    else:
        y = torch.nn.functional.batch_norm(
            x, running_mean, running_var, gamma, beta, training, momentum, eps
        )
        if fuse_relu:
            y = torch.nn.functional.relu(y)
    if dropout_p > 0.0:
        y = torch.nn.functional.dropout(y, p=dropout_p, training=training)
    return y



class _QuantileLossFn(torch.autograd.Function):
    @staticmethod
    def forward(ctx, y, y_hat, tau):
        m = ext()
        loss = m.quantile_loss_fwd(y, y_hat, tau)
        ctx.save_for_backward(y, y_hat)
        ctx.tau = tau
        return loss

    @staticmethod
    def backward(ctx, g):
        y, y_hat = ctx.saved_tensors
        m = ext()
        dy_hat = m.quantile_loss_bwd(g, y, y_hat, ctx.tau)
        return None, dy_hat, None


def quantile_loss(y, y_hat, tau):
    if use_hip(y_hat):
        return _QuantileLossFn.apply(y, y_hat, tau)
    return ref.quantile_loss(y, y_hat, tau)


def eval_metrics(y, y_hat, tau):
    if use_hip(y_hat):
        return ext().eval_metrics(y, y_hat, tau)
    return ref.eval_metrics(y, y_hat, tau)



_GEMM_PRECISION = "fp32"
_SIDE_STREAM = None
_OVERLAP = None


def _overlap_enabled() -> bool:
    global _OVERLAP
    if _OVERLAP is None:
        import os
        _OVERLAP = os.environ.get("PERTGNN_SIDE_STREAM", "0") == "1"
    return _OVERLAP


def _side_stream():
    global _SIDE_STREAM
    if _SIDE_STREAM is None:
        _SIDE_STREAM = torch.cuda.Stream()
    return _SIDE_STREAM


def _mark_cross_stream(t, consumer_stream):
    if not torch.cuda.is_current_stream_capturing():
        t.record_stream(consumer_stream)


def set_gemm_precision(prec: str):
    global _GEMM_PRECISION
    assert prec in ("fp32", "bf16", "fp16"), prec
    _GEMM_PRECISION = prec


def gemm_precision() -> str:
    return _GEMM_PRECISION


class _LinearFn(torch.autograd.Function):
    @staticmethod
    def forward(ctx, x, w, b):
        m = ext()
        prec = _GEMM_PRECISION
        bb = b if b is not None else torch.empty(0, dtype=x.dtype, device=x.device)
        if prec == "bf16":
            y = m.linear_fwd_bf16(x, w, bb)
        elif prec == "fp16":
            y = m.linear_fwd_fp16(x, w, bb)
        else:
            y = m.linear_fwd(x, w, bb)
        ctx.save_for_backward(x, w)
        ctx.has_bias = b is not None
        ctx.prec = prec
        return y

    @staticmethod
    def backward(ctx, g):
        x, w = ctx.saved_tensors
        m = ext()
        g = g.contiguous()
        prec = {"fp32": 0, "bf16": 1, "fp16": 2}[ctx.prec]
        if not _overlap_enabled():
            dw, db = m.linear_wgrad(g, x, ctx.has_bias, prec)
            dx = m.linear_dgrad(g, w, prec)
            return dx, dw, (db if ctx.has_bias else None)
        cur = torch.cuda.current_stream()
        side = _side_stream()
        ev = torch.cuda.Event()
        ev.record(cur)
        side.wait_event(ev)
        with torch.cuda.stream(side):
            dw, db = m.linear_wgrad(g, x, ctx.has_bias, prec)
        dx = m.linear_dgrad(g, w, prec)
        ev2 = torch.cuda.Event()
        ev2.record(side)
        cur.wait_event(ev2)
        _mark_cross_stream(dw, cur)
        if ctx.has_bias:
            _mark_cross_stream(db, cur)
        return dx, dw, (db if ctx.has_bias else None)


def linear(x, w, b=None):
    if use_hip(x) and hasattr(ext(), "linear_fwd"):
        return _LinearFn.apply(x, w, b)
    return torch.nn.functional.linear(x, w, b)


__all__ = [
    "set_gemm_precision",
    "p16_enabled",
    "gemm_precision",
    "linear16",
    "ptables_grouped",
    "ptable_group_enabled",
    "act16_enabled",
    "edge_attention",
    "edge_attention_fused",
    "edge_attention_fused_infer",
    "embedding",
    "pattern_pool",
    "embed_concat_node",
    "embed_concat_edge",
    "batchnorm_relu",
    "quantile_loss",
    "eval_metrics",
    "linear",
]
```

Before: 106,800 graphs/s.

## Fuse BatchNorm/ReLU/dropout backward into fused edge-attention backward kernels

After: 108,900 graphs/s, median of 6. 1.02x the previous value.

```diff
diff --git a/csrc/bindings.cpp b/csrc/bindings.cpp
--- a/csrc/bindings.cpp
+++ b/csrc/bindings.cpp
@@ -2,8 +2,11 @@
 #include <torch/extension.h>
 
 #include <cstdlib>
+#include <optional>
 
 #include <c10/cuda/CUDAStream.h>
+
+#include "hip/attn_bn.h"
 
 namespace {
 
@@ -166,7 +169,11 @@
                                   int, const float*, const int*, const int*,
                                   const int*, const int*, const int*, void*,
                                   void*, float*, int, int, long, int,
-                                  hipStream_t);
+                                  hipStream_t, const AttnBnBwd* = nullptr);
+void launch_bn_bwd_partials_affine16(const void*, const void*,
+                                     const unsigned char*, const float*,
+                                     const float*, long, int, float*, float,
+                                     float*, float*, float*, hipStream_t);
 void launch_edge_attn_fused_infer(const float*, const float*, const float*,
                                   const long*, int, const int*, const int*,
                                   const float*, const float*, int, float*,
@@ -1240,6 +1247,99 @@
                         dgamma.data_ptr<float>(), dbeta.data_ptr<float>(), h,
                         cur_stream());
   return {dx, dgamma, dbeta};
+}
+
+std::vector<torch::Tensor> edge_attn_bn_bwd16(
+    torch::Tensor g, torch::Tensor x, torch::Tensor mask, torch::Tensor gamma,
+    torch::Tensor mean, torch::Tensor invstd, double keep_inv,
+    torch::Tensor qkvs, torch::Tensor pifc, torch::Tensor prpc,
+    torch::Tensor ea, torch::Tensor alpha, torch::Tensor row_ptr,
+    torch::Tensor csr_src, torch::Tensor col_ptr, torch::Tensor csc_dst,
+    torch::Tensor csc_eid, int64_t heads = 1,
+    std::optional<torch::Tensor> partials_global_opt = std::nullopt,
+    std::optional<torch::Tensor> partials_local_opt = std::nullopt) {
+  CHECK_IN(g); CHECK_IN(x); CHECK_IN(qkvs); CHECK_IN(alpha); CHECK_IN(mask);
+  CHECK_IN(gamma); CHECK_IN(mean); CHECK_IN(invstd);
+  const int n = qkvs.size(0);
+  const int h = qkvs.size(1) / 4;
+  const long ne = ea.size(0);
+  TORCH_CHECK(n > 0, "edge_attn_bn_bwd16 needs at least one node");
+  TORCH_CHECK(h == 256 || h == 512, "edge_attn_bn_bwd16 covers H = 256, 512");
+  TORCH_CHECK(qkvs.scalar_type() == torch::kBFloat16 &&
+                  g.scalar_type() == torch::kBFloat16 &&
+                  x.scalar_type() == torch::kBFloat16,
+              "edge_attn_bn_bwd16 takes bf16 qkvs, g and x");
+  TORCH_CHECK(x.dim() == 2 && x.size(0) == n && x.size(1) == h &&
+                  g.sizes() == x.sizes(),
+              "g and x must be [n, h]");
+  TORCH_CHECK(mask.scalar_type() == torch::kUInt8,
+              "edge_attn_bn_bwd16 needs the BN forward's keep mask");
+  TORCH_CHECK(gamma.numel() == h && mean.numel() == h && invstd.numel() == h &&
+                  gamma.scalar_type() == torch::kFloat32 &&
+                  mean.scalar_type() == torch::kFloat32 &&
+                  invstd.scalar_type() == torch::kFloat32,
+              "gamma/mean/invstd must be fp32 [h]");
+  TORCH_CHECK(heads >= 1 && heads <= h && h % heads == 0,
+              "heads must divide H (H=", h, ", heads=", heads, ")");
+  TORCH_CHECK(alpha.scalar_type() == torch::kFloat32 &&
+                  alpha.numel() == ne * heads,
+              "alpha must be the fp32 [E, heads] tensor of the forward");
+  TORCH_CHECK(pifc.scalar_type() == prpc.scalar_type(),
+              "P tables must share a dtype");
+  const bool sync = partials_global_opt.has_value();
+  TORCH_CHECK(sync == partials_local_opt.has_value(),
+              "partials_global and partials_local come together");
+  torch::Tensor partials_global, partials_local;
+  if (sync) {
+    partials_global = *partials_global_opt;
+    partials_local = *partials_local_opt;
+  }
+  auto fopt = qkvs.options().dtype(torch::kFloat32);
+  auto dgamma = torch::empty({h}, fopt);
+  auto dbeta = torch::empty({h}, fopt);
+  AttnBnBwd bn{};
+  bn.x = x.data_ptr();
+  bn.mask = bn_mask_ptr(mask, x);
+  bn.mean = mean.data_ptr<float>();
+  bn.invstd = invstd.data_ptr<float>();
+  bn.gamma = gamma.data_ptr<float>();
+  bn.count = n;
+  bn.keep_inv = (float)keep_inv;
+  torch::Tensor partials, slab;
+  if (sync) {
+    CHECK_IN(partials_global); CHECK_IN(partials_local);
+    TORCH_CHECK(partials_global.numel() == 2 * h + 1 &&
+                    partials_local.numel() >= 2 * h &&
+                    partials_global.scalar_type() == torch::kFloat32 &&
+                    partials_local.scalar_type() == torch::kFloat32,
+                "edge_attn_bn_bwd16 expects fp32 [2h+1] partials with the "
+                "global count in the tail slot");
+    bn.partials = partials_global.data_ptr<float>();
+    bn.count_ptr = partials_global.data_ptr<float>() + 2 * h;
+    launch_bn_grad_affine(partials_local.data_ptr<float>(),
+                          dgamma.data_ptr<float>(), dbeta.data_ptr<float>(), h,
+                          cur_stream());
+  } else {
+    partials = torch::empty({2 * h}, fopt);
+    slab = bn_wide_slab(x);
+    launch_bn_bwd_partials_affine16(
+        g.data_ptr(), x.data_ptr(), bn.mask, bn.mean, bn.invstd, n, h,
+        partials.data_ptr<float>(), bn.keep_inv, bn_slab_ptr(slab),
+        dgamma.data_ptr<float>(), dbeta.data_ptr<float>(), cur_stream());
+    bn.partials = partials.data_ptr<float>();
+  }
+  auto dqkvs = torch::empty_like(qkvs);
+  auto de = torch::empty({ne, h}, qkvs.options());
+  auto dal = torch::empty({ne * heads}, fopt);
+  const int p16 = pifc.scalar_type() == torch::kBFloat16 ? 1 : 0;
+  launch_edge_attn_fused_bwd16(
+      g.data_ptr(), 1, qkvs.data_ptr(), pifc.data_ptr(), prpc.data_ptr(), p16,
+      ea.data_ptr<long>(), (int)ea.size(1), alpha.data_ptr<float>(),
+      row_ptr.data_ptr<int>(), csr_src.data_ptr<int>(),
+      col_ptr.data_ptr<int>(), csc_dst.data_ptr<int>(),
+      csc_eid.data_ptr<int>(), dqkvs.data_ptr(), de.data_ptr(),
+      dal.data_ptr<float>(), n, h, ne, (int)heads, cur_stream(), &bn);
+  return {dqkvs, de, dgamma, dbeta};
 }
 
 torch::Tensor seg_pool_fwd16(torch::Tensor x, torch::Tensor probs,
@@ -1601,6 +1701,14 @@
           py::arg("y"), py::arg("mean"), py::arg("invstd"), py::arg("gamma"),
           py::arg("partials_global"), py::arg("partials_local"),
           py::arg("relu"), py::arg("keep_inv") = 1.0);
+  mod.def("edge_attn_bn_bwd16", &edge_attn_bn_bwd16, py::arg("g"),
+          py::arg("x"), py::arg("mask"), py::arg("gamma"), py::arg("mean"),
+          py::arg("invstd"), py::arg("keep_inv"), py::arg("qkvs"),
+          py::arg("pifc"), py::arg("prpc"), py::arg("edge_attr"),
+          py::arg("alpha"), py::arg("row_ptr"), py::arg("csr_src"),
+          py::arg("col_ptr"), py::arg("csc_dst"), py::arg("csc_eid"),
+          py::arg("heads") = 1, py::arg("partials_global") = py::none(),
+          py::arg("partials_local") = py::none());
   mod.def("seg_pool_fwd16", &seg_pool_fwd16);
   mod.def("seg_pool_bwd16", &seg_pool_bwd16);
   mod.def("linear_fwd_a16o16", &linear_fwd_a16o16, py::arg("x"), py::arg("w"),
diff --git a/csrc/hip/attn_bn.h b/csrc/hip/attn_bn.h
--- /dev/null
+++ b/csrc/hip/attn_bn.h
@@ -0,0 +1,13 @@
+#pragma once
+
+struct AttnBnBwd {
+  const void* x;
+  const unsigned char* mask;
+  const float* mean;
+  const float* invstd;
+  const float* gamma;
+  const float* partials;
+  const float* count_ptr;
+  long count;
+  float keep_inv;
+};
diff --git a/csrc/hip/common.h b/csrc/hip/common.h
--- a/csrc/hip/common.h
+++ b/csrc/hip/common.h
@@ -43,6 +43,17 @@
   return v;
 }
 
+__device__ __forceinline__ __bf16 bn_bwd_dx16(float g, float x, bool keep,
+                                              float mu, float is, float ga,
+                                              float p0, float p1, float invn,
+                                              float keep_inv) {
+#pragma clang fp contract(off)
+  const float gm = keep ? g * keep_inv : 0.f;
+  const float xhat = (x - mu) * is;
+  return (__bf16)((ga * is) *
+                  __builtin_fmaf(-invn, xhat * p1, gm - p0 * invn));
+}
+
 static inline int ceil_div(long a, long b) { return (int)((a + b - 1) / b); }
 
 __device__ __forceinline__ int xcd_swizzle(int bid, int nwg) {
diff --git a/csrc/hip/edge_attn_fused.hip b/csrc/hip/edge_attn_fused.hip
--- a/csrc/hip/edge_attn_fused.hip
+++ b/csrc/hip/edge_attn_fused.hip
@@ -1,7 +1,9 @@
 
 #include "common.h"
+#include "attn_bn.h"
 #include <cmath>
 #include <cstdlib>
+#include <type_traits>
 
 #define WAVES_PER_BLOCK 4
 
@@ -358,6 +360,35 @@
   S::store(&out[(long)row * h], lane, h, res);
 }
 
+template <int VPT>
+__device__ __forceinline__ void attn_bn_bwd_row(const AttnBnBwd& bn, int row,
+                                                int lane, int h,
+                                                float (&gr)[VPT]) {
+  using S = Slice<VPT, true>;
+  static_assert(VPT == 4 || VPT % 8 == 0, "a lane's channels fill mask bytes");
+  constexpr int NB = (VPT + 7) / 8;
+  const float invn =
+      1.f / (bn.count_ptr ? *bn.count_ptr : (float)bn.count);
+  const int c0 = lane * VPT;
+  const unsigned char* mrow = bn.mask + (long)row * (h >> 3) + (c0 >> 3);
+  unsigned bits[NB];
+#pragma unroll
+  for (int b = 0; b < NB; ++b) bits[b] = mrow[b];
+  float xr[VPT], mu[VPT], is[VPT], ga[VPT], p0[VPT], p1[VPT];
+  S::load(&((const __bf16*)bn.x)[(long)row * h], lane, h, xr);
+  S::load(bn.mean, lane, h, mu);
+  S::load(bn.invstd, lane, h, is);
+  S::load(bn.gamma, lane, h, ga);
+  S::load(bn.partials, lane, h, p0);
+  S::load(bn.partials + h, lane, h, p1);
+#pragma unroll
+  for (int j = 0; j < VPT; ++j) {
+    const bool keep = (bits[j >> 3] >> ((c0 & 7) + (j & 7))) & 1u;
+    gr[j] = (float)bn_bwd_dx16(gr[j], xr[j], keep, mu[j], is[j], ga[j], p0[j],
+                               p1[j], invn, bn.keep_inv);
+  }
+}
+
 template <int VPT, bool VEC, typename QT = float,
           int LPR = PERTGNN_WAVE, typename TG = float, typename PT = float,
           int LPH = LPR, bool PCH = false>
@@ -367,7 +398,7 @@
     const long* __restrict__ ea, int astride, const float* __restrict__ alpha,
     const int* __restrict__ row_ptr, const int* __restrict__ csr_src,
     QT* __restrict__ dqkvs, float* __restrict__ dal, int n, int h,
-    float scale) {
+    float scale, AttnBnBwd bn = AttnBnBwd{}) {
   using S = Slice<VPT, VEC>;
   static_assert(VEC || LPR == PERTGNN_WAVE, "sub-wave rows need VEC layout");
   static_assert(PCH ? !VEC : (VEC || LPH == LPR),
@@ -384,6 +415,9 @@
 
   float gr[VPT], a1[VPT], a2[VPT];
   S::load(&g[(long)row * h], lane, h, gr);
+  if constexpr (VEC && std::is_same<TG, __bf16>::value && VPT <= 16) {
+    if (bn.x) attn_bn_bwd_row<VPT>(bn, row, lane, h, gr);
+  }
 #pragma unroll
   for (int j = 0; j < VPT; ++j) { a1[j] = 0.f; a2[j] = 0.f; }
 
@@ -473,11 +507,11 @@
           int LPR = PERTGNN_WAVE, typename TG = float, int LPH = LPR,
           bool PCH = false>
 __global__ void edge_attn_fused_bwd_col_kernel(
-    const TG* __restrict__ g, const QT* __restrict__ qkvs,
+    const TG* g, const QT* __restrict__ qkvs,
     const float* __restrict__ alpha, const float* __restrict__ dal,
     const int* __restrict__ col_ptr, const int* __restrict__ csc_dst,
-    const int* __restrict__ csc_eid, QT* __restrict__ dqkvs,
-    ET* __restrict__ de, int n, int h) {
+    const int* __restrict__ csc_eid, QT* dqkvs,
+    ET* __restrict__ de, int n, int h, long gld) {
   using S = Slice<VPT, VEC>;
   static_assert(VEC || LPR == PERTGNN_WAVE, "sub-wave rows need VEC layout");
   static_assert(PCH ? !VEC : (VEC || LPH == LPR),
@@ -503,7 +537,7 @@
       const long dst = csc_dst[p];
       float qd[VPT], gd[VPT], des[VPT];
       S::load(&qkvs[dst * ld], lane, h, qd);
-      S::load(&g[dst * h], lane, h, gd);
+      S::load(&g[dst * gld], lane, h, gd);
 #pragma unroll
       for (int j = 0; j < VPT; ++j) {
         const bool live = lane + j * PERTGNN_WAVE < h;
@@ -529,7 +563,7 @@
     const float a = alpha[eid * HM::HEADS + hd];
     float qd[VPT], gd[VPT], des[VPT];
     S::load(&qkvs[dst * ld], lane, h, qd);
-    S::load(&g[dst * h], lane, h, gd);
+    S::load(&g[dst * gld], lane, h, gd);
 #pragma unroll
     for (int j = 0; j < VPT; ++j) {
       const float dk1 = dl * qd[j];
@@ -679,7 +713,7 @@
                                        n, h, scale);                           \
       edge_attn_fused_bwd_col_kernel<V, true, float, float, LPR, float, LPH>   \
           <<<grid, block, 0, stream>>>(g, qkvs, alpha, dal, col_ptr, csc_dst,  \
-                                       csc_eid, dqkvs, de, n, h);              \
+                                       csc_eid, dqkvs, de, n, h, h);           \
     }                                                                          \
   } while (0)
 #define BWD_PCH(V, LPR, C)                                                     \
@@ -693,7 +727,7 @@
       edge_attn_fused_bwd_col_kernel<V, false, float, float, LPR, float, C,    \
                                      true>                                     \
           <<<grid, block, 0, stream>>>(g, qkvs, alpha, dal, col_ptr, csc_dst,  \
-                                       csc_eid, dqkvs, de, n, h);              \
+                                       csc_eid, dqkvs, de, n, h, h);           \
     }                                                                          \
   } while (0)
     const char* name = "edge_attn_fused launcher";
@@ -727,13 +761,13 @@
           g, qkvs, pifc, prpc, ea, astride, alpha, row_ptr, csr_src, dqkvs,    \
           dal, n, h, scale);                                                   \
       edge_attn_fused_bwd_col_kernel<V, true><<<grid, block, 0, stream>>>(     \
-          g, qkvs, alpha, dal, col_ptr, csc_dst, csc_eid, dqkvs, de, n, h);    \
+          g, qkvs, alpha, dal, col_ptr, csc_dst, csc_eid, dqkvs, de, n, h, h); \
     } else {                                                                   \
       edge_attn_fused_bwd_row_kernel<V, false><<<grid, block, 0, stream>>>(    \
           g, qkvs, pifc, prpc, ea, astride, alpha, row_ptr, csr_src, dqkvs,    \
           dal, n, h, scale);                                                   \
       edge_attn_fused_bwd_col_kernel<V, false><<<grid, block, 0, stream>>>(    \
-          g, qkvs, alpha, dal, col_ptr, csc_dst, csc_eid, dqkvs, de, n, h);    \
+          g, qkvs, alpha, dal, col_ptr, csc_dst, csc_eid, dqkvs, de, n, h, h); \
     }                                                                          \
     break;
     CASE(1) CASE(2) CASE(3) CASE(4) CASE(5) CASE(6) CASE(7) CASE(8)
@@ -829,10 +863,16 @@
                                   const int* csc_dst, const int* csc_eid,
                                   void* dqkvs_v, void* de_v, float* dal,
                                   int n, int h, long num_edges, int heads,
-                                  hipStream_t stream) {
+                                  hipStream_t stream, const AttnBnBwd* bn) {
   const __bf16* qkvs = (const __bf16*)qkvs_v;
   __bf16* dqkvs = (__bf16*)dqkvs_v;
   __bf16* de = (__bf16*)de_v;
+  if (bn && (!g16 || (h != 256 && h != 512)))
+    pertgnn_shape_fail("edge_attn_fused act16 launcher",
+                       g16 ? "bn, h" : "bn with fp32 g, h", h);
+  const AttnBnBwd bnk = bn ? *bn : AttnBnBwd{};
+  const __bf16* gcol = bn ? dqkvs + 3L * h : (const __bf16*)g_v;
+  const long gld = bn ? 4L * h : h;
   if (n == 0 && heads == 1) return;
   const float scale =
       attn_heads_ok(h, heads) ? 1.f / std::sqrt((float)(h / heads)) : 0.f;
@@ -851,12 +891,12 @@
                                        (const __bf16*)pifc_v,                  \
                                        (const __bf16*)prpc_v,                  \
                                        ea, astride, alpha, row_ptr, csr_src,   \
-                                       dqkvs, dal, n, h, scale);               \
+                                       dqkvs, dal, n, h, scale, bnk);          \
       edge_attn_fused_bwd_col_kernel<VPT, true, __bf16, __bf16, LPR, __bf16,   \
                                      LPH>                                      \
-          <<<grid, block, 0, stream>>>((const __bf16*)g_v, qkvs, alpha, dal,   \
-                                       col_ptr, csc_dst, csc_eid, dqkvs, de,   \
-                                       n, h);                                  \
+          <<<grid, block, 0, stream>>>(gcol, qkvs, alpha, dal, col_ptr,        \
+                                       csc_dst, csc_eid, dqkvs, de, n, h,      \
+                                       gld);                                   \
     } else if (g16) {                                                          \
       edge_attn_fused_bwd_row_kernel<VPT, true, __bf16, LPR, __bf16, float,    \
                                      LPH>                                      \
@@ -864,12 +904,12 @@
                                        (const float*)pifc_v,                   \
                                        (const float*)prpc_v,                   \
                                        ea, astride, alpha, row_ptr, csr_src,   \
-                                       dqkvs, dal, n, h, scale);               \
+                                       dqkvs, dal, n, h, scale, bnk);          \
       edge_attn_fused_bwd_col_kernel<VPT, true, __bf16, __bf16, LPR, __bf16,   \
                                      LPH>                                      \
-          <<<grid, block, 0, stream>>>((const __bf16*)g_v, qkvs, alpha, dal,   \
-                                       col_ptr, csc_dst, csc_eid, dqkvs, de,   \
-                                       n, h);                                  \
+          <<<grid, block, 0, stream>>>(gcol, qkvs, alpha, dal, col_ptr,        \
+                                       csc_dst, csc_eid, dqkvs, de, n, h,      \
+                                       gld);                                   \
     } else if (p16) {                                                          \
               \
       edge_attn_fused_bwd_row_kernel<VPT, true, __bf16, LPR, float, __bf16,    \
@@ -883,7 +923,7 @@
                                      LPH>                                      \
           <<<grid, block, 0, stream>>>((const float*)g_v, qkvs, alpha, dal,    \
                                        col_ptr, csc_dst, csc_eid, dqkvs, de,   \
-                                       n, h);                                  \
+                                       n, h, h);                               \
     } else {                                                                   \
       edge_attn_fused_bwd_row_kernel<VPT, true, __bf16, LPR, float, float,     \
                                      LPH>                                      \
@@ -896,7 +936,7 @@
                                      LPH>                                      \
           <<<grid, block, 0, stream>>>((const float*)g_v, qkvs, alpha, dal,    \
                                        col_ptr, csc_dst, csc_eid, dqkvs, de,   \
-                                       n, h);                                  \
+                                       n, h, h);                               \
     }                                                                          \
   } while (0)
 #define BWD16_H(VPT, LPR)                                                      \
diff --git a/csrc/hip/segops.hip b/csrc/hip/segops.hip
--- a/csrc/hip/segops.hip
+++ b/csrc/hip/segops.hip
@@ -1695,13 +1695,9 @@
     }
     __bf16 ov[8];
 #pragma unroll
-    for (int u = 0; u < 8; ++u) {
-      float gm = gv[u] * keep_inv;
-      if (!((bits >> u) & 1u)) gm = 0.f;
-      const float xhat = (xv[u] - mu[u]) * is[u];
-      ov[u] = (__bf16)(ga[u] * is[u] *
-                       (gm - p0[u] * invn - xhat * p1[u] * invn));
-    }
+    for (int u = 0; u < 8; ++u)
+      ov[u] = bn_bwd_dx16(gv[u], xv[u], (bits >> u) & 1u, mu[u], is[u], ga[u],
+                          p0[u], p1[u], invn, keep_inv);
     bn_st8(&dx[t], ov);
   }
 }
@@ -1975,6 +1971,21 @@
   bn_bwd_partials_dispatch((const __bf16*)g, (const __bf16*)x,
                            (const __bf16*)y, mean, invstd, n, h, relu,
                            partials, keep_inv, s);
+}
+
+void launch_bn_bwd_partials_affine16(const void* g, const void* x,
+                                     const unsigned char* mask,
+                                     const float* mean, const float* invstd,
+                                     long n, int h, float* partials,
+                                     float keep_inv, float* slab,
+                                     float* dgamma, float* dbeta,
+                                     hipStream_t s) {
+  if (n <= 0 || !mask || !bn_wide_ok(h))
+    pertgnn_shape_fail("bn_bwd_partials_affine16", "h", h);
+  bn_bwd_partials_wide_launch((const __bf16*)g, (const __bf16*)x,
+                              (const __bf16*)nullptr, mask, mean, invstd, n,
+                              h, true, partials, slab, dgamma, dbeta,
+                              keep_inv, s);
 }
 
 void launch_bn_bwd_apply_only16(const void* g, const void* x, const void* y,
diff --git a/pertgnn/models/pert_gnn.py b/pertgnn/models/pert_gnn.py
--- a/pertgnn/models/pert_gnn.py
+++ b/pertgnn/models/pert_gnn.py
@@ -149,6 +149,21 @@
 
     def forward_fused(self, x, edge_attr, ifc_weight, rpc_weight, csr,
                       out16=False, pifc=None, prpc=None):
+        qkvs, pifc, prpc = self._fused_operands(x, ifc_weight, rpc_weight,
+                                                pifc, prpc)
+        return ops.edge_attention_fused(qkvs, pifc, prpc, edge_attr, csr,
+                                        out16=out16, heads=self.heads)
+
+    def forward_fused_bn(self, x, edge_attr, ifc_weight, rpc_weight, csr, bn,
+                         comm=None, dropout_p=0.0, pifc=None, prpc=None):
+        qkvs, pifc, prpc = self._fused_operands(x, ifc_weight, rpc_weight,
+                                                pifc, prpc)
+        return ops.edge_attention_fused_bn_relu(
+            qkvs, pifc, prpc, edge_attr, csr, bn.weight, bn.bias,
+            bn.running_mean, bn.running_var, bn.momentum, bn.eps,
+            heads=self.heads, comm=comm, dropout_p=dropout_p)
+
+    def _fused_operands(self, x, ifc_weight, rpc_weight, pifc, prpc):
         h = self.out_channels
         if x.shape[1] != self.k_padded:
             x = torch.nn.functional.pad(x, (0, self.k_padded - x.shape[1]))
@@ -168,8 +183,7 @@
             qkvs = ops.linear(x, self.w4, self.b4)
             pifc = ops.linear(ifc_weight, self.we_ifc, None)
             prpc = ops.linear(rpc_weight, self.we_rpc, None)
-        return ops.edge_attention_fused(qkvs, pifc, prpc, edge_attr, csr,
-                                        out16=out16, heads=self.heads)
+        return qkvs, pifc, prpc
 
 
 class SAGEDeterministic(nn.Module):
@@ -290,14 +304,25 @@
                 )
             return conv(x, edge_index, edge_embeds, csr=csr, num_nodes=n)
 
+        fuse_bn = (out16 and self.training and n > 0
+                   and ops.bn_attn_fuse_enabled(hidden))
         for i, conv in enumerate(self.convs[:-1]):
-            x = run_conv(conv, x, out16=out16)
             bn = self.bns[i]
-            x = ops.batchnorm_relu(
-                x, bn.weight, bn.bias, bn.running_mean, bn.running_var,
-                bn.momentum, bn.eps, self.training, fuse_relu=True,
-                comm=self._bn_comm, out16=out16, dropout_p=self.dropout,
-            )
+            if fuse_bn:
+                pifc, prpc = ptables.get(id(conv), (None, None))
+                x = conv.forward_fused_bn(
+                    x, edge_attr, self.interface_embeds.weight,
+                    self.rpctype_embeds.weight, csr, bn,
+                    comm=self._bn_comm, dropout_p=self.dropout,
+                    pifc=pifc, prpc=prpc,
+                )
+            else:
+                x = run_conv(conv, x, out16=out16)
+                x = ops.batchnorm_relu(
+                    x, bn.weight, bn.bias, bn.running_mean, bn.running_var,
+                    bn.momentum, bn.eps, self.training, fuse_relu=True,
+                    comm=self._bn_comm, out16=out16, dropout_p=self.dropout,
+                )
             if self.training and bn.track_running_stats and bn.num_batches_tracked is not None:
                 bn.num_batches_tracked += 1
         x = run_conv(self.convs[-1], x)
diff --git a/pertgnn/ops/functional.py b/pertgnn/ops/functional.py
--- a/pertgnn/ops/functional.py
+++ b/pertgnn/ops/functional.py
@@ -393,30 +393,35 @@
             g.contiguous(), qkvs, pifc, prpc, edge_attr, alpha,
             row_ptr, csr_src, col_ptr, csc_dst, csc_eid, ctx.heads,
         )
-        if not _overlap_enabled():
-            h = de.shape[1]
-            if (h % 256 == 0 and not deterministic()
-                    and (pifc.shape[0] + prpc.shape[0]) * h * 4 <= 160 * 1024):
-                dpifc, dprpc = m.vocab_scatter_dual(de, edge_attr, pifc.shape[0], prpc.shape[0])
-                if dpifc.dtype != pifc.dtype:
-                    dpifc = dpifc.to(pifc.dtype)
-                    dprpc = dprpc.to(prpc.dtype)
-            else:
-                dpifc, dprpc = _edge_table_grads(m, de, pifc, prpc, edge_attr)
-            return dqkvs, dpifc, dprpc, None, None, None, None, None, None, None, None
-        cur = torch.cuda.current_stream()
-        side = _side_stream()
-        ev = torch.cuda.Event()
-        ev.record(cur)
-        side.wait_event(ev)
-        with torch.cuda.stream(side):
+        dpifc, dprpc = _attn_table_grads(m, de, pifc, prpc, edge_attr)
+        return dqkvs, dpifc, dprpc, None, None, None, None, None, None, None, None
+
+
+def _attn_table_grads(m, de, pifc, prpc, edge_attr):
+    if not _overlap_enabled():
+        h = de.shape[1]
+        if (h % 256 == 0 and not deterministic()
+                and (pifc.shape[0] + prpc.shape[0]) * h * 4 <= 160 * 1024):
+            dpifc, dprpc = m.vocab_scatter_dual(de, edge_attr, pifc.shape[0], prpc.shape[0])
+            if dpifc.dtype != pifc.dtype:
+                dpifc = dpifc.to(pifc.dtype)
+                dprpc = dprpc.to(prpc.dtype)
+        else:
             dpifc, dprpc = _edge_table_grads(m, de, pifc, prpc, edge_attr)
-        ev2 = torch.cuda.Event()
-        ev2.record(side)
-        cur.wait_event(ev2)
-        _mark_cross_stream(dpifc, cur)
-        _mark_cross_stream(dprpc, cur)
-        return dqkvs, dpifc, dprpc, None, None, None, None, None, None, None, None
+        return dpifc, dprpc
+    cur = torch.cuda.current_stream()
+    side = _side_stream()
+    ev = torch.cuda.Event()
+    ev.record(cur)
+    side.wait_event(ev)
+    with torch.cuda.stream(side):
+        dpifc, dprpc = _edge_table_grads(m, de, pifc, prpc, edge_attr)
+    ev2 = torch.cuda.Event()
+    ev2.record(side)
+    cur.wait_event(ev2)
+    _mark_cross_stream(dpifc, cur)
+    _mark_cross_stream(dprpc, cur)
+    return dpifc, dprpc
 
 
 def _fused_eager(qkvs, pifc, prpc, edge_attr, csr, heads):
@@ -588,40 +593,48 @@
     return t
 
 
+def _bn_forward(m, x, gamma, beta, running_mean, running_var, momentum, eps,
+                training, fuse_relu, comm, dropout_p):
+    sync = comm is not None and getattr(comm, "distributed", False) and training
+    drop = float(dropout_p) if training else 0.0
+    if drop > 0.0:
+        assert fuse_relu, "fused dropout rides the ReLU mask (model.py:102-103)"
+    seed = _rng_counter(x.device) if drop > 0.0 else torch.empty(
+        0, dtype=torch.int64, device=x.device)
+    if sync:
+        partials = m.bn_stats(x)
+        comm.all_reduce_(partials)
+        fin = (m.bn_finalize_apply16 if x.dtype == torch.bfloat16
+               else m.bn_finalize_apply)
+        out = fin(
+            x, partials, gamma, beta, running_mean, running_var,
+            momentum, eps, training, fuse_relu, drop, seed)
+    else:
+        fwd = (m.bn_relu_fwd16 if x.dtype == torch.bfloat16
+               else m.bn_relu_fwd)
+        out = fwd(
+            x, gamma, beta, running_mean, running_var, momentum, eps,
+            training, fuse_relu, drop, seed
+        )
+    y, save_mean, save_invstd = out[:3]
+    mask = out[3] if len(out) > 3 and out[3].numel() > 0 else None
+    keep_inv = 1.0 / (1.0 - drop) if drop > 0.0 else 1.0
+    return y, save_mean, save_invstd, mask, sync, keep_inv
+
+
 class _BNReLUFn(torch.autograd.Function):
     @staticmethod
     def forward(ctx, x, gamma, beta, running_mean, running_var, momentum, eps,
                 training, fuse_relu, comm, out16=False, dropout_p=0.0):
-        m = ext()
-        sync = comm is not None and getattr(comm, "distributed", False) and training
-        drop = float(dropout_p) if training else 0.0
-        if drop > 0.0:
-            assert fuse_relu, "fused dropout rides the ReLU mask (model.py:102-103)"
-        seed = _rng_counter(x.device) if drop > 0.0 else torch.empty(
-            0, dtype=torch.int64, device=x.device)
-        if sync:
-            partials = m.bn_stats(x)
-            comm.all_reduce_(partials)
-            fin = (m.bn_finalize_apply16 if x.dtype == torch.bfloat16
-                   else m.bn_finalize_apply)
-            out = fin(
-                x, partials, gamma, beta, running_mean, running_var,
-                momentum, eps, training, fuse_relu, drop, seed)
-        else:
-            fwd = (m.bn_relu_fwd16 if x.dtype == torch.bfloat16
-                   else m.bn_relu_fwd)
-            out = fwd(
-                x, gamma, beta, running_mean, running_var, momentum, eps,
-                training, fuse_relu, drop, seed
-            )
-        y, save_mean, save_invstd = out[:3]
-        mask = out[3] if len(out) > 3 and out[3].numel() > 0 else None
+        y, save_mean, save_invstd, mask, sync, keep_inv = _bn_forward(
+            ext(), x, gamma, beta, running_mean, running_var, momentum, eps,
+            training, fuse_relu, comm, dropout_p)
         ctx.save_for_backward(x, gamma, save_mean, save_invstd,
                               y if mask is None else mask)
         ctx.y16 = y.dtype == torch.bfloat16
         ctx.fuse_relu = fuse_relu
         ctx.comm = comm if sync else None
-        ctx.keep_inv = 1.0 / (1.0 - drop) if drop > 0.0 else 1.0
+        ctx.keep_inv = keep_inv
         return y
 
     @staticmethod
@@ -648,6 +661,67 @@
             )
         return (dx, dgamma, dbeta, None, None, None, None, None, None, None,
                 None, None)
+
+
+def bn_attn_fuse_enabled(h: int) -> bool:
+    import os
+    return (h in (256, 512)
+            and os.environ.get("PERTGNN_NO_BN_ATTN_FUSE", "0") != "1")
+
+
+class _AttnBNReLUFn(torch.autograd.Function):
+
+    @staticmethod
+    def forward(ctx, qkvs, pifc, prpc, gamma, beta, edge_attr, row_ptr,
+                csr_src, col_ptr, csc_dst, csc_eid, heads, running_mean,
+                running_var, momentum, eps, comm, dropout_p):
+        m = ext()
+        x, alpha = m.edge_attn_fused_fwd(qkvs, pifc, prpc, edge_attr, row_ptr,
+                                         csr_src, True, heads)
+        y, save_mean, save_invstd, mask, sync, keep_inv = _bn_forward(
+            m, x, gamma, beta, running_mean, running_var, momentum, eps,
+            True, True, comm, dropout_p)
+        if mask is None:
+            raise RuntimeError(
+                "fused attention+BN needs the BN keep mask (n > 0, H in "
+                f"{{256, 512}}); got x {tuple(x.shape)}")
+        ctx.save_for_backward(qkvs, pifc, prpc, gamma, edge_attr, alpha,
+                              row_ptr, csr_src, col_ptr, csc_dst, csc_eid,
+                              x, save_mean, save_invstd, mask)
+        ctx.heads = heads
+        ctx.comm = comm if sync else None
+        ctx.keep_inv = keep_inv
+        return y
+
+    @staticmethod
+    def backward(ctx, g):
+        (qkvs, pifc, prpc, gamma, edge_attr, alpha, row_ptr, csr_src, col_ptr,
+         csc_dst, csc_eid, x, save_mean, save_invstd, mask) = ctx.saved_tensors
+        m = ext()
+        g = g.contiguous()
+        partials = ()
+        if ctx.comm is not None:
+            partials_local = m.bn_bwd_partials16(
+                g, x, mask, save_mean, save_invstd, True, ctx.keep_inv)
+            partials_global = partials_local.clone()
+            ctx.comm.all_reduce_(partials_global)
+            partials = (partials_global, partials_local)
+        dqkvs, de, dgamma, dbeta = m.edge_attn_bn_bwd16(
+            g, x, mask, gamma, save_mean, save_invstd, ctx.keep_inv, qkvs,
+            pifc, prpc, edge_attr, alpha, row_ptr, csr_src, col_ptr, csc_dst,
+            csc_eid, ctx.heads, *partials)
+        dpifc, dprpc = _attn_table_grads(m, de, pifc, prpc, edge_attr)
+        return (dqkvs, dpifc, dprpc, dgamma, dbeta) + (None,) * 13
+
+
+def edge_attention_fused_bn_relu(qkvs, pifc, prpc, edge_attr, csr, gamma,
+                                 beta, running_mean, running_var, momentum,
+                                 eps, heads=1, comm=None, dropout_p=0.0):
+    row_ptr, csr_src, col_ptr, csc_dst, csc_eid = csr
+    return _AttnBNReLUFn.apply(
+        qkvs, pifc, prpc, gamma, beta, edge_attr, row_ptr, csr_src, col_ptr,
+        csc_dst, csc_eid, heads, running_mean, running_var, momentum, eps,
+        comm, dropout_p)
 
 
 class _EagerSyncBNFn(torch.autograd.Function):
@@ -849,6 +923,8 @@
     "edge_attention",
     "edge_attention_fused",
     "edge_attention_fused_infer",
+    "edge_attention_fused_bn_relu",
+    "bn_attn_fuse_enabled",
     "embedding",
     "pattern_pool",
     "embed_concat_node",
```
